# pachterlab/kallisto

Measured on AMD Instinct MI355X. Metric: M paired-end reads/sec quantified (human txome index), higher is better.
Workload: dtype u64+f64

## Files before the change

### kallisto_amd/csrc/kamd_ctx.hip

```cpp
#include "kamd_dev.h"

namespace {
void tuning_defaults(kamd_tuning* t) {
  memset(t, 0, sizeof *t);
  t->text_verify = 1; t->items_per_wave = 1024; t->refill_min = 8; t->lds_pad = -1;
  t->em_form = 3; t->em_local_block = 1024; t->em_group_div = -1; t->em_split_len = 16; t->em_small_nnz = -1; t->em_entries_per_lane = -1; t->em_windowed = 2; t->em_graph = 1; t->em_row_lanes = 4;
  t->em_fin_blocks = 1024; t->dedup_form = 2; t->align_chunks = -1; t->em_reg_slices = 1;
  t->em_hybrid = 1; t->overflow_second_pass = 1; t->em_giant_nnz = -1; t->em_blocked = 1;
}
void tuning_merge(kamd_tuning* t, const kamd_tuning& n) {
  if (n.text_verify == 1 || n.text_verify == 2) t->text_verify = n.text_verify;
  if (n.dedup_form == 1 || n.dedup_form == 2) t->dedup_form = n.dedup_form;
  if (n.items_per_wave >= 64) t->items_per_wave = n.items_per_wave;
  if (n.refill_min >= 1 && n.refill_min <= 64) t->refill_min = n.refill_min;
  if (n.lds_pad != 0) t->lds_pad = n.lds_pad < 0 ? -1 : n.lds_pad;
  if (n.em_form >= 1 && n.em_form <= 3) t->em_form = n.em_form;
  if (n.em_local_block == 128 || n.em_local_block == 256 || n.em_local_block == 512 || n.em_local_block == 1024) t->em_local_block = n.em_local_block;
  if (n.em_split_len >= 1 && n.em_split_len <= 64) t->em_split_len = n.em_split_len;
  if (n.em_group_div >= 1 && n.em_group_div <= 1024) t->em_group_div = n.em_group_div;
  else if (n.em_group_div < 0) t->em_group_div = -1;
  if (n.em_small_nnz != 0) t->em_small_nnz = n.em_small_nnz < 0 ? -1 : std::min(n.em_small_nnz, 4096);
  if (n.em_entries_per_lane != 0) t->em_entries_per_lane = n.em_entries_per_lane < 0 ? -1 : n.em_entries_per_lane;
  if (n.em_windowed == 1 || n.em_windowed == 2) t->em_windowed = n.em_windowed;
  if (n.em_graph == 1 || n.em_graph == 2) t->em_graph = n.em_graph;
// ... 10 lines not shown
  const char* e = getenv("KAMD_TUNE");
  if (!e || !*e) return;
  kamd_tuning n; memset(&n, 0, sizeof n);
  struct Field { const char* name; int32_t kamd_tuning::*p; bool onoff; };
  static const Field fields[] = {
    {"text_verify", &kamd_tuning::text_verify, true}, {"items_per_wave", &kamd_tuning::items_per_wave, false}, {"refill_min", &kamd_tuning::refill_min, false},
    {"lds_pad", &kamd_tuning::lds_pad, false}, {"em_form", &kamd_tuning::em_form, false}, {"em_entries_per_lane", &kamd_tuning::em_entries_per_lane, false},
    {"em_windowed", &kamd_tuning::em_windowed, true}, {"em_graph", &kamd_tuning::em_graph, true}, {"em_row_lanes", &kamd_tuning::em_row_lanes, false},
    {"em_fin_blocks", &kamd_tuning::em_fin_blocks, false}, {"em_local_block", &kamd_tuning::em_local_block, false}, {"em_group_div", &kamd_tuning::em_group_div, false},
    {"em_split_len", &kamd_tuning::em_split_len, false}, {"dedup_form", &kamd_tuning::dedup_form, false}, {"align_chunks", &kamd_tuning::align_chunks, false},
    {"em_small_nnz", &kamd_tuning::em_small_nnz, false}, {"em_reg_slices", &kamd_tuning::em_reg_slices, true}, {"em_hybrid", &kamd_tuning::em_hybrid, true},
    {"overflow_second_pass", &kamd_tuning::overflow_second_pass, false}, {"em_giant_nnz", &kamd_tuning::em_giant_nnz, false}, {"em_blocked", &kamd_tuning::em_blocked, true}};
  std::string all(e);
  for (size_t pos = 0; pos < all.size();) {
    size_t end = all.find(',', pos);
    if (end == std::string::npos) end = all.size();
    const std::string kv = all.substr(pos, end - pos);
    pos = end + 1;
    const size_t eq = kv.find('=');
    if (eq == std::string::npos) continue;
    const std::string key = kv.substr(0, eq), val = kv.substr(eq + 1);
    bool known = false;
    for (const Field& f : fields) {
      if (key != f.name) continue;
      known = true;
      int32_t v = atoi(val.c_str());
      if (key == "em_form") v = val == "streamed" ? 1 : val == "csr" ? 2 : val == "local" ? 3 : v;
      if (key == "overflow_second_pass" && v == 0) v = 2;
      n.*(f.p) = f.onoff ? (v != 0 ? 1 : 2) : v;
    }
    if (!known) fprintf(stderr, "[kallisto_amd] KAMD_TUNE: unknown field '%s' ignored\n", key.c_str());
  }
  tuning_merge(t, n);
}
}
namespace kamdi {
void apply_quant_opts(kamd_ctx* c, const kamd_quant_opts* o) {
  c->ix.no_jump = o->no_jump ? 1 : 0;
  c->ix.union_mode = o->do_union ? 1 : 0;
  c->ix.comprehensive = (o->strand != 0 && (o->no_jump || o->do_union || c->ix.n_shades)) ? 1 : 0;
}
void apply_tuning(kamd_ctx* c) {
  c->items_per_wave = c->tune.items_per_wave; c->refill_min = c->tune.refill_min;
}
int sync_state(kamd_ctx* c) {
  if (!c->state_pin) HIPC(hipHostMalloc((void**)&c->state_pin, sizeof(DevState), hipHostMallocDefault));
  HIPC(hipMemcpyAsync(c->state_pin, c->state.p, sizeof(DevState), hipMemcpyDeviceToHost, c->stream));
  HIPC(hipStreamSynchronize(c->stream));
  memcpy(&c->host_state, c->state_pin, sizeof(DevState));
  return 0;
}
int push_state(kamd_ctx* c) {
  HIPC(hipMemcpyAsync(c->state.p, &c->host_state, sizeof(DevState), hipMemcpyHostToDevice, c->stream));
  return 0;
}
}

extern "C" uint32_t kamd_abi_version(void) { return KAMD_ABI_VERSION; }
extern "C" int kamd_ctx_create(int device, void* hip_stream, kamd_ctx** out) {
  if (!out) return kamd::fail(-1, "kamd_ctx_create: null output pointer");
  *out = nullptr;
  int ndev = 0;
  if (hipGetDeviceCount(&ndev) != hipSuccess || ndev == 0)
    return kamd::fail(-102, "kamd_ctx_create: no HIP device available (this library has no CPU path)");
  if (device < 0 || device >= ndev) return kamd::fail(-1, "kamd_ctx_create: bad device ordinal");
  HIPC(hipSetDevice(device));
  kamd_ctx* c = new kamd_ctx;
  c->device = device;
  c->stream = (hipStream_t)hip_stream;
  { int v = 0; if (hipDeviceGetAttribute(&v, hipDeviceAttributeMultiprocessorCount, device) != hipSuccess || v <= 0) v = 256; c->n_cus = v; }
  if (c->state.ensure(sizeof(DevState), 0, c->stream)) { delete c; return -100; }
  memset(&c->host_state, 0, sizeof c->host_state);
  if (push_state(c)) { delete c; return -100; }
  if (hipEventCreate(&c->ev0) != hipSuccess || hipEventCreate(&c->ev1) != hipSuccess || hipEventCreate(&c->ev2) != hipSuccess || hipEventCreate(&c->ev3) != hipSuccess) { delete c; return kamd::fail(-100, "hipEventCreate failed"); }
  if (c->stats_a.ensure(sizeof(DevStatsA), 0, c->stream) || hipMemsetAsync(c->stats_a.p, 0, sizeof(DevStatsA), c->stream) != hipSuccess) { delete c; return -100; }
  tuning_defaults(&c->tune);
  tuning_from_env(&c->tune);
  apply_tuning(c);
  *out = c;
  return 0;
}

extern "C" int kamd_ctx_tune(kamd_ctx* c, const kamd_tuning* t) {
  if (!c || !t) return kamd::fail(-1, "kamd_ctx_tune: null argument");
  tuning_merge(&c->tune, *t);
  apply_tuning(c);
  return 0;
}
extern "C" int kamd_ctx_get_tuning(const kamd_ctx* c, kamd_tuning* out) {
  if (!c || !out) return kamd::fail(-1, "kamd_ctx_get_tuning: null argument");
  *out = c->tune;
  return 0;
}

extern "C" void kamd_ctx_destroy(kamd_ctx* c) {
  if (!c) return;
  (void)hipSetDevice(c->device);
  (void)hipStreamSynchronize(c->stream);
  comm_detach_all(c);
  if (c->ev0) (void)hipEventDestroy(c->ev0);
  if (c->ev1) (void)hipEventDestroy(c->ev1);
  if (c->ev2) (void)hipEventDestroy(c->ev2);
  if (c->ev3) (void)hipEventDestroy(c->ev3);
  if (c->al_stream) { (void)hipStreamSynchronize(c->al_stream); (void)hipStreamDestroy(c->al_stream); }
  if (c->al_ev_in) (void)hipEventDestroy(c->al_ev_in);
  if (c->al_ev_out) (void)hipEventDestroy(c->al_ev_out);
  for (hipEvent_t e : c->al_ev_chunk) if (e) (void)hipEventDestroy(e);
  if (c->ev_fin0) (void)hipEventDestroy(c->ev_fin0);
  if (c->ev_fin1) (void)hipEventDestroy(c->ev_fin1);
  for (hipEvent_t e : c->aa_ev) if (e) (void)hipEventDestroy(e);
  for (hipEvent_t e : c->rec_ev) if (e) (void)hipEventDestroy(e);
  for (hipEvent_t e : c->bus_ev) if (e) (void)hipEventDestroy(e);
  if (c->ev_ab0) (void)hipEventDestroy(c->ev_ab0);
  if (c->ev_ab1) (void)hipEventDestroy(c->ev_ab1);
  if (c->em_stream) (void)hipStreamDestroy(c->em_stream);
  if (c->em_side_stream) { (void)hipStreamSynchronize(c->em_side_stream); (void)hipStreamDestroy(c->em_side_stream); }
  if (c->em_ev_fork) (void)hipEventDestroy(c->em_ev_fork);
  if (c->em_ev_join) (void)hipEventDestroy(c->em_ev_join);
  if (c->em_pin) (void)hipHostFree(c->em_pin);
  if (c->plan_pin) (void)hipHostFree(c->plan_pin);
  if (c->state_pin) (void)hipHostFree(c->state_pin);
  c->em_clk.release();
  if (c->hy_giant_stream) { (void)hipStreamSynchronize(c->hy_giant_stream); (void)hipStreamDestroy(c->hy_giant_stream); }
  if (c->hy_ev_sell) (void)hipEventDestroy(c->hy_ev_sell);
  if (c->hy_ev_giant) (void)hipEventDestroy(c->hy_ev_giant);
  if (c->ev_mg0) (void)hipEventDestroy(c->ev_mg0);
  if (c->ev_mg1) (void)hipEventDestroy(c->ev_mg1);
  if (c->ev_ov0) (void)hipEventDestroy(c->ev_ov0);
  if (c->ev_ov1) (void)hipEventDestroy(c->ev_ov1);
  if (c->ov_stream) { (void)hipStreamSynchronize(c->ov_stream); (void)hipStreamDestroy(c->ov_stream); }
  for (hipEvent_t e : {c->ov_ev_in, c->ov_ev_done, c->ov_ev_t0, c->ov_ev_t1}) if (e) (void)hipEventDestroy(e);
  if (c->ov_pin) (void)hipHostFree(c->ov_pin);
  c->ov_state.release();
  for (DBuf* b : {&c->hy_sub, &c->hy_a, &c->hy_b, &c->hy_x, &c->hy_maps, &c->hy_gb[0], &c->hy_gb[1], &c->hy_gb[2], &c->hy_gb[3], &c->hy_gb[4], &c->hy_gb[5]}) b->release();
  if (c->fld_stream) { (void)hipStreamSynchronize(c->fld_stream); (void)hipStreamDestroy(c->fld_stream); }
  if (c->fld_ev) (void)hipEventDestroy(c->fld_ev);
  if (c->fld_ev_in) (void)hipEventDestroy(c->fld_ev_in);
  if (c->fld_host) (void)hipHostFree(c->fld_host);
  if (c->fq_host) (void)hipHostFree(c->fq_host);
  if (c->sell_cache) sell_cache_free(c->sell_cache);
  for (void* p : c->index_allocs) (void)hipFree(p);
  for (DBuf* b : {&c->dense, &c->stream_buf, &c->rec_off, &c->overflow_items, &c->overflow_scratch, &c->state, &c->rec_slot,
                  &c->retry, &c->ttable, &c->tstore, &c->stats_a, &c->list, &c->cand, &c->cand_off, &c->cand_slot, &c->ctable, &c->tup_bound, &c->tup_off, &c->tup_big, &c->raw2, &c->overflow_left, &c->stats_b, &c->clist, &c->sizes, &c->explicit_items,
                  &c->explicit_items_big, &c->exp_stream, &c->exp_off, &c->exp_scratch, &c->bs_cp, &c->bs_samp, &c->raw, &c->dense_first, &c->exp_key, &c->cand_key, &c->ec_first, &c->pm_a, &c->pm_b, &c->pm_rank, &c->eml_tmp, &c->ems_tmp, &c->ems_plan, &c->ems_maps, &c->fld_tl, &c->fld_card, &c->fld_scratch, &c->fld_items, &c->fld_cand,
                  &c->block_sums, &c->ec_off, &c->ec_ids, &c->ec_counts, &c->em_alpha, &c->em_next, &c->em_eff,
                  &c->em_state, &c->em_cn, &c->em_colcnt, &c->em_coloff, &c->em_colrow,
                  &c->em_segoff, &c->em_segt, &c->em_partial, &c->em_a0, &c->em_a1, &c->em_single, &c->em_actflag, &c->em_actpos, &c->em_active, &c->pt_label, &c->pt_flag, &c->pt_len,
                  &c->pt_rowpos, &c->pt_nnzpos, &c->pt_off, &c->pt_ids, &c->pt_counts, &c->pt_wcounts, &c->pt_hist, &c->pt_ck_alpha,
                  &c->pt_ck_a, &c->fq_tiles, &c->fq_nlpos[0], &c->fq_nlpos[1], &c->fq_recs, &c->fq_res, &c->fq_words, &c->fq_len, &c->aa_frames, &c->aa_flen, &c->aa_scratch, &c->aa_offlist, &c->aa_ctr, &c->inf_members, &c->inf_res, &c->txt_counts, &c->txt_res,
                  &c->rec_table, &c->rec_scratch, &c->rec_big_scratch, &c->rec_big_items, &c->rec_ctr, &c->bus_blk, &c->bus_ctr})
    b->release();
  delete c;
}

namespace {
__global__ void k_bm_fill(const u64* __restrict__ ec_off, const u32* __restrict__ ec_ids, const u32* __restrict__ which, u32 stride, u32* words) {
  const u32 e = which[blockIdx.x];
  u32* w = words + (u64)blockIdx.x * stride;
  for (u64 j = ec_off[e] + threadIdx.x; j < ec_off[e + 1]; j += blockDim.x) { const u32 x = ec_ids[j]; atomicOr(&w[x >> 5], 1u << (x & 31)); }
}
}
extern "C" int kamd_index_upload(kamd_ctx* c, const kamd_index* hix) {
  if (!c || !hix) return kamd::fail(-1, "kamd_index_upload: null argument");
  HIPC(hipSetDevice(c->device));
  kamd_index_view v;
  if (int rc = kamd_index_get_view(hix, &v)) return rc;
  const bool build_table = v.table == nullptr;
  HIPC(hipStreamSynchronize(c->stream));
  c->has_index = false;
  for (void* p : c->index_allocs) (void)hipFree(p);
  c->index_allocs.clear();
  DevIndex d{};
  d.k = v.k; d.n_buckets = v.n_buckets; d.n_ecs = v.n_ecs;
  d.table_layout = (int)v.table_layout; d.tag_q = v.tag_q; d.tag_dsh = v.tag_dsh; d.tag_w = v.tag_w;
  const u64 slots = (v.n_buckets + v.pad_buckets) * v.slots_per_bucket;
  if (!build_table) {
    if (int rc = upload(c, (const u64*)v.table, (size_t)(v.n_buckets + v.pad_buckets) * 8, &d.table)) return rc;
    if (int rc = upload(c, v.slot_block, slots, &d.slot_block)) return rc;
    if (int rc = upload(c, v.slot_dist, slots, &d.slot_dist)) return rc;
  }
  if (int rc = upload(c, v.uec_ec, v.n_uec, &d.uec_ec)) return rc;
  if (int rc = upload(c, (const u64*)v.ec_off, v.n_ecs + 1, &d.ec_off)) return rc;
  if (int rc = upload(c, v.ec_ids, v.ec_nnz, &d.ec_ids)) return rc;
  std::vector<uint8_t> ne(v.n_ecs + 1);
  for (u64 e = 0; e < v.n_ecs; e++) ne[e] = v.ec_off[e + 1] > v.ec_off[e];
  if (int rc = upload(c, ne.data(), v.n_ecs, &d.ec_nonempty)) return rc;
  std::vector<u32> ecn(v.n_uec + 1);
  for (u64 u = 0; u < v.n_uec; u++) ecn[u] = v.uec_ec[u] | (ne[v.uec_ec[u]] ? 0x80000000u : 0u);
  if (int rc = upload(c, ecn.data(), v.n_uec, &d.uec_ecn)) return rc;
  if (int rc = upload(c, v.onlist_bits, v.onlist_words, &d.onlist_bits)) return rc;
  d.n_shades = v.n_shades;
  if (v.n_shades) {
    if (int rc = upload(c, (const u64*)v.core_off, v.n_ecs + 1, &d.core_off)) return rc;
    if (int rc = upload(c, v.core_ids, (size_t)v.core_nnz, &d.core_ids)) return rc;
    if (int rc = upload(c, (const u64*)v.shade_off, v.n_ecs + 1, &d.shade_off)) return rc;
    if (int rc = upload(c, v.shade_ids, (size_t)v.shade_nnz, &d.shade_ids)) return rc;
// ... 434 lines not shown
  c->em_coll_ms = 0.f; c->em_coll_n = 0;
  if (int rc = kamd_em_run_partitioned(c, (uint32_t)m->rank, (uint32_t)m->world, comm_sum_cb, m, eff_lens, n_targets, n_iter, min_rounds, alpha, abz, rounds)) return rc;
  const auto t_fin = std::chrono::steady_clock::now();
  HIPC(hipSetDevice(c->device));
  if (int rc = m->tmp_a.ensure(2 * n_targets * sizeof(double), 0, c->stream)) return rc;
  double* d = m->tmp_a.as<double>();
  HIPC(hipMemcpyAsync(d, alpha, n_targets * sizeof(double), hipMemcpyHostToDevice, c->stream));
  HIPC(hipMemcpyAsync(d + n_targets, abz, n_targets * sizeof(double), hipMemcpyHostToDevice, c->stream));
  HIPC(hipStreamSynchronize(c->stream));
  if (int rc = comm_allreduce(m, d, 2 * n_targets, 3)) return rc;
  HIPC(hipMemcpyAsync(alpha, d, n_targets * sizeof(double), hipMemcpyDeviceToHost, c->stream));
  HIPC(hipMemcpyAsync(abz, d + n_targets, n_targets * sizeof(double), hipMemcpyDeviceToHost, c->stream));
  HIPC(hipStreamSynchronize(c->stream));
  c->em_coll_ms += std::chrono::duration<float, std::milli>(std::chrono::steady_clock::now() - t_fin).count(); c->em_coll_n += 1;
  return 0;
}

extern "C" int kamd_quant_batches(kamd_ctx* c, const kamd_quant_opts* o, const kamd_batch* batches, uint64_t n_batches, const int32_t* target_lens,
                                  uint64_t n_targets, kamd_comm* comm, kamd_quant_out* out) {
  if (!c || !o || (n_batches && !batches) || !target_lens || !out || !out->flens || !out->eff_lens || !out->est_counts)
    return kamd::fail(-1, "kamd_quant_batches: null argument");
  if (comm && comm->ctx != c) return kamd::fail(-1, "kamd_quant_batches: communicator of another context");
  if (n_targets != c->n_targets) return kamd::fail(-1, "kamd_quant_batches: n_targets differs from the uploaded index");
  const bool multi = comm && (comm->world > 1 || comm->nccl);
  const bool rank0 = !comm || comm->rank == 0;
  const bool estimate = o->paired && o->fld == 0.0;
  memset(out->flens, 0, KAMD_MAX_FRAG_LEN * sizeof(uint32_t));
  uint64_t used = 0, n_proc = 0;
  for (uint64_t b = 0; b < n_batches; b++) {
    const kamd_batch& B = batches[b];
    if (b == 0 && estimate && rank0) if (int rc = kamd_fld_prefetch(c, o, B.d_words, B.d_len, B.n_items, B.max_len)) return rc;
    if (int rc = kamd_pseudoalign(c, o, B.d_words, B.d_len, B.n_items, B.max_len)) return rc;
    n_proc += B.n_items;
    if (estimate && used < 10000 && rank0) if (int rc = kamd_fld_from_batch(c, o, B.d_words, B.d_len, B.n_items, B.max_len, out->flens, &used)) return rc;
  }
  if (multi) {
    if (int rc = kamd_comm_sum_u64_host(c, comm, &n_proc, 1)) return rc;
    if (estimate) {
      std::vector<uint32_t> pack(KAMD_MAX_FRAG_LEN + 2);
      for (int r = 0; r < comm->world; r++) {
        if (r > 0 && comm->rank == r)
          for (uint64_t b = 0; b < n_batches && used < 10000; b++)
            if (int rc = kamd_fld_from_batch(c, o, batches[b].d_words, batches[b].d_len, batches[b].n_items, batches[b].max_len, out->flens, &used)) return rc;
        memcpy(pack.data(), out->flens, KAMD_MAX_FRAG_LEN * sizeof(uint32_t));
        pack[KAMD_MAX_FRAG_LEN] = (uint32_t)used; pack[KAMD_MAX_FRAG_LEN + 1] = (uint32_t)(used >> 32);
        if (int rc = kamd_comm_broadcast_host(c, comm, pack.data(), pack.size() * sizeof(uint32_t), r)) return rc;
        memcpy(out->flens, pack.data(), KAMD_MAX_FRAG_LEN * sizeof(uint32_t));
        used = (uint64_t)pack[KAMD_MAX_FRAG_LEN] | ((uint64_t)pack[KAMD_MAX_FRAG_LEN + 1] << 32);
        if (used >= 10000) break;
      }
    }
    if (int rc = kamd_ec_allreduce(c, comm)) return rc;
  }
  std::vector<double> mft(KAMD_MAX_FRAG_LEN);
  std::thread eff_thread([&] {
    if (o->fld == 0.0) kamd_mean_frag_lens_trunc(out->flens, mft.data());
    else kamd_trunc_gaussian_fld(0, KAMD_MAX_FRAG_LEN, o->fld, o->sd, mft.data());
    kamd_eff_lens(target_lens, n_targets, mft.data(), out->eff_lens);
  });
  const int fin_rc = kamd_ec_finalize(c, nullptr);
  eff_thread.join();
  if (fin_rc) return fin_rc;
  int32_t rounds = 0;
  if (multi) { if (int rc = kamd_em_run_comm(c, comm, out->eff_lens, n_targets, 10000, 50, out->est_counts, out->alpha_before_zeroes, &rounds)) return rc; }
  else if (int rc = kamd_em_run(c, nullptr, nullptr, nullptr, nullptr, 0, out->eff_lens, n_targets, 10000, 50, out->est_counts, out->alpha_before_zeroes, &rounds)) return rc;
  if (out->tpm) kamd_counts_to_tpm(out->est_counts, out->eff_lens, n_targets, out->tpm);
  out->n_processed = n_proc; out->em_rounds = rounds;
  return 0;
}
```

### kallisto_amd/csrc/kamd_dev.h

```cpp
#pragma once

#include <hip/hip_runtime.h>

#include <dlfcn.h>

#include <algorithm>
#include <cstring>
#include <string>
#include <chrono>
#include <thread>
#include <vector>

#include "../../include/kallisto_amd.h"
#include "kamd_core.h"
#include "kamd_fq_core.h"
#include "kamd_host.h"
#include "kamd_em_local.h"
#include "kamd_em_sell.h"

#define HIPC(x)                                                                                   \
  do {                                                                                            \
    hipError_t e_ = (x);                                                                          \
    if (e_ != hipSuccess) return kamd::fail(-100, std::string(#x) + ": " + hipGetErrorString(e_)); \
  } while (0)

namespace kamdi {

typedef unsigned long long u64;
typedef unsigned int u32;

constexpr int BLOCK = 256;
constexpr int TUPLE_CAP = 12;
constexpr int TUPLE_CAP_BIG = 1024;
constexpr int EXPLICIT_HITS = 256;

struct DevIndex {
  const u64* table; u64 n_buckets;
  int table_layout; u32 tag_q, tag_dsh, tag_w;
  const u32* slot_block; const u32* slot_dist;
  const u32* uec_ec;
  const u64* ec_off; const u32* ec_ids; const uint8_t* ec_nonempty;
  const u32* uec_ecn;
  const u32* onlist_bits;
  const u32* ec_bm_slot; const u32* bm_words; u32 bm_stride, bm_min;
  u64 n_ecs; int k;
  const u64* unitig_blk_off; const u32* unitig_len; const u32* blk_unitig; const u32* blk_lb; const u32* blk_ub; const u32* blk_ec;
  const u64* blk_pos_off; const u32* blk_posw; const uint8_t* blk_sense; const int32_t* target_lens;
  const u64* dtable; u64 n_dbuckets; u64 dummy_slot; u32 dummy_uec; u32 dummy_strand;
  const u32* utext;
  int no_jump;
  int union_mode;
  int comprehensive;
  u64 n_shades; const u64* core_off; const u32* core_ids; const u64* shade_off; const u32* shade_ids; const u32* shade_colour;
};
__host__ __device__ inline kamd::Table make_table(const DevIndex& ix, bool partial) {
  kamd::Table t{(const uint64_t*)ix.table, ix.n_buckets};
  t.layout = (uint8_t)ix.table_layout; t.q = (uint8_t)ix.tag_q; t.dsh = (uint8_t)ix.tag_dsh; t.tagw = (uint8_t)ix.tag_w;
  t.dslots = (const uint64_t*)ix.dtable; t.n_dbuckets = ix.n_dbuckets; t.dummy_uec = ix.dummy_uec; t.dummy_slot = ix.dummy_slot;
  t.dummy_strand = ix.dummy_strand != 0; t.partial = partial && !ix.union_mode && !ix.n_shades;
  t.no_jump = ix.no_jump != 0;
// ... 144 lines not shown
using namespace kamdi;
namespace {
__global__ void k_copy_words(const u32* __restrict__ src, u64 n, u32* dst) {
  u64 i = (u64)blockIdx.x * blockDim.x + threadIdx.x;
  if (i < n) dst[i] = src[i];
}
__global__ void k_copy_offsets(const u64* __restrict__ src, u64 n, u64 base, u64* dst) {
  u64 i = (u64)blockIdx.x * blockDim.x + threadIdx.x;
  if (i < n) dst[i] = src[i] + base;
}
}

struct kamd_ctx {
  int device = 0;
  hipStream_t stream = nullptr;
  bool has_index = false;
  DevIndex ix{};
  std::vector<void*> index_allocs;
  u64 n_ecs = 0, n_targets = 0;
  u32 n_set_bitmaps = 0;
  kamd_table_info tinfo{};
  DBuf dense, stream_buf, rec_off, overflow_items, overflow_scratch, state, rec_slot, retry, ttable, list;
  DBuf cand, cand_off, cand_slot, ctable, clist, sizes, block_sums, tup_bound, tup_off, tup_big;
  DBuf raw2, overflow_left, stats_b;
  u64 overflow_second_total = 0;
  DBuf ov_state; DevState* ov_pin = nullptr; hipStream_t ov_stream = nullptr; hipEvent_t ov_ev_in = nullptr, ov_ev_done = nullptr, ov_ev_t0 = nullptr, ov_ev_t1 = nullptr;
  bool ov_side_pending = false;
  u64 last_fin_big = 0;
  DBuf explicit_items, explicit_items_big, exp_stream, exp_off, exp_scratch, bs_cp, bs_samp, raw, dense_first, exp_key, cand_key, ec_first;
  DBuf ec_off, ec_ids, ec_counts;
  DBuf em_alpha, em_next, em_eff, em_state, em_cn, em_colcnt, em_coloff, em_colrow, em_segoff, em_segt, em_partial, em_a0, em_a1, em_single, em_actflag, em_actpos, em_active;
  DBuf pm_a, pm_b, pm_rank;
  DBuf eml_tmp, ems_tmp, ems_plan, ems_maps;
  SellCache* sell_cache = nullptr;
  u64 ec_generation = 0;
  int last_em_plan_cached = 0;
  DBuf fq_tiles, fq_nlpos[2], fq_recs, fq_res, fq_words, fq_len;
  void* fq_host = nullptr;
  u64 fq_batch_reads = 0; int32_t fq_batch_max_len = 0, fq_batch_files = 0;
  DBuf fld_tl, fld_card, fld_scratch, fld_items, fld_cand;
  void* fld_host = nullptr; u64 fld_host_cap = 0;
  hipStream_t fld_stream = nullptr; hipEvent_t fld_ev = nullptr, fld_ev_in = nullptr;
  struct { const uint32_t* w = nullptr; const uint16_t* l = nullptr; u64 n = 0; int32_t max_len = 0, strand = 0, so = 0; bool valid = false; } fld_pending;
  struct { const uint32_t* w = nullptr; const uint16_t* l = nullptr; u64 n = 0; int32_t max_len = 0, strand = 0, so = 0, comp = 0; bool valid = false; } fld_deferred;
  DBuf pt_label, pt_flag, pt_len, pt_rowpos, pt_nnzpos, pt_off, pt_ids, pt_counts, pt_wcounts, pt_hist, pt_ck_alpha, pt_ck_a;
  DevState host_state{};
  DevState* state_pin = nullptr;
  u64 tcap = 0, ccap = 0;
  DBuf tstore;
  bool ttable_clean = false;
  u64 recs_total = 0;
  u64 multi_before = 0;
  u64 n_distinct_tuples = 0;
  float last_absorb_ms = 0.f; hipEvent_t ev_ab0 = nullptr, ev_ab1 = nullptr;
  kamd_ec_result result{};
  bool finalized = false;
  u64 exp_words_done = 0;
  hipEvent_t ev0 = nullptr, ev1 = nullptr;
  float last_align_ms = 0.f, last_em_ms = 0.f, last_classify_ms = 0.f;
  hipEvent_t ev2 = nullptr, ev3 = nullptr, ev_fin0 = nullptr, ev_fin1 = nullptr;
  DBuf stats_a;
  hipStream_t al_stream = nullptr; hipEvent_t al_ev_in = nullptr, al_ev_out = nullptr; std::vector<hipEvent_t> al_ev_chunk;
  float last_finalize_ms = 0.f; u64 last_fin_records = 0, last_fin_stream_words = 0, last_fin_cand_words = 0;
  hipStream_t em_stream = nullptr;
  hipStream_t em_side_stream = nullptr; hipEvent_t em_ev_fork = nullptr, em_ev_join = nullptr;
  void* em_pin = nullptr; size_t em_pin_bytes = 0;
  void* plan_pin = nullptr; size_t plan_pin_bytes = 0;
  DBuf em_clk;
  DBuf hy_sub, hy_a, hy_b, hy_x, hy_maps;
  DBuf hy_gb[6];
  hipStream_t hy_giant_stream = nullptr;
  hipEvent_t hy_ev_sell = nullptr, hy_ev_giant = nullptr;
  uint64_t last_em_max_comp_nnz = 0, last_em_giant_nnz = 0, last_em_giant_rows = 0, last_em_giant_tr = 0;
  uint32_t last_em_giant_chunks = 0; uint64_t last_em_giant_pieces = 0; int last_em_graph_fallback = 0; float last_em_plan_ms = 0.f;
  float last_merge_ms = 0.f, em_coll_ms = 0.f; uint32_t em_coll_n = 0; hipEvent_t ev_mg0 = nullptr, ev_mg1 = nullptr;
  const uint32_t* labels_override = nullptr;
  bool em_prefer_hybrid = false;
  uint64_t overflow_total = 0; float overflow_ms = 0.f; hipEvent_t ev_ov0 = nullptr, ev_ov1 = nullptr;
  int items_per_wave = 1024, refill_min = 8;
  kamd_tuning tune{};
  bool track_order = false;
  bool had_overflow_items = false;
  int n_cus = 0, last_em_k = 0; unsigned last_em_grid = 0, last_em_lds = 0;
  uint64_t last_em_iters = 0, last_em_nnz = 0, last_em_nnz_multi = 0, last_em_nseg = 0, last_em_necs = 0;
  DBuf aa_frames, aa_flen, aa_scratch, aa_offlist, aa_ctr;
  bool aa_ready = false;
  kamd_aa_stats aa_stats{};
  hipEvent_t aa_ev[3] = {nullptr, nullptr, nullptr};
  DBuf inf_members, inf_res, txt_counts, txt_res;
  DBuf rec_table, rec_scratch, rec_big_scratch, rec_big_items, rec_ctr;
  u64 rec_table_gen = 0, rec_table_cap = 0, rec_chunk = 0, rec_second = 0;
  int rec_small_cap = 0;
  hipEvent_t rec_ev[3] = {nullptr, nullptr, nullptr};
  float rec_table_ms = 0.f, rec_items_ms = 0.f;
  DBuf bus_blk, bus_ctr;
  hipEvent_t bus_ev[2] = {nullptr, nullptr};
  std::vector<struct kamd_comm*> comms;
};

namespace kamdi {
int sync_state(kamd_ctx* c);
int push_state(kamd_ctx* c);
void apply_quant_opts(kamd_ctx* c, const kamd_quant_opts* o);
void apply_tuning(kamd_ctx* c);
void comm_detach_all(kamd_ctx* c);
int index_build_device(kamd_ctx* c, const kamd_index* hix, const kamd_index_view& v, DevIndex* d, kamd_table_info* info);
int exclusive_scan(kamd_ctx* c, const u32* sizes, u64 n, u64* out, u64* d_total);
int tuples_clear(kamd_ctx* c);
int absorb_tuples(kamd_ctx* c, const u32* batch, const u64* rec_off, u64 n, u64 batch_words, u64 key_base, u64 n_tuple_bound,
                  const u64* first_idx = nullptr, u32 fixed_stride = 0, u64 item0 = 0);
template <class T>
int upload(kamd_ctx* c, const T* host, size_t n, const T** dev) {
  void* p = nullptr;
  size_t bytes = std::max<size_t>(n, 1) * sizeof(T);
  HIPC(hipMalloc(&p, bytes));
  c->index_allocs.push_back(p);
  if (n) HIPC(hipMemcpyAsync(p, host, n * sizeof(T), hipMemcpyHostToDevice, c->stream));
  *dev = reinterpret_cast<const T*>(p);
  return 0;
}
}
```

### kallisto_amd/csrc/kamd_ec.hip

```cpp
#include "kamd_dev.h"

namespace {

__global__ void k_table_init(TSlot* t, u64 cap) {
  u64 i = (u64)blockIdx.x * blockDim.x + threadIdx.x;
  if (i < cap) { t[i].tag = 0; t[i].owner = ~0ULL; t[i].count = 0; t[i].first = ~0ULL; }
}
__global__ void k_rec_insert(const u32* __restrict__ stream, const u64* __restrict__ rec_off, const u64* __restrict__ idx,
                             u64 r0, u64 n, TSlot* table, u64 mask, u64 seed, u64* rec_slot) {
  u64 i = (u64)blockIdx.x * blockDim.x + threadIdx.x;
  if (i >= n) return;
  const u64 r = idx ? idx[i] : r0 + i;
  const u64 off = rec_off[r];
  if (off == ~0ULL || stream[off] == 0u) return;
  const u32 m = stream[off + 1];
  const u64 tag = rec_hash(stream + off + 1, m + 1, seed);
  u64 s = (tag >> 1) & mask;
  for (;;) {
    u64 old = atomicCAS(&table[s].tag, 0ULL, tag);
    if (old == 0ULL || old == tag) break;
    s = (s + 1) & mask;
  }
  atomicMin(&table[s].owner, off);
  rec_slot[r] = s;
// ... 152 lines not shown
  for (int q = 0; q < ABS_Q; q++) {
    cand[q] = live[q] && !slow[q] && old[q] != 0ULL && (old[q] >> 32) == (h[q] >> 32);
    const u32* o = ((old[q] & TAG_LOCAL) ? batch : store) + ((old[q] & 0x7FFFFFFFULL) - 1);
    const u32 m = w[q][1];
#pragma unroll
    for (int j = 0; j < 5; j++) ow[q][j] = (cand[q] && (u32)j <= m) ? o[1 + j] : 0u;
  }
#pragma unroll
  for (int q = 0; q < ABS_Q; q++) {
    if (!live[q] || slow[q]) continue;
    bool same = cand[q] && ow[q][0] == w[q][1];
#pragma unroll
    for (int j = 0; j < 4; j++) if ((u32)j < w[q][1]) same = same && ow[q][1 + j] == w[q][2 + j];
    if (same) {
      atomicAdd(&table[sl[q]].count, (u64)w[q][0]);
      if (track & 1) atomicMin(&table[sl[q]].first, key_base + i + (u64)q * T);
    } else slow[q] = true;
  }
  u32 my[ABS_Q]; u64 own_s[ABS_Q]; bool is_owner[ABS_Q];
#pragma unroll
  for (int q = 0; q < ABS_Q; q++) {
    is_owner[q] = false; my[q] = 0; own_s[q] = 0;
    if (!slow[q]) continue;
    const u64 r = i + (u64)q * T, o = off[q];
    const u32 m = batch[o + 1];
    const u64 hh = rec_hash(batch + o + 1, m + 1, 1);
    const u64 mine = (hh & 0xFFFFFFFF00000000ULL) | TAG_LOCAL | (o + 1);
    u64 s = (hh >> 1) & mask;
    bool placed = false;
    for (u32 probes = 0; probes < max_probe; probes++) {
      u64 od = table[s].tag;
      if (od == 0ULL) od = atomicCAS(&table[s].tag, 0ULL, mine);
      if (od == 0ULL) { is_owner[q] = true; table[s].owner = o; placed = true; break; }
      if ((od >> 32) == (mine >> 32)) {
        const u32* ob = ((od & TAG_LOCAL) ? batch : store) + ((od & 0x7FFFFFFFULL) - 1);
        bool same = ob[1] == m;
        for (u32 j = 0; same && j < m; j++) same = ob[2 + j] == batch[o + 2 + j];
        if (same) { placed = true; break; }
      }
      s = (s + 1) & mask;
    }
    if (placed) {
      atomicAdd(&table[s].count, (u64)batch[o]);
      if (track & 1) atomicMin(&table[s].first, key_base + r);
    } else fail[atomicAdd(&st->tl_fail, 1ULL)] = r;
    if (is_owner[q]) { own_s[q] = s; my[q] = atomicAdd(&blk_n, 1u); atomicAdd(&blk_words, m + 2u); }
  }
  __syncthreads();
  if (threadIdx.x == 0 && blk_n) { blk_base = atomicAdd(&st->tl_n, (u64)blk_n); atomicAdd(&st->bound_words, (u64)blk_words); }
  __syncthreads();
#pragma unroll
  for (int q = 0; q < ABS_Q; q++) if (is_owner[q]) list[blk_base + my[q]] = own_s[q];
}
__global__ __launch_bounds__(BLOCK) void k_tup_store(const u32* __restrict__ batch, u32* store, TSlot* table, u64* list, u64 first_new,
                                                     u64 n_new, DevState* st) {
  __shared__ u32 wsum[BLOCK / 64]; __shared__ u64 blk_base;
  const u64 i = (u64)blockIdx.x * blockDim.x + threadIdx.x;
  u64 s = 0, off = 0; u32 need = 0;
  if (i < n_new) { s = list[first_new + i] & 0xFFFFFFFFULL; off = table[s].owner; need = batch[off + 1] + 2u; }
  const u32 incl = wave_incl_scan(need);
  if (lane_id() == 63) wsum[threadIdx.x >> 6] = incl;
  __syncthreads();
  if (threadIdx.x == 0) { u32 t = 0; for (int j = 0; j < BLOCK / 64; j++) t += wsum[j]; blk_base = t ? atomicAdd(&st->ts_words, (u64)t) : 0ULL; }
  __syncthreads();
  if (i >= n_new) return;
  u32 before = 0;
  for (u32 j = 0; j < (threadIdx.x >> 6); j++) before += wsum[j];
  const u64 dst = blk_base + before + incl - need;
  for (u32 j = 0; j < need; j++) store[dst + j] = batch[off + j];
  table[s].owner = dst;
  table[s].tag = (table[s].tag & 0xFFFFFFFF00000000ULL) | (dst + 1);
  list[first_new + i] = s | (dst << 32);
}
__global__ void k_tup_rehash(const u32* __restrict__ store, const TSlot* __restrict__ old, TSlot* nu, u64 mask, u64* list, u64 n) {
  const u64 i = (u64)blockIdx.x * blockDim.x + threadIdx.x;
  if (i >= n) return;
  const TSlot o = old[list[i] & 0xFFFFFFFFULL];
  const u32 m = store[o.owner + 1];
  const u64 h = rec_hash(store + o.owner + 1, m + 1, 1);
  const u64 tag = (h & 0xFFFFFFFF00000000ULL) | (o.owner + 1);
  u64 s = (h >> 1) & mask;
  while (atomicCAS(&nu[s].tag, 0ULL, tag) != 0ULL) s = (s + 1) & mask;
  nu[s].owner = o.owner; nu[s].count = o.count; nu[s].first = o.first;
  list[i] = s | (o.owner << 32);
}

constexpr u64 SHADE_SMALL = 64;
constexpr u64 SHADE_SLOT_FACTOR = 4;
constexpr u32 RES_BIG_MIN = 16;
__global__ void k_bound_tuples(DevIndex ix, const u32* __restrict__ stream, const TSlot* table, const u64* list, u64 n,
                               u32* per_tuple, u32* big_idx, u32* shade_idx, DevState* st) {
  u64 i = (u64)blockIdx.x * blockDim.x + threadIdx.x;
  u64 b = 0;
  bool big = false, huge = false, sh_small = false, sh_long = false;
  if (i < n) {
    const u64 off = list[i] >> 32;
    const u32 m = stream[off + 1];
    u64 core_b;
    if (ix.n_shades) {
      const kamd::ShadeTables sh = shade_tables(ix);
      const kamd::SetTables core{sh.core_off, sh.core_ids};
      core_b = kamd::set_size_bound(core, stream + off + 2, (int)m, ix.union_mode != 0);
      const u64 S = kamd::shaded_size_bound(sh, stream + off + 2, (int)m, ix.union_mode != 0) - core_b;
      b = core_b + (ix.union_mode ? S : SHADE_SLOT_FACTOR * S) + 2;
      sh_small = !ix.union_mode && S != 0 && core_b + S <= SHADE_SMALL;
      sh_long = !ix.union_mode && S != 0 && !sh_small;
    } else {
      const kamd::SetTables stt{(const uint64_t*)ix.ec_off, ix.ec_ids};
      core_b = kamd::set_size_bound(stt, stream + off + 2, (int)m, ix.union_mode != 0);
      b = core_b + 2;
    }
    per_tuple[i] = (u32)b;
    big = big_idx && !ix.union_mode && core_b > RES_BIG_MIN;
    huge = big && core_b > 1024;
  }
  b = wave_sum64(b);
  if (lane_id() == 0 && b) atomicAdd(&st->bound_words, b);
  const u64 bm = __ballot(big && !huge), hm = __ballot(huge);
  if (bm) {
    u64 base = 0;
    if (lane_id() == 0) base = atomicAdd(&st->n_big, (u64)__popcll(bm));
    base = shfl_u64(base, 0);
    if (big && !huge) big_idx[base + __popcll(bm & ((1ULL << lane_id()) - 1ULL))] = (u32)i;
  }
  if (hm) {
    u64 base = 0;
    if (lane_id() == 0) base = atomicAdd(&st->n_huge, (u64)__popcll(hm));
    base = shfl_u64(base, 0);
    if (huge) big_idx[n - 1 - (base + __popcll(hm & ((1ULL << lane_id()) - 1ULL)))] = (u32)i;
  }
  const u64 sm = __ballot(sh_small), lm = __ballot(sh_long);
  if (sm) {
    u64 base = 0;
    if (lane_id() == 0) base = atomicAdd(&st->n_sh_small, (u64)__popcll(sm));
    base = shfl_u64(base, 0);
    if (sh_small) shade_idx[base + __popcll(sm & ((1ULL << lane_id()) - 1ULL))] = (u32)i;
  }
  if (lm) {
    u64 base = 0;
    if (lane_id() == 0) base = atomicAdd(&st->n_sh_long, (u64)__popcll(lm));
    base = shfl_u64(base, 0);
    if (sh_long) shade_idx[n - 1 - (base + __popcll(lm & ((1ULL << lane_id()) - 1ULL)))] = (u32)i;
  }
}
__global__ void k_bound_singles(DevIndex ix, const u32* __restrict__ dense, DevState* st) {
  u64 e = (u64)blockIdx.x * blockDim.x + threadIdx.x;
  u64 b = 0;
  if (e < ix.n_ecs && dense[e]) b = ix.ec_off[e + 1] - ix.ec_off[e] + 2;
  b = wave_sum64(b);
  if (lane_id() == 0 && b) atomicAdd(&st->bound_words, b);
}
__global__ void k_cand_singles(DevIndex ix, const u32* __restrict__ dense, const u64* __restrict__ dense_first, u32* cand,
                               u64* cand_off, u64* cand_key, DevState* st) {
  u64 e = (u64)blockIdx.x * blockDim.x + threadIdx.x;
  const bool have = e < ix.n_ecs && dense[e] != 0;
  const u32* ids = nullptr; u32 n = 0;
  if (have) { ids = ix.ec_ids + ix.ec_off[e]; n = (u32)(ix.ec_off[e + 1] - ix.ec_off[e]); }
  const bool longset = n > 64;
  if (have && !longset) {
    u32 keep = 0;
    for (u32 j = 0; j < n; j++) keep += onlisted(ix.onlist_bits, ids[j]);
    if (keep) {
      u64 off = atomicAdd(&st->cand_words, (u64)keep + 2);
      u64 r = atomicAdd(&st->cand_recs, 1ULL);
      u32* w = cand + off;
      w[0] = dense[e]; w[1] = keep;
      u32 o = 0;
      for (u32 j = 0; j < n; j++) if (onlisted(ix.onlist_bits, ids[j])) w[2 + o++] = ids[j];
      cand_off[r] = off;
      if (cand_key) cand_key[r] = dense_first[e];
    }
  }
  u64 m = __ballot(longset);
  while (m) {
    const int src = __ffsll((long long)m) - 1;
    m &= m - 1;
    const u64 se = shfl_u64(e, src);
    const u32* sid = ix.ec_ids + ix.ec_off[se];
    const u32 sn = (u32)__shfl((int)n, src, 64);
    u32 keep = 0;
    for (u32 j = lane_id(); j < sn; j += 64) keep += onlisted(ix.onlist_bits, sid[j]);
#pragma unroll
    for (int d = 1; d < 64; d <<= 1) keep += (u32)__shfl_xor((int)keep, d, 64);
    if (keep == 0) continue;
    u64 off = 0, r = 0;
    if (lane_id() == 0) { off = atomicAdd(&st->cand_words, (u64)keep + 2); r = atomicAdd(&st->cand_recs, 1ULL); }
    off = shfl_u64(off, 0); r = shfl_u64(r, 0);
    u32* w = cand + off;
    if (lane_id() == 0) { w[0] = dense[se]; w[1] = keep; cand_off[r] = off; if (cand_key) cand_key[r] = dense_first[se]; }
    u32 o = 0;
    for (u32 j0 = 0; j0 < sn; j0 += 64) {
      const u32 j = j0 + lane_id();
      const u32 x = j < sn ? sid[j] : 0u;
      const bool ok = j < sn && onlisted(ix.onlist_bits, x);
      const u64 bm = __ballot(ok);
      if (ok) w[2 + o + __popcll(bm & ((1ULL << lane_id()) - 1ULL))] = x;
      o += (u32)__popcll(bm);
    }
  }
}
constexpr int RES_LANES = 16;
constexpr int RES_BLOCK = BLOCK;
__global__ __launch_bounds__(RES_BLOCK) void k_resolve(DevIndex ix, const u32* __restrict__ stream, const TSlot* table,
                                                   const u64* list, u64 n, const u64* __restrict__ slot_off, u32* cand, u64* cand_off,
                                                   u64* cand_key, const DevState* st) {
  const u64 base_words = st->cand_words, base_recs = st->cand_recs;
  const u64 gid = ((u64)blockIdx.x * blockDim.x + threadIdx.x) / RES_LANES;
  const bool valid = gid < n;
  const int lane = lane_id();
  const int sub = lane & (RES_LANES - 1);
  const int gsh = lane & ~(RES_LANES - 1);
  TSlot sl; sl.owner = 0; sl.count = 0; sl.tag = 0; sl.first = ~0ULL;
  u32 m = 0, best = 0, nb = 0;
  const u32* es = nullptr; const u32* base = nullptr;
  u64 my_off = 0; u32 my_sz = 0xFFFFFFFFu;
  bool small = false;
  if (valid) {
// ... 509 lines not shown
  if (c->tune.dedup_form != 1 && stream_words < 0xFFFFFFFFULL) {
    c->host_state.n_retry = 0;
    HIPC(hipMemcpyAsync(&((DevState*)c->state.p)->n_retry, &c->host_state.n_retry, sizeof(u64), hipMemcpyHostToDevice, c->stream));
    hipLaunchKernelGGL(k_rec_dedup, dim3(grid_for(n, BLOCK)), dim3(BLOCK), 0, c->stream, stream, rec_off, r0, n, table, cap - 1, list, keys, track,
                       max_probe ? max_probe : 0xFFFFFFFFu, (DevState*)c->state.p);
    HIPC(hipGetLastError());
    if (int rc = sync_state(c)) return rc;
    return c->host_state.n_retry ? 2 : 0;
  }
  if (int rc = slot_buf.ensure(r1 * sizeof(u64), 0, c->stream)) return rc;
  if (int rc = c->retry.ensure(2 * n * sizeof(u64), 0, c->stream)) return rc;
  u64* retry_a = c->retry.as<u64>();
  u64* retry_b = retry_a + n;
  const u64* idx = nullptr;
  u64 count = n;
  for (u64 seed = 1; count; seed++) {
    c->host_state.n_retry = 0;
    HIPC(hipMemcpyAsync(&((DevState*)c->state.p)->n_retry, &c->host_state.n_retry, sizeof(u64), hipMemcpyHostToDevice, c->stream));
    hipLaunchKernelGGL(k_rec_insert, dim3(grid_for(count, BLOCK)), dim3(BLOCK), 0, c->stream, stream, rec_off, idx, r0, count,
                       table, cap - 1, seed, slot_buf.as<u64>());
    hipLaunchKernelGGL(k_rec_verify, dim3(grid_for(count, VERIFY_BLOCK)), dim3(VERIFY_BLOCK), 0, c->stream, stream, rec_off, idx, r0, count,
                       table, slot_buf.as<u64>(), retry_b, list, keys, track, (DevState*)c->state.p);
    HIPC(hipGetLastError());
    if (int rc = sync_state(c)) return rc;
    count = c->host_state.n_retry;
    std::swap(retry_a, retry_b);
    idx = retry_a;
    if (seed > 64) return kamd::fail(-101, "dedup_records: tag collisions did not resolve");
  }
  return 0;
}


int exclusive_scan(kamd_ctx* c, const u32* sizes, u64 n, u64* out, u64* d_total) {
  const u64 nblocks = std::max<u64>(1, (n + SCAN_ELEMS - 1) / SCAN_ELEMS);
  if (int rc = c->block_sums.ensure((nblocks + 2) * sizeof(u64), 0, c->stream)) return rc;
  hipLaunchKernelGGL(k_scan_local, dim3((unsigned)nblocks), dim3(BLOCK), 0, c->stream, sizes, n, out, c->block_sums.as<u64>());
  hipLaunchKernelGGL(k_scan_blocks, dim3(1), dim3(BLOCK), 0, c->stream, c->block_sums.as<u64>(), nblocks, d_total);
  hipLaunchKernelGGL(k_scan_add, dim3((unsigned)nblocks), dim3(BLOCK), 0, c->stream, out, n, c->block_sums.as<u64>());
  HIPC(hipGetLastError());
  return 0;
}

u64 pow2_at_least(u64 x) { u64 p = 1024; while (p < x) p <<= 1; return p; }

int tuples_clear(kamd_ctx* c) {
  if (c->tcap && !c->ttable_clean) {
    hipLaunchKernelGGL(k_table_init, dim3(grid_for(c->tcap, BLOCK)), dim3(BLOCK), 0, c->stream, c->ttable.as<TSlot>(), c->tcap);
    HIPC(hipGetLastError());
    c->ttable_clean = true;
  }
  c->host_state.tl_n = 0; c->host_state.ts_words = 0; c->host_state.tl_fail = 0;
  c->n_distinct_tuples = 0;
  return 0;
}
int tuples_resize(kamd_ctx* c, u64 cap) {
  if (cap > (1ULL << 32)) return kamd::fail(-101, "absorb_tuples: the tuple table would need more than 2^32 slots");
  const u64 n = c->host_state.tl_n;
  DBuf nu;
  if (int rc = nu.ensure(cap * sizeof(TSlot), 0, c->stream)) return rc;
  hipLaunchKernelGGL(k_table_init, dim3(grid_for(cap, BLOCK)), dim3(BLOCK), 0, c->stream, nu.as<TSlot>(), cap);
  if (n) hipLaunchKernelGGL(k_tup_rehash, dim3(grid_for(n, BLOCK)), dim3(BLOCK), 0, c->stream, (const u32*)c->tstore.as<u32>(), (const TSlot*)c->ttable.as<TSlot>(),
                            nu.as<TSlot>(), cap - 1, c->list.as<u64>(), n);
  HIPC(hipGetLastError());
  HIPC(hipStreamSynchronize(c->stream));
  c->ttable.release();
  c->ttable = nu; c->tcap = cap; c->ttable_clean = n == 0;
  return 0;
}
int absorb_tuples(kamd_ctx* c, const u32* batch, const u64* rec_off, u64 n, u64 batch_words, u64 key_base, u64 n_tuple_bound,
                  const u64* first_idx, u32 fixed_stride, u64 item0) {
  if (n == 0) return 0;
  if (batch_words >= 0x7FFFFFF0ULL) return kamd::fail(-1, "kamd_pseudoalign: the record stream of one batch must stay below 2^31 words (use smaller batches)");
  DevState* dst = (DevState*)c->state.p;
  if (!c->ev_ab0) { HIPC(hipEventCreate(&c->ev_ab0)); HIPC(hipEventCreate(&c->ev_ab1)); }
  HIPC(hipEventRecord(c->ev_ab0, c->stream));
  const u64 bound = std::min(n, n_tuple_bound);
  u64 want = pow2_at_least(std::max<u64>(bound / 4, 2 * c->host_state.tl_n) + 16);
  if (c->tcap == 0) {
    c->tcap = want;
    if (int rc = c->ttable.ensure(c->tcap * sizeof(TSlot), 0, c->stream)) return rc;
    hipLaunchKernelGGL(k_table_init, dim3(grid_for(c->tcap, BLOCK)), dim3(BLOCK), 0, c->stream, c->ttable.as<TSlot>(), c->tcap);
    c->ttable_clean = true;
  } else if (2 * c->host_state.tl_n + 16 > c->tcap) {
    if (int rc = tuples_resize(c, pow2_at_least(4 * c->host_state.tl_n + 16))) return rc;
  }
  if (int rc = c->list.ensure((c->host_state.tl_n + bound + 1) * sizeof(u64), c->host_state.tl_n * sizeof(u64), c->stream)) return rc;
  if (int rc = c->retry.ensure(2 * (bound + 1) * sizeof(u64), 0, c->stream)) return rc;
  u64* fail_a = c->retry.as<u64>();
  u64* fail_b = fail_a + bound + 1;
  const u64* idx = first_idx;
  u64 count = n;
  for (int round = 0; count; round++) {
    if (round > 40) return kamd::fail(-101, "absorb_tuples: the tuple table does not settle");
    const u64 tl_before = c->host_state.tl_n;
    c->host_state.tl_fail = 0; c->host_state.bound_words = 0;
    if (int rc = push_state(c)) return rc;
    if (!idx && fixed_stride >= 6 && (fixed_stride & 1) == 0)
      hipLaunchKernelGGL(k_tup_absorb4, dim3(grid_for((count + ABS_Q - 1) / ABS_Q, BLOCK)), dim3(BLOCK), 0, c->stream, batch, (const u32*)c->tstore.as<u32>(), count,
                         c->ttable.as<TSlot>(), c->tcap - 1, c->list.as<u64>(), key_base, c->track_order ? 1 : 0, 64u, fail_a, dst, fixed_stride, item0);
    else
    hipLaunchKernelGGL(k_tup_absorb, dim3(grid_for(count, BLOCK)), dim3(BLOCK), 0, c->stream, batch, (const u32*)c->tstore.as<u32>(), rec_off, idx, count,
                       c->ttable.as<TSlot>(), c->tcap - 1, c->list.as<u64>(), key_base,
                       c->track_order ? 1 : 0, 64u, fail_a, dst,
                       fixed_stride, item0);
    HIPC(hipGetLastError());
    c->ttable_clean = false;
    if (int rc = sync_state(c)) return rc;
    const u64 n_new = c->host_state.tl_n - tl_before, new_words = c->host_state.bound_words;
    if (n_new) {
      if (c->host_state.ts_words + new_words >= 0x7FFFFFF0ULL) return kamd::fail(-101, "absorb_tuples: more than 2^31 words of distinct tuples");
      if (int rc = c->tstore.ensure((c->host_state.ts_words + new_words + 2) * sizeof(u32), c->host_state.ts_words * sizeof(u32), c->stream)) return rc;
      hipLaunchKernelGGL(k_tup_store, dim3(grid_for(n_new, BLOCK)), dim3(BLOCK), 0, c->stream, batch, c->tstore.as<u32>(), c->ttable.as<TSlot>(),
                         c->list.as<u64>(), tl_before, n_new, dst);
      HIPC(hipGetLastError());
      c->host_state.ts_words += new_words;
    }
    count = c->host_state.tl_fail;
    if (count) {
      if (int rc = tuples_resize(c, c->tcap * 4)) return rc;
      std::swap(fail_a, fail_b);
      idx = fail_b;
    }
  }
  c->n_distinct_tuples = c->host_state.tl_n;
  HIPC(hipEventRecord(c->ev_ab1, c->stream));
  HIPC(hipEventSynchronize(c->ev_ab1));
  float ms = 0.f;
  HIPC(hipEventElapsedTime(&ms, c->ev_ab0, c->ev_ab1));
  c->last_absorb_ms += ms;
  return 0;
}

}
extern "C" int kamd_ec_dense_counts(kamd_ctx* c, uint32_t** d_counts, uint64_t* n) {
  if (!c || !d_counts || !n) return kamd::fail(-1, "kamd_ec_dense_counts: null argument");
  *d_counts = c->dense.as<u32>(); *n = c->n_ecs;
  return 0;
}
extern "C" int kamd_ec_tuples_export(kamd_ctx* c, uint64_t* n_words, uint64_t* n_tuples) {
  if (!c || !n_words || !n_tuples) return kamd::fail(-1, "kamd_ec_tuples_export: null argument");
  HIPC(hipSetDevice(c->device));
  if (int rc = sync_state(c)) return rc;
  c->host_state.bound_words = 0;
  if (int rc = push_state(c)) return rc;
  const u64 n = c->n_distinct_tuples;
  if (n) hipLaunchKernelGGL(k_tuple_export_size, dim3(grid_for(n, BLOCK)), dim3(BLOCK), 0, c->stream, c->tstore.as<u32>(),
                            c->ttable.as<TSlot>(), c->list.as<u64>(), n, (DevState*)c->state.p);
  HIPC(hipGetLastError());
  if (int rc = sync_state(c)) return rc;
  *n_words = c->host_state.bound_words; *n_tuples = n;
  return 0;
}
extern "C" int kamd_ec_tuples_copy(kamd_ctx* c, uint32_t* d_out_words, uint64_t* d_out_rec_off) {
  if (!c || !d_out_words || !d_out_rec_off) return kamd::fail(-1, "kamd_ec_tuples_copy: null argument");
  HIPC(hipSetDevice(c->device));
  const u64 n = c->n_distinct_tuples;
  c->host_state.cand_words = 0; c->host_state.cand_recs = 0;
  if (int rc = push_state(c)) return rc;
  if (n) hipLaunchKernelGGL(k_tuple_export_offsets, dim3(grid_for(n, BLOCK)), dim3(BLOCK), 0, c->stream, c->tstore.as<u32>(),
                            c->ttable.as<TSlot>(), c->list.as<u64>(), n, d_out_words, (u64*)d_out_rec_off, (DevState*)c->state.p);
  HIPC(hipGetLastError());
  return sync_state(c);
}
extern "C" int kamd_ec_tuples_replace(kamd_ctx* c, const uint32_t* d_words, uint64_t n_words, const uint64_t* d_rec_off,
                                      uint64_t n_recs) {
  if (!c) return kamd::fail(-1, "kamd_ec_tuples_replace: null argument");
  if (c->track_order) return kamd::fail(-1, "kamd_ec_tuples_replace: merged records have no input order (kamd_ec_track_order is on)");
  HIPC(hipSetDevice(c->device));
  if (int rc = sync_state(c)) return rc;
  if (int rc = tuples_clear(c)) return rc;
  if (int rc = push_state(c)) return rc;
  c->had_overflow_items = true;
  c->finalized = false;
  return absorb_tuples(c, d_words, (const u64*)d_rec_off, n_recs, n_words, 0, n_recs);
}

extern "C" int kamd_ec_explicit_export(kamd_ctx* c, uint64_t* n_words, uint64_t* n_recs) {
  if (!c || !n_words || !n_recs) return kamd::fail(-1, "kamd_ec_explicit_export: null argument");
  HIPC(hipSetDevice(c->device));
  if (int rc = sync_state(c)) return rc;
  *n_words = c->exp_words_done; *n_recs = c->host_state.exp_recs;
  return 0;
}
extern "C" int kamd_ec_explicit_copy(kamd_ctx* c, uint32_t* d_out_words, uint64_t* d_out_rec_off) {
  if (!c) return kamd::fail(-1, "kamd_ec_explicit_copy: null argument");
  HIPC(hipSetDevice(c->device));
  if (c->exp_words_done) HIPC(hipMemcpyAsync(d_out_words, c->exp_stream.p, c->exp_words_done * sizeof(u32), hipMemcpyDeviceToDevice, c->stream));
  if (c->host_state.exp_recs) HIPC(hipMemcpyAsync(d_out_rec_off, c->exp_off.p, c->host_state.exp_recs * sizeof(u64), hipMemcpyDeviceToDevice, c->stream));
  HIPC(hipStreamSynchronize(c->stream));
  return 0;
}
extern "C" int kamd_ec_explicit_replace(kamd_ctx* c, const uint32_t* d_words, uint64_t n_words, const uint64_t* d_rec_off,
                                        uint64_t n_recs) {
  if (!c) return kamd::fail(-1, "kamd_ec_explicit_replace: null argument");
  if (c->track_order) return kamd::fail(-1, "kamd_ec_explicit_replace: merged records have no input order (kamd_ec_track_order is on)");
  HIPC(hipSetDevice(c->device));
  if (int rc = sync_state(c)) return rc;
  if (int rc = c->exp_stream.ensure(std::max<u64>(n_words, 1) * sizeof(u32), 0, c->stream)) return rc;
  if (int rc = c->exp_off.ensure((n_recs + 1) * sizeof(u64), 0, c->stream)) return rc;
  if (n_words) HIPC(hipMemcpyAsync(c->exp_stream.p, d_words, n_words * sizeof(u32), hipMemcpyDeviceToDevice, c->stream));
  if (n_recs) HIPC(hipMemcpyAsync(c->exp_off.p, d_rec_off, n_recs * sizeof(u64), hipMemcpyDeviceToDevice, c->stream));
  c->exp_words_done = n_words; c->host_state.exp_recs = n_recs; c->host_state.exp_words = n_words;
  c->finalized = false;
  return push_state(c);
}

extern "C" int kamd_ec_track_order(kamd_ctx* c, int on) {
  if (!c) return kamd::fail(-1, "kamd_ec_track_order: null context");
  if (c->host_state.st_processed != 0) return kamd::fail(-1, "kamd_ec_track_order: call before the first batch (or after kamd_ec_reset)");
  c->track_order = on != 0;
  return 0;
}

extern "C" int kamd_ec_finalize(kamd_ctx* c, kamd_ec_result* out) {
  if (!c) return kamd::fail(-1, "kamd_ec_finalize: null context");
  if (!c->has_index) return kamd::fail(-1, "kamd_ec_finalize: no index uploaded");
  HIPC(hipSetDevice(c->device));
  if (!c->ev_fin0) { HIPC(hipEventCreate(&c->ev_fin0)); HIPC(hipEventCreate(&c->ev_fin1)); }
  HIPC(hipEventRecord(c->ev_fin0, c->stream));
  if (int rc = sync_state(c)) return rc;
  DevState* dst = (DevState*)c->state.p;
  const u64 n_t = c->n_distinct_tuples;
  c->host_state.bound_words = 0; c->host_state.cand_words = 0; c->host_state.cand_recs = 0; c->host_state.n_big = 0; c->host_state.n_huge = 0;
  c->host_state.n_sh_small = 0; c->host_state.n_sh_long = 0; c->host_state.shade_err = 0;
  if (int rc = push_state(c)) return rc;
  hipLaunchKernelGGL(k_bound_singles, dim3(grid_for(c->n_ecs, BLOCK)), dim3(BLOCK), 0, c->stream, c->ix, c->dense.as<u32>(), dst);
  if (int rc = c->tup_bound.ensure((n_t + 1) * sizeof(u32), 0, c->stream)) return rc;
  if (int rc = c->tup_off.ensure((n_t + 2) * sizeof(u64), 0, c->stream)) return rc;
  if (int rc = c->tup_big.ensure(2 * (n_t + 1) * sizeof(u32), 0, c->stream)) return rc;
  if (n_t) {
    hipLaunchKernelGGL(k_bound_tuples, dim3(grid_for(n_t, BLOCK)), dim3(BLOCK), 0, c->stream, c->ix, c->tstore.as<u32>(),
                       c->ttable.as<TSlot>(), c->list.as<u64>(), n_t, c->tup_bound.as<u32>(), c->tup_big.as<u32>(), c->tup_big.as<u32>() + (n_t + 1), dst);
    if (int rc = exclusive_scan(c, c->tup_bound.as<u32>(), n_t, c->tup_off.as<u64>(), c->tup_off.as<u64>() + n_t)) return rc;
  }
  HIPC(hipGetLastError());
  u64 tup_words = 0;
  if (n_t) HIPC(hipMemcpyAsync(&tup_words, c->tup_off.as<u64>() + n_t, sizeof(u64), hipMemcpyDeviceToHost, c->stream));
  if (int rc = sync_state(c)) return rc;
  const u64 n_exp_w = c->exp_words_done, n_exp_r = c->host_state.exp_recs;
  const u64 bound = c->host_state.bound_words + n_exp_w;
  const u64 max_cands = c->n_ecs + n_t + n_exp_r;
  if (int rc = c->cand.ensure((bound + 2) * sizeof(u32), 0, c->stream)) return rc;
  if (int rc = c->cand_off.ensure((max_cands + 1) * sizeof(u64), 0, c->stream)) return rc;
  if (c->track_order) if (int rc = c->cand_key.ensure((max_cands + 1) * sizeof(u64), 0, c->stream)) return rc;
  u64* cand_key = c->track_order ? c->cand_key.as<u64>() : nullptr;
  hipLaunchKernelGGL(k_cand_singles, dim3(grid_for(c->n_ecs, BLOCK)), dim3(BLOCK), 0, c->stream, c->ix, c->dense.as<u32>(),
                     c->dense_first.as<u64>(), c->cand.as<u32>(), c->cand_off.as<u64>(), cand_key, dst);
  if (n_t && c->ix.union_mode) {
    const bool big = c->had_overflow_items;
    if (big) if (int rc = c->overflow_scratch.ensure(n_t * (u64)TUPLE_CAP_BIG * sizeof(u32), 0, c->stream)) return rc;
    hipLaunchKernelGGL(k_resolve_union, dim3(grid_for(n_t, BLOCK)), dim3(BLOCK), 0, c->stream, c->ix, c->tstore.as<u32>(),
                       c->ttable.as<TSlot>(), c->list.as<u64>(), n_t, c->tup_off.as<u64>(), c->cand.as<u32>(), c->cand_off.as<u64>(),
                       cand_key, big ? c->overflow_scratch.as<u32>() : nullptr, dst);
  } else if (n_t) {
    const DevIndex rix = core_view(c->ix);
    hipLaunchKernelGGL(k_resolve, dim3(grid_for(n_t * RES_LANES, RES_BLOCK)), dim3(RES_BLOCK), 0, c->stream, rix, c->tstore.as<u32>(),
                       c->ttable.as<TSlot>(), c->list.as<u64>(), n_t, c->tup_off.as<u64>(), c->cand.as<u32>(), c->cand_off.as<u64>(),
                       cand_key, dst);
    const u64 n_big = c->host_state.n_big, n_huge = c->host_state.n_huge;
    if (n_big) hipLaunchKernelGGL(k_resolve_big<(int)RB_CAND_BIG>, dim3(grid_for(n_big, RB_WAVES)), dim3(64 * RB_WAVES), 0, c->stream, rix, c->tstore.as<u32>(),
                                  c->ttable.as<TSlot>(), c->list.as<u64>(), c->tup_big.as<u32>(), n_big, c->tup_off.as<u64>(), c->cand.as<u32>(),
                                  c->cand_off.as<u64>(), cand_key, dst);
    if (n_huge) hipLaunchKernelGGL(k_resolve_big<(int)RB_CAND_HUGE>, dim3(grid_for(n_huge, RB_WAVES)), dim3(64 * RB_WAVES), 0, c->stream, rix, c->tstore.as<u32>(),
                                   c->ttable.as<TSlot>(), c->list.as<u64>(), c->tup_big.as<u32>() + (n_t - n_huge), n_huge, c->tup_off.as<u64>(), c->cand.as<u32>(),
                                   c->cand_off.as<u64>(), cand_key, dst);
    c->last_fin_big = n_big + n_huge;
    if (c->ix.n_shades) {
      const u64 n_s = c->host_state.n_sh_small, n_l = c->host_state.n_sh_long;
      const u32* sw = c->tup_big.as<u32>() + (n_t + 1);
      if (n_s) hipLaunchKernelGGL(k_shade_extend<16>, dim3(grid_for(n_s * 16, BLOCK)), dim3(BLOCK), 0, c->stream, c->ix, c->tstore.as<u32>(), c->list.as<u64>(), sw, n_s,
                                  c->tup_off.as<u64>(), c->tup_bound.as<u32>(), c->cand.as<u32>(), c->cand_off.as<u64>(), dst);
      if (n_l) hipLaunchKernelGGL(k_shade_extend<64>, dim3(grid_for(n_l * 64, BLOCK)), dim3(BLOCK), 0, c->stream, c->ix, c->tstore.as<u32>(), c->list.as<u64>(), sw + (n_t - n_l), n_l,
                                  c->tup_off.as<u64>(), c->tup_bound.as<u32>(), c->cand.as<u32>(), c->cand_off.as<u64>(), dst);
    }
    if (getenv("KAMD_DEBUG_FIN")) fprintf(stderr, "[kamd] finalize: %llu distinct tuples, smallest set 17..1024: %llu, beyond: %llu\n", (unsigned long long)n_t,
                                          (unsigned long long)n_big, (unsigned long long)n_huge);
  }
  HIPC(hipGetLastError());
  if (int rc = sync_state(c)) return rc;
  if (c->host_state.shade_err) return kamd::fail(-4, "kamd_ec_finalize: a candidate slot is smaller than its shades need (k_bound_tuples and k_shade_extend disagree)");
  c->host_state.cand_words += tup_words; c->host_state.cand_recs += n_t;
  if (int rc = push_state(c)) return rc;
  if (n_exp_r) {
    const u64 wbase = c->host_state.cand_words, rbase = c->host_state.cand_recs;
    hipLaunchKernelGGL(k_copy_words, dim3(grid_for(n_exp_w, BLOCK)), dim3(BLOCK), 0, c->stream, c->exp_stream.as<u32>(), n_exp_w,
                       c->cand.as<u32>() + wbase);
    hipLaunchKernelGGL(k_copy_offsets, dim3(grid_for(n_exp_r, BLOCK)), dim3(BLOCK), 0, c->stream, c->exp_off.as<u64>(), n_exp_r, wbase,
                       c->cand_off.as<u64>() + rbase);
    if (cand_key) hipLaunchKernelGGL(k_copy_offsets, dim3(grid_for(n_exp_r, BLOCK)), dim3(BLOCK), 0, c->stream, c->exp_key.as<u64>(), n_exp_r,
                                     0ULL, cand_key + rbase);
    HIPC(hipGetLastError());
    c->host_state.cand_words = wbase + n_exp_w; c->host_state.cand_recs = rbase + n_exp_r;
  }
  const u64 n_cand = c->host_state.cand_recs;
  c->ccap = pow2_at_least(2 * n_cand + 16);
  if (int rc = c->ctable.ensure(c->ccap * sizeof(TSlot), 0, c->stream)) return rc;
  hipLaunchKernelGGL(k_table_init, dim3(grid_for(c->ccap, BLOCK)), dim3(BLOCK), 0, c->stream, c->ctable.as<TSlot>(), c->ccap);
  if (int rc = c->clist.ensure((n_cand + 1) * sizeof(u64), 0, c->stream)) return rc;
  if (int rc = dedup_records(c, c->cand.as<u32>(), c->cand_off.as<u64>(), 0, n_cand, c->ctable.as<TSlot>(), c->ccap, c->cand_slot,
                             c->clist.as<u64>(), cand_key ? 2 : 0, cand_key, 0, c->host_state.cand_words)) return rc;
  const u64 n_final = c->host_state.n_list;
  if (c->track_order && n_final > 1) {
    if (int rc = c->ec_first.ensure(n_final * sizeof(u64), 0, c->stream)) return rc;
    hipLaunchKernelGGL(k_final_keys, dim3(grid_for(n_final, BLOCK)), dim3(BLOCK), 0, c->stream, c->ctable.as<TSlot>(), c->clist.as<u64>(), n_final,
                       c->ec_first.as<u64>());
    std::vector<u64> keys(n_final), slots(n_final), sorted(n_final);
    HIPC(hipMemcpyAsync(keys.data(), c->ec_first.p, n_final * sizeof(u64), hipMemcpyDeviceToHost, c->stream));
    HIPC(hipMemcpyAsync(slots.data(), c->clist.p, n_final * sizeof(u64), hipMemcpyDeviceToHost, c->stream));
    HIPC(hipStreamSynchronize(c->stream));
    std::vector<u64> perm(n_final);
    for (u64 i = 0; i < n_final; i++) perm[i] = i;
    std::sort(perm.begin(), perm.end(), [&](u64 a, u64 b) { return keys[a] != keys[b] ? keys[a] < keys[b] : slots[a] < slots[b]; });
    for (u64 i = 0; i < n_final; i++) sorted[i] = slots[perm[i]];
    HIPC(hipMemcpyAsync(c->clist.p, sorted.data(), n_final * sizeof(u64), hipMemcpyHostToDevice, c->stream));
    HIPC(hipStreamSynchronize(c->stream));
  }
  if (int rc = c->sizes.ensure((n_final + 1) * sizeof(u32), 0, c->stream)) return rc;
  if (int rc = c->ec_off.ensure((n_final + 2) * sizeof(u64), 0, c->stream)) return rc;
  if (int rc = c->ec_counts.ensure((n_final + 1) * sizeof(u32), 0, c->stream)) return rc;
  u64 nnz = 0;
  if (n_final) {
    hipLaunchKernelGGL(k_final_sizes, dim3(grid_for(n_final, BLOCK)), dim3(BLOCK), 0, c->stream, c->cand.as<u32>(), c->ctable.as<TSlot>(),
                       c->clist.as<u64>(), n_final, c->sizes.as<u32>());
    if (int rc = exclusive_scan(c, c->sizes.as<u32>(), n_final, c->ec_off.as<u64>(), &dst->bound_words)) return rc;
    hipLaunchKernelGGL(k_set_last, dim3(1), dim3(64), 0, c->stream, c->ec_off.as<u64>(), n_final, &dst->bound_words);
    if (int rc = sync_state(c)) return rc;
    nnz = c->host_state.bound_words;
    if (int rc = c->ec_ids.ensure((nnz + 1) * sizeof(u32), 0, c->stream)) return rc;
    hipLaunchKernelGGL(k_final_write, dim3(grid_for(n_final * 64, BLOCK)), dim3(BLOCK), 0, c->stream, c->cand.as<u32>(), c->ctable.as<TSlot>(),
                       c->clist.as<u64>(), n_final, c->ec_off.as<u64>(), c->ec_ids.as<u32>(), c->ec_counts.as<u32>());
    HIPC(hipGetLastError());
  } else {
    HIPC(hipMemsetAsync(c->ec_off.p, 0, sizeof(u64), c->stream));
    if (int rc = c->ec_ids.ensure(sizeof(u32), 0, c->stream)) return rc;
  }
  HIPC(hipEventRecord(c->ev_fin1, c->stream));
  HIPC(hipStreamSynchronize(c->stream));
  HIPC(hipEventElapsedTime(&c->last_finalize_ms, c->ev_fin0, c->ev_fin1));
  c->last_fin_records = n_t; c->last_fin_stream_words = c->host_state.ts_words; c->last_fin_cand_words = c->host_state.cand_words;
  ++c->ec_generation;
  c->result.n_ecs = n_final; c->result.nnz = nnz;
  c->result.d_ec_off = c->ec_off.as<uint64_t>(); c->result.d_ec_ids = c->ec_ids.as<u32>(); c->result.d_counts = c->ec_counts.as<u32>();
  c->result.n_pseudoaligned = 0;
  c->finalized = true;
  if (out) *out = c->result;
  return 0;
}

extern "C" int kamd_ec_finalize_result(kamd_ctx* c, kamd_ec_result* out) {
  if (!c || !out) return kamd::fail(-1, "kamd_ec_finalize_result: null argument");
  if (!c->finalized) return kamd::fail(-1, "kamd_ec_finalize_result: call kamd_ec_finalize first");
  *out = c->result;
  return 0;
}

extern "C" int kamd_ec_download(kamd_ctx* c, uint64_t* ec_off, uint32_t* ec_ids, uint32_t* counts) {
  if (!c || !c->finalized) return kamd::fail(-1, "kamd_ec_download: call kamd_ec_finalize first");
  HIPC(hipSetDevice(c->device));
  HIPC(hipMemcpyAsync(ec_off, c->ec_off.p, (c->result.n_ecs + 1) * sizeof(u64), hipMemcpyDeviceToHost, c->stream));
  if (c->result.nnz) HIPC(hipMemcpyAsync(ec_ids, c->ec_ids.p, c->result.nnz * sizeof(u32), hipMemcpyDeviceToHost, c->stream));
  if (c->result.n_ecs) HIPC(hipMemcpyAsync(counts, c->ec_counts.p, c->result.n_ecs * sizeof(u32), hipMemcpyDeviceToHost, c->stream));
  HIPC(hipStreamSynchronize(c->stream));
  return 0;
}

extern "C" int kamd_ec_upload(kamd_ctx* c, const uint64_t* ec_off, const uint32_t* ec_ids, const uint32_t* counts, uint64_t n_ecs) {
  if (!c || !ec_off || (n_ecs && !ec_ids)) return kamd::fail(-1, "kamd_ec_upload: null argument");
  if (ec_off[0] != 0) return kamd::fail(-1, "kamd_ec_upload: ec_off[0] must be 0");
  std::vector<std::pair<u64, u64>> by_hash((size_t)n_ecs);
  for (u64 e = 0; e < n_ecs; e++) {
    if (ec_off[e + 1] <= ec_off[e]) return kamd::fail(-1, "kamd_ec_upload: empty equivalence class or offsets not increasing");
    u64 h = kamd::mix64(ec_off[e + 1] - ec_off[e]);
    for (u64 j = ec_off[e]; j < ec_off[e + 1]; j++) {
      if (j > ec_off[e] && ec_ids[j] <= ec_ids[j - 1]) return kamd::fail(-1, "kamd_ec_upload: the transcripts of an equivalence class must be sorted and distinct");
      if (c->has_index && ec_ids[j] >= c->n_targets) return kamd::fail(-1, "kamd_ec_upload: transcript id beyond the targets of the uploaded index");
      h = kamd::mix64(h ^ ec_ids[j]);
    }
    by_hash[(size_t)e] = {h, e};
  }
  std::sort(by_hash.begin(), by_hash.end());
  for (size_t i = 1; i < by_hash.size(); i++) {
    if (by_hash[i].first != by_hash[i - 1].first) continue;
    const u64 a = by_hash[i - 1].second, b = by_hash[i].second;
    if (ec_off[a + 1] - ec_off[a] == ec_off[b + 1] - ec_off[b] && std::equal(ec_ids + ec_off[a], ec_ids + ec_off[a + 1], ec_ids + ec_off[b]))
      return kamd::fail(-1, "kamd_ec_upload: equivalence classes " + std::to_string(std::min(a, b)) + " and " + std::to_string(std::max(a, b)) + " hold the same transcripts");
  }
  HIPC(hipSetDevice(c->device));
  const u64 nnz = ec_off[n_ecs];
  if (int rc = c->ec_off.ensure((n_ecs + 1) * sizeof(u64), 0, c->stream)) return rc;
  if (int rc = c->ec_ids.ensure(std::max<u64>(nnz, 1) * sizeof(u32), 0, c->stream)) return rc;
// ... 25 lines not shown
```

### kallisto_amd/csrc/kamd_em.hip

```cpp
#include "kamd_dev.h"

namespace {

struct EmState {
  int iter;
  int chcount;
  int final_round;
  int done;
  int rounds;
  int force_final;
  int pad[2];
};
struct EmNow { int it, fin, done, rounds; };
__host__ __device__ inline EmNow em_next_round(const EmState& prev, int n_iter, int min_rounds, bool spec) {
  EmNow n; n.it = prev.iter; n.fin = prev.final_round; n.done = prev.done; n.rounds = prev.rounds;
  if (n.done) return n;
  if (prev.final_round) { n.done = 1; n.rounds = prev.iter; return n; }
  const bool stopEM = !spec && prev.chcount == 0 && prev.iter > min_rounds;
  n.it = prev.iter + 1;
  n.fin = (stopEM || prev.force_final) ? 1 : 0;
  if (n.it >= n_iter) { n.done = 1; n.rounds = n_iter; }
  return n;
}
__device__ __forceinline__ double em_clamped(const double* alpha, const double* a, u32 t, int clamp) {
// ... 1806 lines not shown
  for (u64 r = (u64)blockIdx.x * blockDim.x + threadIdx.x; r < T; r += (u64)gridDim.x * blockDim.x) {
    v0 = max(v0, c_nnz[r]);
    if (c_rows) v1 = max(v1, c_rows[r]);
    if (c_tr) v2 = max(v2, c_tr[r]);
  }
  __shared__ u32 red[3][BLOCK / 64];
#pragma unroll
  for (int d = 32; d > 0; d >>= 1) { v0 = max(v0, (u32)__shfl_down(v0, d, 64)); v1 = max(v1, (u32)__shfl_down(v1, d, 64)); v2 = max(v2, (u32)__shfl_down(v2, d, 64)); }
  const int w = threadIdx.x >> 6;
  if (lane_id() == 0) { red[0][w] = v0; red[1][w] = v1; red[2][w] = v2; }
  __syncthreads();
  if (threadIdx.x == 0) {
    for (int i = 1; i < (int)(blockDim.x >> 6); i++) { v0 = max(v0, red[0][i]); v1 = max(v1, red[1][i]); v2 = max(v2, red[2][i]); }
    if (v0 > __atomic_load_n(&stats[0], __ATOMIC_RELAXED)) atomicMax(&stats[0], v0);
    if (v1 > __atomic_load_n(&stats[1], __ATOMIC_RELAXED)) atomicMax(&stats[1], v1);
    if (v2 > __atomic_load_n(&stats[2], __ATOMIC_RELAXED)) atomicMax(&stats[2], v2);
  }
}
constexpr unsigned COMP_STATS_BLOCKS = 256;
int cc_labels(kamd_ctx* c, const u64* d_ec_off, const u32* d_ec_ids, u64 n_ecs, u64 T) {
  if (int rc = c->pt_label.ensure((T + 1) * sizeof(u32), 0, c->stream)) return rc;
  hipLaunchKernelGGL(k_cc_init, dim3(grid_for(T, BLOCK)), dim3(BLOCK), 0, c->stream, c->pt_label.as<u32>(), T);
  if (n_ecs) hipLaunchKernelGGL(k_cc_union, dim3(grid_for(n_ecs, BLOCK)), dim3(BLOCK), 0, c->stream, d_ec_off, d_ec_ids, n_ecs, c->pt_label.as<u32>());
  hipLaunchKernelGGL(k_cc_flatten, dim3(grid_for(T, BLOCK)), dim3(BLOCK), 0, c->stream, c->pt_label.as<u32>(), T);
  HIPC(hipGetLastError());
  return 0;
}
int plan_pin_ensure(kamd_ctx* c, size_t bytes) {
  if (c->plan_pin_bytes >= bytes) return 0;
  if (c->plan_pin) { HIPC(hipStreamSynchronize(c->stream)); HIPC(hipHostFree(c->plan_pin)); c->plan_pin = nullptr; c->plan_pin_bytes = 0; }
  const size_t want = std::max<size_t>(bytes * 2, 64 * 1024);
  HIPC(hipHostMalloc(&c->plan_pin, want, hipHostMallocDefault));
  c->plan_pin_bytes = want;
  return 0;
}
int em_local_setup_device(kamd_ctx* c, const u64* d_ec_off, const u32* d_ec_ids, const u32* d_counts, const u32* d_wcounts, u64 n_ecs, u64 nnz,
                          const double* eff_lens, u64 T, u64 budget, u64 target, kamd_em_local::Plan* P, EmLocalDev* dev,
                          kamd_em_local::BuildArgs* args_out = nullptr, u32 small_limit = 0, u64 target_small = 0, bool host_maps = true,
                          CompStats* comp_out = nullptr) {
  namespace L = kamd_em_local;
  if (nnz >= (1ULL << 32) || T >= 0xFFFFFFF0ULL || n_ecs >= 0xFFFFFFF0ULL) return 1;
  if (int rc = c->pt_label.ensure((T + 1) * sizeof(u32), 0, c->stream)) return rc;
  if (int rc = c->pt_hist.ensure(64, 0, c->stream)) return rc;
  if (!c->labels_override) if (int rc = cc_labels(c, d_ec_off, d_ec_ids, n_ecs, T)) return rc;
  Carver t1;
  const size_t o_inm = t1.take(T + 8), o_sall = t1.take(T * 8 + 8), o_cn = t1.take(T * 4 + 8), o_cr = t1.take(T * 4 + 8), o_ct = t1.take(T * 4 + 8);
  const size_t o_cum = t1.take((T + 2) * 8), o_loc = t1.take(T * 4 + 8), o_eff = t1.take(T * 8 + 8), o_rnew = t1.take(n_ecs * 4 + 8);
  const size_t o_cs = t1.take(small_limit ? T * 4 + 8 : 8), o_cb = t1.take(small_limit ? T * 4 + 8 : 8), o_cumb = t1.take(small_limit ? (T + 2) * 8 : 8);
  const u64 ng_max = nnz / std::max<u64>(1, target) + 2 + (small_limit ? nnz / std::max<u64>(1, target_small) + 2 : 0);
  const size_t o_gr = t1.take(ng_max * 4 + 8), o_gt = t1.take(ng_max * 4 + 8), o_gn = t1.take(ng_max * 4 + 8), o_rf = t1.take(ng_max * 4 + 8),
               o_tf = t1.take(ng_max * 4 + 8);
  if (int rc = c->eml_tmp.ensure(t1.off, 0, c->stream)) return rc;
  char* tb = (char*)c->eml_tmp.p;
  HIPC(hipMemsetAsync(tb, 0, o_cum, c->stream));
  HIPC(hipMemcpyAsync(tb + o_eff, eff_lens, T * 8, hipMemcpyHostToDevice, c->stream));
  L::BuildArgs A{};
  A.ec_off = (const uint64_t*)d_ec_off; A.ec_ids = d_ec_ids; A.counts = d_counts; A.wcounts = d_wcounts; A.n_ecs = n_ecs;
  A.eff = (const double*)(tb + o_eff); A.T = T; A.label = c->labels_override ? c->labels_override : c->pt_label.as<u32>(); A.target_nnz = std::max<u64>(1, target);
  A.in_multi = (uint8_t*)(tb + o_inm); A.single_all = (double*)(tb + o_sall); A.c_nnz = (u32*)(tb + o_cn); A.c_rows = (u32*)(tb + o_cr);
  A.c_tr = (u32*)(tb + o_ct); A.cum_nnz = (const uint64_t*)(tb + o_cum); A.local_of = (u32*)(tb + o_loc); A.row_new = (u32*)(tb + o_rnew);
  hipLaunchKernelGGL(k_eml_step<0>, dim3(grid_for(n_ecs, BLOCK)), dim3(BLOCK), 0, c->stream, A, n_ecs);
  hipLaunchKernelGGL(k_eml_step<1>, dim3(grid_for(T, BLOCK)), dim3(BLOCK), 0, c->stream, A, T);
  if (int rc = plan_pin_ensure(c, 256)) return rc;
  CompStats cst{};
  CompStats* const cst_pin = (CompStats*)c->plan_pin;
  u64* const nz_pin = (u64*)((char*)c->plan_pin + 64);
  HIPC(hipMemsetAsync(c->pt_hist.p, 0, sizeof(CompStats), c->stream));
  hipLaunchKernelGGL(k_comp_stats, dim3(std::min<unsigned>(grid_for(T, BLOCK), COMP_STATS_BLOCKS)), dim3(BLOCK), 0, c->stream, A.c_nnz, A.c_rows, A.c_tr, T, (u32*)c->pt_hist.p);
  HIPC(hipMemcpyAsync(cst_pin, c->pt_hist.p, sizeof(CompStats), hipMemcpyDeviceToHost, c->stream));
  u64 NZ = 0;
  u32 ng = 0;
  P->n_small = 0;
  if (small_limit) {
    A.small_limit = small_limit; A.c_small = (u32*)(tb + o_cs); A.c_big = (u32*)(tb + o_cb);
    hipLaunchKernelGGL(k_eml_step<9>, dim3(grid_for(T, BLOCK)), dim3(BLOCK), 0, c->stream, A, T);
    if (int rc = exclusive_scan(c, A.c_small, T, (u64*)(tb + o_cum), (u64*)(tb + o_cum) + T)) return rc;
    if (int rc = exclusive_scan(c, A.c_big, T, (u64*)(tb + o_cumb), (u64*)(tb + o_cumb) + T)) return rc;
    HIPC(hipMemcpyAsync(&nz_pin[0], (u64*)(tb + o_cum) + T, 8, hipMemcpyDeviceToHost, c->stream));
    HIPC(hipMemcpyAsync(&nz_pin[1], (u64*)(tb + o_cumb) + T, 8, hipMemcpyDeviceToHost, c->stream));
    HIPC(hipStreamSynchronize(c->stream));
    const u64 nz2[2] = {nz_pin[0], nz_pin[1]};
    cst = *cst_pin;
    NZ = nz2[0] + nz2[1];
    if (comp_out) *comp_out = cst;
    if (NZ == 0) return 1;
    A.target_big = A.target_nnz; A.target_nnz = std::max<u64>(1, target_small); A.cum_big = (const uint64_t*)(tb + o_cumb);
    A.ng_small = nz2[0] ? (u32)((nz2[0] - 1) / A.target_nnz + 1) : 0u;
    ng = A.ng_small + (nz2[1] ? (u32)((nz2[1] - 1) / A.target_big + 1) : 0u);
    P->n_small = A.ng_small;
  } else {
    if (int rc = exclusive_scan(c, A.c_nnz, T, (u64*)(tb + o_cum), (u64*)(tb + o_cum) + T)) return rc;
    HIPC(hipMemcpyAsync(&nz_pin[0], (u64*)(tb + o_cum) + T, 8, hipMemcpyDeviceToHost, c->stream));
    HIPC(hipStreamSynchronize(c->stream));
    NZ = nz_pin[0];
    cst = *cst_pin;
    if (comp_out) *comp_out = cst;
    if (NZ == 0) return 1;
    ng = (u32)((NZ - 1) / A.target_nnz + 1);
  }
  if (comp_out) *comp_out = cst;
  if ((u64)ng > ng_max) return kamd::fail(-105, "kamd_em_run: component-local EM: more groups than entries allow");
  A.n_groups = ng;
  HIPC(hipMemsetAsync(tb + o_gr, 0, t1.off - o_gr, c->stream));
  A.g_rows = (u32*)(tb + o_gr); A.g_tr = (u32*)(tb + o_gt); A.g_nnz = (u32*)(tb + o_gn); A.row_fill = (u32*)(tb + o_rf); A.tr_fill = (u32*)(tb + o_tf);
  hipLaunchKernelGGL(k_eml_step<2>, dim3(grid_for(T, BLOCK)), dim3(BLOCK), 0, c->stream, A, T);
  const size_t g_span = (o_gn - o_gr) + (size_t)ng * 4;
  if (int rc = plan_pin_ensure(c, g_span)) return rc;
  HIPC(hipMemcpyAsync(c->plan_pin, tb + o_gr, g_span, hipMemcpyDeviceToHost, c->stream));
  HIPC(hipStreamSynchronize(c->stream));
  const u32* const g_rows = (const u32*)c->plan_pin;
  const u32* const g_tr = (const u32*)((const char*)c->plan_pin + (o_gt - o_gr));
  const u32* const g_nnz = (const u32*)((const char*)c->plan_pin + (o_gn - o_gr));
  P->n_groups = ng; P->T = T; P->max_group_bytes = 0;
  P->row_base.assign(ng + 1, 0); P->tr_base.assign(ng + 1, 0); P->nz_base.assign(ng + 1, 0);
  for (u32 g = 0; g < ng; g++) {
    const u64 gb = L::group_bytes(g_nnz[g], g_rows[g], g_tr[g]);
    if (g_rows[g] > 65535 || g_tr[g] > 65535 || gb > budget) return 1;
    P->max_group_bytes = std::max<uint64_t>(P->max_group_bytes, gb);
    P->row_base[g + 1] = P->row_base[g] + g_rows[g]; P->tr_base[g + 1] = P->tr_base[g] + g_tr[g]; P->nz_base[g + 1] = P->nz_base[g] + g_nnz[g];
  }
  const u64 R = P->row_base[ng], M = P->tr_base[ng];
  if (P->nz_base[ng] != NZ) return kamd::fail(-105, "kamd_em_run: component-local EM: group sizes do not add up");
  Carver pv;
  const size_t p_rb = pv.take((ng + 1) * 4), p_tb = pv.take((ng + 1) * 4), p_zb = pv.take((ng + 1) * 8);
  const size_t p_rp = pv.take((R + ng) * 4 + 8), p_cp = pv.take((M + ng) * 4 + 8), p_rt = pv.take(NZ * 2 + 8), p_cr = pv.take(NZ * 2 + 8);
  const size_t p_cw = pv.take(R * 8 + 8), p_sg = pv.take(M * 8 + 8), p_ef = pv.take(M * 8 + 8), p_id = pv.take(M * 4 + 8);
  const size_t p_len = pv.take(R * 4 + 8), p_rabs = pv.take((R + 2) * 8), p_cc = pv.take(M * 4 + 8), p_cf = pv.take(M * 4 + 8), p_cabs = pv.take((M + 2) * 8);
  const size_t p_tt = pv.take(M * 4 + 8), p_rk = pv.take(R * 8 + 8), p_crt = pv.take(NZ * 2 + 8), p_ec = pv.take(NZ * 4 + 8), p_re = pv.take(R * 4 + 8), p_ref = pv.take(R * 4 + 8);
  if (int rc = c->pm_a.ensure(pv.off, 0, c->stream)) return rc;
  char* pb = (char*)c->pm_a.p;
  HIPC(hipMemcpyAsync(pb + p_rb, P->row_base.data(), (ng + 1) * 4, hipMemcpyHostToDevice, c->stream));
  HIPC(hipMemcpyAsync(pb + p_tb, P->tr_base.data(), (ng + 1) * 4, hipMemcpyHostToDevice, c->stream));
  HIPC(hipMemcpyAsync(pb + p_zb, P->nz_base.data(), (ng + 1) * 8, hipMemcpyHostToDevice, c->stream));
  HIPC(hipMemsetAsync(pb + p_cc, 0, p_cabs - p_cc, c->stream));
  A.row_base = (const u32*)(pb + p_rb); A.tr_base = (const u32*)(pb + p_tb); A.nz_base = (const uint64_t*)(pb + p_zb);
  A.row_ptr = (u32*)(pb + p_rp); A.col_ptr = (u32*)(pb + p_cp); A.row_tr = (uint16_t*)(pb + p_rt); A.col_row = (uint16_t*)(pb + p_cr);
  A.cw = (uint64_t*)(pb + p_cw); A.single = (double*)(pb + p_sg); A.eff_m = (double*)(pb + p_ef); A.tr_id = (u32*)(pb + p_id);
  A.len_new = (u32*)(pb + p_len); A.row_abs = (const uint64_t*)(pb + p_rabs); A.col_cnt = (u32*)(pb + p_cc); A.col_fill = (u32*)(pb + p_cf);
  A.col_abs = (const uint64_t*)(pb + p_cabs);
  A.tmp_tr_id = (u32*)(pb + p_tt); A.row_key = (uint64_t*)(pb + p_rk); A.col_row_tmp = (uint16_t*)(pb + p_crt); A.ent_col = (u32*)(pb + p_ec); A.row_e = (u32*)(pb + p_re); A.row_e_final = (u32*)(pb + p_ref);
  size_t rk_lds = 0;
  for (u32 g = 0; g < ng; g++) rk_lds = std::max(rk_lds, std::max((size_t)g_tr[g] * 4, (size_t)g_rows[g] * 12) + 16);
  const bool lds_rank = rk_lds <= 150 * 1024;
  hipLaunchKernelGGL(k_eml_step<3>, dim3(grid_for(T, BLOCK)), dim3(BLOCK), 0, c->stream, A, T);
  if (lds_rank) {
    HIPC(hipFuncSetAttribute((const void*)k_eml_rank_tr, hipFuncAttributeMaxDynamicSharedMemorySize, (int)rk_lds));
    HIPC(hipFuncSetAttribute((const void*)k_eml_rank_rows, hipFuncAttributeMaxDynamicSharedMemorySize, (int)rk_lds));
    hipLaunchKernelGGL(k_eml_rank_tr, dim3(ng), dim3(BLOCK), rk_lds, c->stream, A);
  } else hipLaunchKernelGGL(k_eml_step<10>, dim3(grid_for(M, BLOCK)), dim3(BLOCK), 0, c->stream, A, M);
  if (A.n_groups <= (u32)RG_BINS) hipLaunchKernelGGL(k_eml_rows_g, dim3(grid_for(n_ecs, RG_BLOCK * RG_PER)), dim3(RG_BLOCK), 0, c->stream, A);
  else hipLaunchKernelGGL(k_eml_step<4>, dim3(grid_for(n_ecs, BLOCK)), dim3(BLOCK), 0, c->stream, A, n_ecs);
  if (lds_rank) hipLaunchKernelGGL(k_eml_rank_rows, dim3(ng), dim3(EML_RANK_BLOCK), rk_lds, c->stream, A);
  else hipLaunchKernelGGL(k_eml_step<11>, dim3(grid_for(R, BLOCK)), dim3(BLOCK), 0, c->stream, A, R);
  size_t gb_lds = 0;
  for (u32 g = 0; g < ng; g++)
    gb_lds = std::max(gb_lds, ((size_t)g_rows[g] + 1 + 2 * (size_t)g_tr[g] + 1) * 4 + (((size_t)g_nnz[g] + 1) & ~(size_t)1) * 4 + 16);
  if (gb_lds <= 150 * 1024) {
    HIPC(hipFuncSetAttribute((const void*)k_eml_group_build, hipFuncAttributeMaxDynamicSharedMemorySize, (int)gb_lds));
    hipLaunchKernelGGL(k_eml_group_build, dim3(ng), dim3(BLOCK), gb_lds, c->stream, A);
  } else {
    if (int rc = exclusive_scan(c, A.len_new, R, (u64*)(pb + p_rabs), (u64*)(pb + p_rabs) + R)) return rc;
    hipLaunchKernelGGL(k_eml_step<5>, dim3(grid_for(n_ecs, BLOCK)), dim3(BLOCK), 0, c->stream, A, n_ecs);
    if (int rc = exclusive_scan(c, A.col_cnt, M, (u64*)(pb + p_cabs), (u64*)(pb + p_cabs) + M)) return rc;
    hipLaunchKernelGGL(k_eml_step<6>, dim3(grid_for(M, BLOCK)), dim3(BLOCK), 0, c->stream, A, M);
    hipLaunchKernelGGL(k_eml_step<7>, dim3(grid_for(ng, BLOCK)), dim3(BLOCK), 0, c->stream, A, (u64)ng);
    hipLaunchKernelGGL(k_eml_step<8>, dim3(grid_for(n_ecs, BLOCK)), dim3(BLOCK), 0, c->stream, A, n_ecs);
    hipLaunchKernelGGL(k_eml_step<12>, dim3(grid_for(NZ, BLOCK)), dim3(BLOCK), 0, c->stream, A, NZ);
  }
  HIPC(hipGetLastError());
  if (host_maps) {
    P->tr_id.resize(M); P->single_all.resize(T);
    if (M) HIPC(hipMemcpyAsync(P->tr_id.data(), A.tr_id, M * 4, hipMemcpyDeviceToHost, c->stream));
    HIPC(hipMemcpyAsync(P->single_all.data(), A.single_all, T * 8, hipMemcpyDeviceToHost, c->stream));
    HIPC(hipStreamSynchronize(c->stream));
  }
  *dev = EmLocalDev{(const u32*)(pb + p_rb), (const u32*)(pb + p_tb), (const u64*)(pb + p_zb), (const u32*)(pb + p_rp), (const u32*)(pb + p_cp),
                    (const uint16_t*)(pb + p_rt), (const uint16_t*)(pb + p_cr), (const u64*)(pb + p_cw), (const double*)(pb + p_sg),
                    (const double*)(pb + p_ef), (const u32*)(pb + p_id)};
  if (args_out) *args_out = A;
  return 0;
}
constexpr u32 SELL_NONE = 0xFFFFFFFFu;
__global__ void k_sell_maps(kamd_em_local::BuildArgs A, SellBuild B, u32* row_final, u32* mslot) {
  const u64 i = (u64)blockIdx.x * blockDim.x + threadIdx.x;
  if (i < A.n_ecs) {
    const u64 a = A.ec_off[i], b = A.ec_off[i + 1];
    u32 rf = SELL_NONE;
    if (b - a >= 2) {
      const u32 rn = A.row_new[i];
      const u32 g = sell_group_of(B.row_base, B.n_groups, rn);
      rf = B.row_base[g] + B.rnew[rn];
    }
    row_final[i] = rf;
  }
  if (i < A.T) {
    u32 ms = SELL_NONE;
    if (A.in_multi[i]) {
      const u32 g = kamd_em_local::eml_group_of(A, A.label[i]);
      const u32 old_m = B.tr_base[g] + A.local_of[i];
      ms = B.tr_base[g] + B.cnew[old_m];
    }
    mslot[i] = ms;
  }
}
__global__ void k_sell_refresh(const u64* __restrict__ ec_off, const u32* __restrict__ ec_ids, const u32* __restrict__ counts,
                               const u32* __restrict__ wcounts, u64 n_ecs, const double* __restrict__ eff, u64 T,
                               const u32* __restrict__ row_final, const u32* __restrict__ mslot, u64* cw, double* single_m,
                               double* eff_m, double* single_all) {
  const u64 i = (u64)blockIdx.x * blockDim.x + threadIdx.x;
  if (i < n_ecs) {
    const u64 a = ec_off[i], b = ec_off[i + 1];
    if (b - a == 1) {
      const u32 t = ec_ids[a];
      single_all[t] = (double)counts[i];
      if (mslot[t] != SELL_NONE) single_m[mslot[t]] = (double)counts[i];
    } else if (b - a >= 2) cw[row_final[i]] = (u64)counts[i] | ((u64)wcounts[i] << 32);
  }
  if (i < T && mslot[i] != SELL_NONE) eff_m[mslot[i]] = eff[i];
}

struct GiDesc { int* hist; int stopped; int pad; };
__global__ void k_gi_set_desc(GiDesc* d, EmsPrev prev, int* hist) {
// ... 505 lines not shown
  HIPC(hipMemsetD16Async((hipDeviceptr_t)stream, (unsigned short)GB_PAD, nzpad, c->stream));
  HIPC(hipMemcpyAsync(wg_desc, desc.data(), desc.size() * 4, hipMemcpyHostToDevice, c->stream));
  if (!items.empty()) HIPC(hipMemcpyAsync(wg_items, items.data(), items.size() * 4, hipMemcpyHostToDevice, c->stream));
  if (dir == 0) {
    hipLaunchKernelGGL(k_gb_scatter<true>, dim3(grid_for(n_seg * 8, BLOCK)), dim3(BLOCK), 0, c->stream, off, ids, n_seg, (const u32*)cnt, (const u64*)sub_off, (const u64*)blk_shift,
                       shift, fill, stream, (u32*)nullptr);
  } else {
    u32* info = end_slot;
    hipLaunchKernelGGL(k_gb_scatter<false>, dim3(grid_for(n_seg * 8, BLOCK)), dim3(BLOCK), 0, c->stream, off, ids, n_seg, (const u32*)cnt, (const u64*)sub_off, (const u64*)blk_shift,
                       shift, fill, stream, info);
    hipLaunchKernelGGL(k_gb_sort_small, dim3(grid_for(nzpad, BLOCK)), dim3(BLOCK), 0, c->stream, (const uint16_t*)stream, (const u32*)info, (const u32*)cnt, (const u64*)sub_off,
                       (const u64*)blk_shift, n_seg, nzpad, tmp);
    hipLaunchKernelGGL(k_gb_sort_big, dim3(grid_for(n_keys, BLOCK)), dim3(BLOCK), 0, c->stream, (const uint16_t*)stream, (const u32*)cnt, (const u64*)sub_off, (const u64*)blk_shift,
                       n_seg, n_keys, tmp);
    HIPC(hipMemcpyAsync(stream, tmp, nzpad * 2, hipMemcpyDeviceToDevice, c->stream));
  }
  hipLaunchKernelGGL(k_gb_piece_count, dim3(grid_for(n_keys, BLOCK)), dim3(BLOCK), 0, c->stream, (const u32*)cnt, (const u64*)sub_off, (const u64*)blk_shift, n_seg, (u32)n_blk, pc);
  HIPC(hipGetLastError());
  if (int rc = exclusive_scan(c, pc, n_keys, slot_scan, slot_scan + n_keys)) return rc;
  u64 n_pieces = 0;
  HIPC(hipMemcpyAsync(&n_pieces, slot_scan + n_keys, 8, hipMemcpyDeviceToHost, c->stream));
  HIPC(hipStreamSynchronize(c->stream));
  if (n_pieces == 0 || n_pieces >= 0x7FFFFFF0ULL) return 1;
  Carver vq;
  const size_t o_ps = vq.take((n_pieces + 64) * 4), o_part = vq.take(n_pieces * 8), o_slb = vq.take((n_seg + 2) * 4);
  if (int rc = pq.ensure(vq.off, 0, c->stream)) return rc;
  char* bq = (char*)pq.p;
  u32* piece_slot = (u32*)(bq + o_ps); double* part = (double*)(bq + o_part); u32* slot_base = (u32*)(bq + o_slb);
  hipLaunchKernelGGL(k_gb_piece_ends, dim3(grid_for(n_keys, BLOCK)), dim3(BLOCK), 0, c->stream, (const u32*)cnt, (const u64*)sub_off, (const u64*)blk_shift, n_seg, (u32)n_blk,
                     (const u64*)slot_scan, stream, end_slot);
  hipLaunchKernelGGL(k_gb_slot_base, dim3(grid_for(n_seg + 1, BLOCK)), dim3(BLOCK), 0, c->stream, (const u64*)slot_scan, n_seg, (u32)n_blk, n_pieces, slot_base);
  hipLaunchKernelGGL(k_gb_lanes, dim3(grid_for(n_chunks, BLOCK / 64)), dim3(BLOCK), 0, c->stream, (const uint16_t*)stream, (u32)n_chunks, lane_word, chunk_ends);
  HIPC(hipGetLastError());
  if (int rc = exclusive_scan(c, chunk_ends, n_chunks, seg_base64, seg_base64 + n_chunks)) return rc;
  hipLaunchKernelGGL(k_gb_piece_slot, dim3(grid_for(n_chunks, BLOCK / 64)), dim3(BLOCK), 0, c->stream, (const uint16_t*)stream, (const u32*)lane_word, (const u64*)seg_base64,
                     (u32)n_chunks, (const u32*)end_slot, piece_slot, seg_base);
  HIPC(hipMemsetAsync(part, 0, n_pieces * 8, c->stream));
  HIPC(hipMemsetAsync(piece_slot + n_pieces, 0, 64 * 4, c->stream));
  HIPC(hipGetLastError());
  out->stream = stream; out->seg_base = seg_base; out->lane_word = lane_word; out->piece_slot = piece_slot; out->part = part; out->slot_base = slot_base; out->wg_desc = wg_desc; out->wg_items = wg_items;
  out->n_wg = n_wg; out->n_chunks = (u32)n_chunks; out->n_pieces = (u32)n_pieces; out->n_seg = (u32)n_seg; out->n_tgt = (u32)n_tgt;
  return 0;
}
constexpr size_t GB_LDS_BYTES = (size_t)(GB_B + 1) * 8 + 8 + (size_t)GB_WAVES * GB_CH * 8;
int gb_setup(kamd_ctx* c, GiantPart& G) {
  G.gb.valid = false;
  const PmPlan& P = G.plan;
  const PmArgs& A = P.args;
  if (P.nzpad == 0 || A.R < 2 || A.M < 2) return 1;
  GbArgs ga{};
  if (int rc = gb_setup_side(c, P.roff, P.rs, A.R, A.M, 0, &ga.rows)) return rc;
  if (int rc = gb_setup_side(c, P.coff, P.cs, A.M, A.R, 1, &ga.cols)) return rc;
  ga.cw = A.cw; ga.single = A.single; ga.eff = A.eff; ga.R = A.R; ga.M = A.M;
  HIPC(hipFuncSetAttribute((const void*)k_gb_pass<0>, hipFuncAttributeMaxDynamicSharedMemorySize, (int)GB_LDS_BYTES));
  HIPC(hipFuncSetAttribute((const void*)k_gb_pass<1>, hipFuncAttributeMaxDynamicSharedMemorySize, (int)GB_LDS_BYTES));
  G.gb.args = ga; G.gb.valid = true;
  if (getenv("KAMD_DEBUG_FIN")) fprintf(stderr, "[kamd] blocked EM: R %u M %u nnz %llu; rows: %u chunks, %u pieces, %u workgroups; columns: %u chunks, %u pieces, %u workgroups\n", A.R, A.M,
                                        (unsigned long long)P.nzpad, ga.rows.n_chunks, ga.rows.n_pieces, ga.rows.n_wg, ga.cols.n_chunks, ga.cols.n_pieces, ga.cols.n_wg);
  return 0;
}
void gb_round(const GiantPart& G, hipStream_t s, int round, int clamp, const double* al_src, const double* a_src, double* al_dst, double* a_dst) {
  const GbArgs& A = G.gb.args;
  hipLaunchKernelGGL(k_gb_pass<0>, dim3(A.rows.n_wg), dim3(GB_THREADS), GB_LDS_BYTES, s, A, a_src, G.desc);
  hipLaunchKernelGGL(k_gb_pass<1>, dim3(A.cols.n_wg), dim3(GB_THREADS), GB_LDS_BYTES, s, A, a_src, G.desc);
  hipLaunchKernelGGL(k_gb_finish, dim3(grid_for(A.M, BLOCK)), dim3(BLOCK), 0, s, A, al_src, a_src, al_dst, a_dst, round, clamp, G.desc);
}
template <int K>
void gi_round(const GiantPart& G, hipStream_t s, int round, int clamp, const double* al_src, const double* a_src, double* al_dst, double* a_dst) {
  const PmPlan& P = G.plan;
  const unsigned grid = grid_for(P.n_chunks, PM_BLOCK / 64);
  constexpr int PRE_R = (K + 5) / 6 < 2 ? 2 : (K + 5) / 6;
  constexpr int PRE_C = K / 16 + 1;
  if (P.windowed) hipLaunchKernelGGL((k_gi_rows<K, PRE_R, true>), dim3(grid), dim3(PM_BLOCK), 0, s, P.args, a_src, G.desc);
  else hipLaunchKernelGGL((k_gi_rows<K, PRE_R, false>), dim3(grid), dim3(PM_BLOCK), 0, s, P.args, a_src, G.desc);
  if (P.n_fix[0]) hipLaunchKernelGGL(k_gi_rows_fix, dim3(grid_for(P.n_chunks, PM_BLOCK)), dim3(PM_BLOCK), 0, s, P.args, G.desc);
  if (P.windowed) hipLaunchKernelGGL((k_gi_cols<K, PRE_C, true>), dim3(grid), dim3(PM_BLOCK), 0, s, P.args, al_src, a_src, al_dst, a_dst, round, clamp, G.desc);
  else hipLaunchKernelGGL((k_gi_cols<K, PRE_C, false>), dim3(grid), dim3(PM_BLOCK), 0, s, P.args, al_src, a_src, al_dst, a_dst, round, clamp, G.desc);
  if (P.n_fix[1]) hipLaunchKernelGGL(k_gi_cols_fix, dim3(grid_for(P.n_chunks, PM_BLOCK)), dim3(PM_BLOCK), 0, s, P.args, al_src, a_src, al_dst, a_dst, round, clamp, G.desc);
}
void gi_enqueue_rounds(const GiantPart& G, hipStream_t s, int n, int clamp, int pin, int pout) {
  const u32 M = G.plan.args.M;
  for (int i = 0; i < n; i++) {
    const double* al_src = i == 0 ? G.G_al[pin] : G.S_al[(i - 1) & 1];
    const double* a_src = i == 0 ? G.G_a[pin] : G.S_a[(i - 1) & 1];
    double* al_dst = i == n - 1 ? G.G_al[pout] : G.S_al[i & 1];
    double* a_dst = i == n - 1 ? G.G_a[pout] : G.S_a[i & 1];
    if (clamp) {
      hipLaunchKernelGGL(k_gi_clamp, dim3(grid_for((u64)M + 1, BLOCK)), dim3(BLOCK), 0, s, al_src, a_src, G.ac, M, G.desc);
      a_src = G.ac;
    }
    if (G.gb.valid) { gb_round(G, s, i, clamp, al_src, a_src, al_dst, a_dst); continue; }
    switch (G.plan.k) {
      case 8: gi_round<8>(G, s, i, clamp, al_src, a_src, al_dst, a_dst); break;
      case 12: gi_round<12>(G, s, i, clamp, al_src, a_src, al_dst, a_dst); break;
      case 16: gi_round<16>(G, s, i, clamp, al_src, a_src, al_dst, a_dst); break;
      case 20: gi_round<20>(G, s, i, clamp, al_src, a_src, al_dst, a_dst); break;
      case 24: gi_round<24>(G, s, i, clamp, al_src, a_src, al_dst, a_dst); break;
      case 28: gi_round<28>(G, s, i, clamp, al_src, a_src, al_dst, a_dst); break;
      default: gi_round<32>(G, s, i, clamp, al_src, a_src, al_dst, a_dst); break;
    }
  }
}
int gi_launch_chunk(GiantPart& G, int n, int clamp, int pin, int pout, int* d_h, const EmsPrev& prev) {
  hipLaunchKernelGGL(k_gi_set_desc, dim3(1), dim3(64), 0, G.stream, G.desc, prev, d_h);
  if (G.use_graph && n == EML_MAX_ROUNDS && !clamp && pin != pout) {
    if (!G.gexec[pin]) {
      const bool inject = getenv("KAMD_DEBUG_GRAPH_FAIL") != nullptr;
      hipError_t e = hipStreamBeginCapture(G.stream, hipStreamCaptureModeThreadLocal);
// ... 101 lines not shown
    EmsPrev prev_w = prev;
    if (n_big) prev_w.host_hist = nullptr;
    if (P.n_small) hipLaunchKernelGGL(k_em_sell_wave, dim3((P.n_small + EMS_WAVE_TEAMS - 1) / EMS_WAVE_TEAMS), dim3(64 * EMS_WAVE_TEAMS), (size_t)EMS_WAVE_TEAMS * team_bytes,
                                      fork ? side : c->stream, dev, P.n_small, (u32)team_bytes, al_in, a_in, al_out, a_out, n, clamp, d_h, prev_w);
    if (hipGetLastError() != hipSuccess) return -104;
    if (fork && (hipEventRecord(ev_join, side) != hipSuccess || hipStreamWaitEvent(c->stream, ev_join, 0) != hipSuccess)) return -104;
    if (gi) {
      if (ss != c->stream && (hipEventRecord(ev_sell, ss) != hipSuccess || hipStreamWaitEvent(c->stream, ev_sell, 0) != hipSuccess)) return -104;
      if (hipStreamWaitEvent(c->stream, gi->ev, 0) != hipSuccess) return -104;
    }
    return 0;
  }
  void run(int n, int clamp, int* hist) {
    if (err || n <= 0) return;
    if (n > EML_MAX_ROUNDS) { err = -104; return; }
    if (hist && hipMemsetAsync(d_hist, 0, (size_t)n * sizeof(int), c->stream) != hipSuccess) { err = -104; return; }
    if (int rc = launch(n, clamp, d_alpha, d_a, d_alpha, d_a, hist ? d_hist : nullptr, EmsPrev{})) { err = rc; return; }
    if (hist && part) {
      if (hipStreamSynchronize(c->stream) != hipSuccess) { err = -104; return; }
      if (part->cb(part->user, (int32_t*)d_hist, n)) { err = -103; return; }
    }
    if (hist && (hipMemcpyAsync(hist, d_hist, (size_t)n * sizeof(int), hipMemcpyDeviceToHost, c->stream) != hipSuccess ||
                 hipStreamSynchronize(c->stream) != hipSuccess)) err = -104;
  }
  const std::vector<double>& host_alpha() {
    h_alpha.resize(M);
    if (gi && !err) {
      h_gi_prev.swap(h_gi_cur);
      h_gi_cur.resize(gi->plan.args.M);
      if (hipMemcpyAsync(h_gi_cur.data(), gi->G_al[0], (size_t)gi->plan.args.M * 8, hipMemcpyDeviceToHost, c->stream) != hipSuccess) err = -104;
    }
    ++host_reads;
    if (!err && ((M && hipMemcpyAsync(h_alpha.data(), d_alpha, M * 8, hipMemcpyDeviceToHost, c->stream) != hipSuccess) ||
                 hipStreamSynchronize(c->stream) != hipSuccess)) err = -104;
    return h_alpha;
  }
};
int EmSellGpu::setup(int hist_ints, const double* d_eff_new, u64 T_out) {
  Carver sv;
  const u64 Mp = M ? M : 1;
  const size_t o_al = sv.take(2 * Mp * 8 + 8), o_a = sv.take(2 * Mp * 8 + 8), o_h = sv.take((size_t)hist_ints * 4 + 8), o_out = sv.take(2 * T_out * 8 + 8);
  if (int rc = c->pm_b.ensure(sv.off, 0, c->stream)) return rc;
  char* sb = (char*)c->pm_b.p;
  d_alpha = (double*)(sb + o_al); d_a = (double*)(sb + o_a); d_ck_alpha = d_alpha + Mp; d_ck_a = d_a + Mp; d_hist = (int*)(sb + o_h); d_out = (double*)(sb + o_out);
  if (M) hipLaunchKernelGGL(k_eml_init, dim3(grid_for(M, BLOCK)), dim3(BLOCK), 0, c->stream, d_alpha, d_a, d_eff_new, M, 1.0 / (double)P.T);
  HIPC(hipGetLastError());
  lds = (size_t)P.max_group_bytes;
  reg_words = 0;
  {
    const int cap = std::min(64, std::max(1, c->tune.em_split_len));
    if (c->tune.em_reg_slices == 1) reg_words = cap <= 8 ? 2 : cap <= 16 ? 4 : cap <= 32 ? 8 : 0;
  }
  if (P.n_groups > P.n_small) {
    HIPC(hipFuncSetAttribute((const void*)k_em_sell<false, 0>, hipFuncAttributeMaxDynamicSharedMemorySize, (int)lds));
    HIPC(hipFuncSetAttribute((const void*)k_em_sell<true, 0>, hipFuncAttributeMaxDynamicSharedMemorySize, (int)lds));
    HIPC(hipFuncSetAttribute((const void*)k_em_sell<false, 0, 2>, hipFuncAttributeMaxDynamicSharedMemorySize, (int)lds));
    HIPC(hipFuncSetAttribute((const void*)k_em_sell<true, 0, 2>, hipFuncAttributeMaxDynamicSharedMemorySize, (int)lds));
    HIPC(hipFuncSetAttribute((const void*)k_em_sell<false, 0, 4, 2>, hipFuncAttributeMaxDynamicSharedMemorySize, (int)lds));
    HIPC(hipFuncSetAttribute((const void*)k_em_sell<true, 0, 4, 2>, hipFuncAttributeMaxDynamicSharedMemorySize, (int)lds));
    HIPC(hipFuncSetAttribute((const void*)k_em_sell<false, 0, 8>, hipFuncAttributeMaxDynamicSharedMemorySize, (int)lds));
    HIPC(hipFuncSetAttribute((const void*)k_em_sell<true, 0, 8>, hipFuncAttributeMaxDynamicSharedMemorySize, (int)lds));
  }
  if (gi && !c->em_ev_fork) {
    HIPC(hipEventCreateWithFlags(&c->em_ev_fork, hipEventDisableTiming));
    HIPC(hipEventCreateWithFlags(&c->em_ev_join, hipEventDisableTiming));
  }
  if (gi) ev_fork = c->em_ev_fork;
  if (P.n_small) {
    team_bytes = ((size_t)P.max_small_bytes + 15) & ~(size_t)15;
    HIPC(hipFuncSetAttribute((const void*)k_em_sell_wave, hipFuncAttributeMaxDynamicSharedMemorySize, (int)(EMS_WAVE_TEAMS * team_bytes)));
    if (!c->em_side_stream) {
      HIPC(hipStreamCreateWithFlags(&c->em_side_stream, hipStreamNonBlocking));
      if (!c->em_ev_fork) {
        HIPC(hipEventCreateWithFlags(&c->em_ev_fork, hipEventDisableTiming));
        HIPC(hipEventCreateWithFlags(&c->em_ev_join, hipEventDisableTiming));
      }
    }
    side = c->em_side_stream; ev_fork = c->em_ev_fork; ev_join = c->em_ev_join;
  }
  return 0;
}
__global__ void k_em_scatter(const u32* __restrict__ mslot, const double* __restrict__ single_all, const double* __restrict__ fin,
                             const double* __restrict__ before, u64 T, int have_final, double* out_alpha, double* out_abz) {
  const u64 t = (u64)blockIdx.x * blockDim.x + threadIdx.x;
  if (t >= T) return;
  const u32 ms = mslot[t];
  const double sa = single_all[t];
  out_alpha[t] = ms != 0xFFFFFFFFu ? fin[ms] : sa;
  out_abz[t] = have_final ? (ms != 0xFFFFFFFFu ? before[ms] : sa) : 0.0;
}
__global__ void k_em_publish(EmsPrev prev) {
  __shared__ int s_stop;
  (void)ems_prev_stopped(prev, &s_stop);
}
int em_sell_drive_async(kamd_ctx* c, EmSellGpu& B, const SellCache& K, u64 T, int n_iter, int min_rounds, double* alpha_out, double* abz_out, int* rounds_out) {
  const int CH = EML_MAX_ROUNDS;
  if (n_iter <= 0) {
    hipLaunchKernelGGL(k_em_scatter, dim3(grid_for(T, BLOCK)), dim3(BLOCK), 0, c->stream, K.mslot, K.single_all, B.d_alpha, B.d_alpha, T, 0, B.d_out, B.d_out + T);
    if (B.gi) hipLaunchKernelGGL(k_gi_scatter, dim3(grid_for(T, BLOCK)), dim3(BLOCK), 0, c->stream, T, B.gi->plan.mflag, B.gi->plan.mpos, B.gi->G_al[0], B.gi->G_al[0], 0,
                                 B.d_out, B.d_out + T);
    HIPC(hipGetLastError());
    std::vector<double> tmp(2 * T);
    HIPC(hipMemcpyAsync(tmp.data(), B.d_out, 2 * T * 8, hipMemcpyDeviceToHost, c->stream));
    HIPC(hipStreamSynchronize(c->stream));
    memcpy(alpha_out, tmp.data(), T * 8);
    if (abz_out) memcpy(abz_out, tmp.data() + T, T * 8);
    *rounds_out = 0;
    return 0;
  }
  const int n_chunks = std::max(1, (n_iter + CH - 1) / CH);
  const size_t hist_ints = (size_t)(n_chunks + 1) * CH;
  const size_t need = hist_ints * 4 + 256 + 2 * T * 8 + 256;
  if (c->em_pin_bytes < need) {
    if (c->em_pin) { HIPC(hipStreamSynchronize(c->stream)); HIPC(hipHostFree(c->em_pin)); c->em_pin = nullptr; c->em_pin_bytes = 0; }
    HIPC(hipHostMalloc(&c->em_pin, need, hipHostMallocMapped));
    c->em_pin_bytes = need;
  }
  int* h_hist = (int*)c->em_pin;
  int* h_seq = h_hist + hist_ints;
  double* h_out = (double*)((char*)c->em_pin + hist_ints * 4 + 256);
  void* dp = nullptr;
  HIPC(hipHostGetDevicePointer(&dp, c->em_pin, 0));
  int* d_hh = (int*)dp; int* d_seq = d_hh + hist_ints;
// ... 59 lines not shown
    if (int rc = B.launch(1, 1, al[(s + 1) & 1], av[(s + 1) & 1], al[s & 1], av[s & 1], nullptr, EmsPrev{})) return kamd::fail(rc, "kamd_em_run: final round failed to launch");
    before = al[(s + 1) & 1]; fin = al[s & 1];
    rounds = stop + 1;
  } else {
    fin = al[n_chunks & 1]; before = fin;
    rounds = n_iter;
  }
  hipLaunchKernelGGL(k_em_scatter, dim3(grid_for(T, BLOCK)), dim3(BLOCK), 0, c->stream, K.mslot, K.single_all, fin, before, T, have_final ? 1 : 0, B.d_out, B.d_out + T);
  if (B.gi) hipLaunchKernelGGL(k_gi_scatter, dim3(grid_for(T, BLOCK)), dim3(BLOCK), 0, c->stream, T, B.gi->plan.mflag, B.gi->plan.mpos, B.gi->G_al[B.gi_par(fin)],
                               B.gi->G_al[B.gi_par(before)], have_final ? 1 : 0, B.d_out, B.d_out + T);
  HIPC(hipGetLastError());
  HIPC(hipMemcpyAsync(h_out, B.d_out, 2 * T * 8, hipMemcpyDeviceToHost, c->stream));
  HIPC(hipStreamSynchronize(c->stream));
  memcpy(alpha_out, h_out, T * 8);
  if (abz_out) memcpy(abz_out, h_out + T, T * 8);
  if (d_clk) {
    std::vector<long long> hc(clk_words);
    HIPC(hipMemcpy(hc.data(), d_clk, clk_words * 8, hipMemcpyDeviceToHost));
    if (FILE* f = fopen(clk_path, "wb")) {
      const long long hdr[4] = {(long long)(B.P.n_groups - B.P.n_small), EMS_MAX_BLOCK / 64, EMS_CLK_WORDS, B.block};
      fwrite(hdr, 8, 4, f); fwrite(hc.data(), 8, clk_words, f); fclose(f);
    }
  }
  *rounds_out = rounds;
  return 0;
}
int em_sell_setup_device(kamd_ctx* c, const u64* d_ec_off, const u32* d_ec_ids, const u32* d_counts, const u32* d_wcounts, u64 n_ecs, u64 nnz,
                         const double* eff_lens, u64 T, u64 lds_budget, u64 target, kamd_em_sell::Plan* P, EmSellDev* dev, SellCache* cache,
                         u32 small_limit = 0, u64 target_small = 0, u64 small_budget = 0, bool host_maps = true, CompStats* comp_out = nullptr) {
  namespace S = kamd_em_sell;
  kamd_em_local::Plan C;
  EmLocalDev cd{};
  kamd_em_local::BuildArgs A{};
  if (int rc = em_local_setup_device(c, d_ec_off, d_ec_ids, d_counts, d_wcounts, n_ecs, nnz, eff_lens, T, ~0ULL, target, &C, &cd, &A, small_limit, target_small, host_maps, comp_out)) return rc;
  const u32 ng = C.n_groups;
  const u64 R = C.row_base[ng], M = C.tr_base[ng];
  if (R >= 0xFFFFFFF0ULL || M >= 0xFFFFFFF0ULL) return 1;
  for (u32 g = 0; g < ng; g++)
    if (C.row_base[g + 1] - C.row_base[g] >= S::SELL_PAD || C.tr_base[g + 1] - C.tr_base[g] >= S::SELL_PAD) return 1;
  Carver tv;
  const size_t o_rlen = tv.take(R * 4 + 8), o_clen = tv.take(M * 4 + 8), o_rnew = tv.take(R * 4 + 8), o_cnew = tv.take(M * 4 + 8);
  const size_t o_rlane = tv.take(R * 4 + 8), o_clane = tv.take(M * 4 + 8), o_rvl = tv.take(R * 4 + 8), o_cvl = tv.take(M * 4 + 8), o_gsz = tv.take((size_t)ng * 16 + 16);
  if (int rc = c->ems_tmp.ensure(tv.off, 0, c->stream)) return rc;
  char* tb = (char*)c->ems_tmp.p;
  SellBuild B{};
  B.row_base = cd.row_base; B.tr_base = cd.tr_base; B.row_ptr = cd.row_ptr; B.col_ptr = cd.col_ptr; B.row_tr = cd.row_tr; B.col_row = cd.col_row;
  B.nz_base = cd.nz_base; B.cw = cd.cw; B.single = cd.single; B.eff = cd.eff; B.tr_id = cd.tr_id; B.n_groups = ng; B.R = (u32)R; B.M = (u32)M;
  B.cap = (u32)std::min(64, std::max(1, c->tune.em_split_len));
  B.rlen = (u32*)(tb + o_rlen); B.clen = (u32*)(tb + o_clen); B.rnew = (u32*)(tb + o_rnew); B.cnew = (u32*)(tb + o_cnew);
  B.rlane = (u32*)(tb + o_rlane); B.clane = (u32*)(tb + o_clane); B.rvl = (u32*)(tb + o_rvl); B.cvl = (u32*)(tb + o_cvl); B.gsz = (u32*)(tb + o_gsz);
  const u64 nseg = std::max(R, M);
  hipLaunchKernelGGL(k_sell_lens, dim3(grid_for(nseg, BLOCK)), dim3(BLOCK), 0, c->stream, B);
  hipLaunchKernelGGL(k_sell_sizes, dim3(grid_for(2 * (u64)ng, SELL_BUILD_WAVES)), dim3(64 * SELL_BUILD_WAVES), 0, c->stream, B);
  if (int rc = plan_pin_ensure(c, (size_t)ng * 16)) return rc;
  const u32* const gsz = (const u32*)c->plan_pin;
  HIPC(hipMemcpyAsync(c->plan_pin, B.gsz, (size_t)ng * 16, hipMemcpyDeviceToHost, c->stream));
  HIPC(hipStreamSynchronize(c->stream));
  P->n_groups = ng; P->n_small = C.n_small; P->T = T; P->row_base = C.row_base; P->tr_base = C.tr_base; P->single_all = C.single_all;
  P->rslice_base.assign(ng + 1, 0); P->cslice_base.assign(ng + 1, 0); P->rell_base.assign(ng + 1, 0); P->cell_base.assign(ng + 1, 0);
  P->max_group_bytes = 0; P->max_small_bytes = 0;
  for (u32 g = 0; g < ng; g++) {
    const u64 gb = S::group_bytes(C.row_base[g + 1] - C.row_base[g], C.tr_base[g + 1] - C.tr_base[g], gsz[4 * g], gsz[4 * g + 2], gsz[4 * g + 1], gsz[4 * g + 3]);
    if (g < P->n_small) {
      if (gb > small_budget) return 2;
      P->max_small_bytes = std::max<uint64_t>(P->max_small_bytes, gb);
    } else {
      if (gb > lds_budget) return 1;
      P->max_group_bytes = std::max<uint64_t>(P->max_group_bytes, gb);
    }
    P->rslice_base[g + 1] = P->rslice_base[g] + gsz[4 * g]; P->rell_base[g + 1] = P->rell_base[g] + gsz[4 * g + 1];
    P->cslice_base[g + 1] = P->cslice_base[g] + gsz[4 * g + 2]; P->cell_base[g + 1] = P->cell_base[g] + gsz[4 * g + 3];
  }
  const u64 nrs = P->rslice_base[ng], ncs = P->cslice_base[ng], nru = P->rell_base[ng], ncu = P->cell_base[ng];
  Carver pv;
  const size_t p_rsb = pv.take((ng + 1) * 4), p_csb = pv.take((ng + 1) * 4), p_reb = pv.take((ng + 1) * 8), p_ceb = pv.take((ng + 1) * 8);
  const size_t p_rd = pv.take(nrs * 8 + 8), p_cdesc = pv.take(ncs * 8 + 8), p_re = pv.take(nru * 2 + 16), p_ce = pv.take(ncu * 2 + 16);
  const size_t p_cw = pv.take(R * 8 + 8), p_sg = pv.take(M * 8 + 8), p_ef = pv.take(M * 8 + 8), p_id = pv.take(M * 4 + 8);
  if (int rc = c->ems_plan.ensure(pv.off, 0, c->stream)) return rc;
  char* pb = (char*)c->ems_plan.p;
  HIPC(hipMemcpyAsync(pb + p_rsb, P->rslice_base.data(), (ng + 1) * 4, hipMemcpyHostToDevice, c->stream));
  HIPC(hipMemcpyAsync(pb + p_csb, P->cslice_base.data(), (ng + 1) * 4, hipMemcpyHostToDevice, c->stream));
  HIPC(hipMemcpyAsync(pb + p_reb, P->rell_base.data(), (ng + 1) * 8, hipMemcpyHostToDevice, c->stream));
  HIPC(hipMemcpyAsync(pb + p_ceb, P->cell_base.data(), (ng + 1) * 8, hipMemcpyHostToDevice, c->stream));
  HIPC(hipMemsetAsync(pb + p_re, 0xFF, nru * 2, c->stream));
  HIPC(hipMemsetAsync(pb + p_ce, 0xFF, ncu * 2, c->stream));
  B.rslice_base = (const u32*)(pb + p_rsb); B.cslice_base = (const u32*)(pb + p_csb); B.rell_base = (const u64*)(pb + p_reb); B.cell_base = (const u64*)(pb + p_ceb);
  B.rdesc = (u32*)(pb + p_rd); B.cdesc = (u32*)(pb + p_cdesc); B.rell = (uint16_t*)(pb + p_re); B.cell = (uint16_t*)(pb + p_ce);
  B.cw_new = (u64*)(pb + p_cw); B.single_new = (double*)(pb + p_sg); B.eff_new = (double*)(pb + p_ef); B.tr_id_new = (u32*)(pb + p_id);
  hipLaunchKernelGGL(k_sell_layout, dim3(grid_for(2 * (u64)ng, SELL_BUILD_WAVES)), dim3(64 * SELL_BUILD_WAVES), 0, c->stream, B);
  hipLaunchKernelGGL(k_sell_entries, dim3(grid_for(nseg, BLOCK)), dim3(BLOCK), 0, c->stream, B);
  HIPC(hipGetLastError());
  if (host_maps) {
    P->tr_id.resize(M);
    if (M) HIPC(hipMemcpyAsync(P->tr_id.data(), B.tr_id_new, M * 4, hipMemcpyDeviceToHost, c->stream));
  }
  Carver bv;
  const size_t b_rb = bv.take((ng + 1) * 4), b_tb = bv.take((ng + 1) * 4), b_rf = bv.take(n_ecs * 4 + 8), b_ms = bv.take(T * 4 + 8), b_sa = bv.take(T * 8 + 8),
               b_ef = bv.take(T * 8 + 8), b_gr = bv.take((size_t)ng * EMS_GREC_WORDS * 4 + 16);
  if (int rc = c->ems_maps.ensure(bv.off, 0, c->stream)) return rc;
  char* mb = (char*)c->ems_maps.p;
  HIPC(hipMemcpyAsync(mb + b_rb, cd.row_base, (ng + 1) * 4, hipMemcpyDeviceToDevice, c->stream));
  HIPC(hipMemcpyAsync(mb + b_tb, cd.tr_base, (ng + 1) * 4, hipMemcpyDeviceToDevice, c->stream));
  hipLaunchKernelGGL(k_sell_maps, dim3(grid_for(std::max<u64>(n_ecs, T), BLOCK)), dim3(BLOCK), 0, c->stream, A, B, (u32*)(mb + b_rf), (u32*)(mb + b_ms));
  HIPC(hipMemcpyAsync(mb + b_sa, A.single_all, T * 8, hipMemcpyDeviceToDevice, c->stream));
  *dev = EmSellDev{(const u32*)(mb + b_rb), (const u32*)(mb + b_tb), B.rslice_base, B.cslice_base, B.rell_base, B.cell_base, B.rdesc, B.cdesc, B.rell, B.cell,
                   B.cw_new, B.single_new, B.eff_new, (const u32*)(mb + b_gr)};
  hipLaunchKernelGGL(k_sell_group_rec, dim3(grid_for(ng, BLOCK)), dim3(BLOCK), 0, c->stream, *dev, ng, (u32*)(mb + b_gr));
  HIPC(hipGetLastError());
  HIPC(hipStreamSynchronize(c->stream));
  if (cache) { cache->row_final = (u32*)(mb + b_rf); cache->mslot = (u32*)(mb + b_ms); cache->single_all = (double*)(mb + b_sa); cache->d_eff = (double*)(mb + b_ef); }
  return 0;
}
}
namespace kamdi { void sell_cache_free(SellCache* k) { delete k; } }
namespace {
__global__ void k_hy_comp_nnz(const u64* __restrict__ ec_off, const u32* __restrict__ ec_ids, u64 n_ecs, const u32* __restrict__ label, u32* c_nnz) {
  const u64 e = (u64)blockIdx.x * blockDim.x + threadIdx.x;
  u32 root = 0xFFFFFFFFu, len = 0;
  if (e < n_ecs) {
    const u64 a = ec_off[e], b = ec_off[e + 1];
    if (b - a >= 2) { root = label[ec_ids[a]]; len = (u32)(b - a); }
  }
  const bool act = len != 0;
  const u64 am = __ballot(act);
  if (!am) return;
  const int leader = __ffsll((long long)am) - 1;
  const u32 lroot = (u32)__shfl((int)root, leader, 64);
  const bool with_leader = act && root == lroot;
  u32 v = with_leader ? len : 0u;
#pragma unroll
  for (int d = 32; d > 0; d >>= 1) v += (u32)__shfl_down((int)v, d, 64);
  if (lane_id() == 0 && v) atomicAdd(&c_nnz[lroot], v);
  if (act && !with_leader) atomicAdd(&c_nnz[root], len);
}
__global__ void k_hy_sizes(const u64* __restrict__ ec_off, const u32* __restrict__ ec_ids, u64 n_ecs, const u32* __restrict__ label,
                           const u32* __restrict__ c_nnz, u32 lim, u32* flag_s, u32* len_s, u32* flag_g, u32* len_g) {
  const u64 e = (u64)blockIdx.x * blockDim.x + threadIdx.x;
  if (e >= n_ecs) return;
  const u64 a = ec_off[e], b = ec_off[e + 1];
  const bool any = b > a;
  const bool giant = any && c_nnz[label[ec_ids[a]]] > lim;
  flag_s[e] = any && !giant ? 1u : 0u; len_s[e] = any && !giant ? (u32)(b - a) : 0u;
  flag_g[e] = giant ? 1u : 0u; len_g[e] = giant ? (u32)(b - a) : 0u;
}
__global__ void k_hy_single(const u64* __restrict__ ec_off, const u32* __restrict__ ec_ids, const u32* __restrict__ counts, u64 n_ecs, double* single_all) {
  const u64 e = (u64)blockIdx.x * blockDim.x + threadIdx.x;
  if (e >= n_ecs) return;
  const u64 a = ec_off[e];
  if (ec_off[e + 1] - a == 1) single_all[ec_ids[a]] = (double)counts[e];
}
int hy_streams(kamd_ctx* c) {
  if (!c->hy_giant_stream) {
    HIPC(hipStreamCreateWithFlags(&c->hy_giant_stream, hipStreamNonBlocking));
    HIPC(hipEventCreateWithFlags(&c->hy_ev_giant, hipEventDisableTiming));
    HIPC(hipEventCreateWithFlags(&c->hy_ev_sell, hipEventDisableTiming));
  }
  return 0;
}
int em_sell_plan_search(kamd_ctx* c, const u64* d_ec_off, const u32* d_ec_ids, const u32* d_counts, const u32* d_wcounts, u64 n_ecs, u64 nnz,
                        const double* eff_lens, u64 T, u64 lds_budget, int n_cus, bool multi, SellCache& K, CompStats* cst) {
  u32 small = c->tune.em_small_nnz > 0 ? (u32)c->tune.em_small_nnz : 0u;
  const bool auto_div = c->tune.em_group_div < 0;
// ... 660 lines not shown
```

### kallisto_amd/csrc/kamd_match.hip

```cpp
#include "kamd_dev.h"

namespace {

struct AlignOut {
  u32* dense_counts;
  u64* dense_first;
  u32* stream;
  u64* rec_off;
  u64* overflow_items;
  u64* explicit_items;
  u64* explicit_items_big;
  DevState* st;
};

template <bool PAIRED, bool FILTER>
__device__ __forceinline__ void emit_item(const DevIndex& ix, const FilterDev& fd, const AlignOut& out, const kamd::EcList& ecs,
                                          const kamd::MateInfo& m0, const kamd::MateInfo& m1, u64 item, bool active) {
  int kind = 0;
  if (active) {
    if (ecs.overflow) kind = 3;
    else if (kamd::pair_is_mapped(m0, m1)) kind = ecs.n == 1 ? 1 : 2;
  }
  if (FILTER && (kind == 1 || kind == 2)) {
    u32 kept = 0;
// ... 652 lines not shown
#pragma unroll
    for (int k = 0; k < FLD_RANK_BLOCK / 64; k++) { const u32 x = wsum[k]; total += x; if (k < wv) before += x; }
    const u32 carry = carry_s;
    if (i < n_blk) blk[i] = carry + before + incl - v;
    __syncthreads();
    if (tid == 0) carry_s = carry + total;
    __syncthreads();
  }
  if (tid == 0) head[2] = carry_s;
}
__global__ __launch_bounds__(FLD_RANK_BLOCK) void k_fld_emit(const int32_t* __restrict__ tl, const u32* __restrict__ card, u64 n, u32 want,
                                                            const u32* __restrict__ blk, int32_t* out) {
  __shared__ u32 wsum[FLD_RANK_BLOCK / 64];
  const u32 base = blk[blockIdx.x];
  if (base >= want) return;
  const int tid = (int)threadIdx.x, wv = tid >> 6, lane = tid & 63;
  int32_t t[FLD_RANK_PER];
  const u32 mine = fld_rank_load(tl, card, n, ((u64)blockIdx.x * FLD_RANK_BLOCK + threadIdx.x) * FLD_RANK_PER, t);
  const u32 incl = wave_incl_scan(mine);
  if (lane == 63) wsum[wv] = incl;
  __syncthreads();
  u32 before = 0;
#pragma unroll
  for (int k = 0; k < FLD_RANK_BLOCK / 64; k++) if (k < wv) before += wsum[k];
  u32 r = base + before + incl - mine;
#pragma unroll
  for (int j = 0; j < FLD_RANK_PER; j++) if (t[j] > 0) { if (r < want) out[r] = t[j]; ++r; }
}

}

namespace {
__global__ void k_mark_overflow(u32* raw, int raw_stride, u64 n_items) {
  const u64 i = (u64)blockIdx.x * blockDim.x + threadIdx.x;
  if (i < n_items) raw[i * (u64)raw_stride] = RAW_OVERFLOW;
}
template <bool PAIRED, bool FILTER>
int launch_match_chunk(kamd_ctx* c, hipStream_t s, const u32* d_words, const uint16_t* d_len, u64 first, u64 n, int seq_words, int rec_words, u32* slots,
                       int stride) {
  constexpr int WAVES = BLOCK / 64;
  constexpr int NM = PAIRED ? 2 : 1;
  const int lane_words = seq_words * NM;
  size_t lds_bytes = ((size_t)WAVES * 64 * lane_words + (size_t)BLOCK * V3_LIST_CAP) * sizeof(u32);
  if (c->tune.lds_pad > 0 && lds_bytes <= 64 * 1024) lds_bytes = std::min<size_t>(64 * 1024, lds_bytes + (size_t)c->tune.lds_pad);
  const u64 n_waves = (n + c->items_per_wave - 1) / c->items_per_wave;
  const u32* w = d_words + first * (u64)(rec_words * NM);
  const uint16_t* l = d_len + first * NM;
  u32* raw = slots + first * (u64)stride;
  if (lds_bytes > 64 * 1024) {
    hipLaunchKernelGGL(k_mark_overflow, dim3(grid_for(n, BLOCK)), dim3(BLOCK), 0, s, raw, stride, n);
  } else {
#define KAMD_LAUNCH_V3L(DLV, TXT, LAY)                                                                                                   \
  do {                                                                                                                                  \
    HIPC(hipFuncSetAttribute((const void*)k_match_v3<PAIRED, FILTER, DLV, TXT, LAY>, hipFuncAttributeMaxDynamicSharedMemorySize, (int)lds_bytes)); \
    hipLaunchKernelGGL((k_match_v3<PAIRED, FILTER, DLV, TXT, LAY>), dim3(grid_for(n_waves, WAVES)), dim3(BLOCK), lds_bytes, s, c->ix, w, l, n, seq_words, \
                       rec_words, c->items_per_wave, c->refill_min, raw, stride, c->stats_a.as<DevStatsA>());                           \
  } while (0)
#define KAMD_LAUNCH_V3(DLV, TXT)                                                                                                         \
  do { if (c->ix.table_layout == kamd::LAYOUT_COMPACT) KAMD_LAUNCH_V3L(DLV, TXT, kamd::LAYOUT_COMPACT); else KAMD_LAUNCH_V3L(DLV, TXT, kamd::LAYOUT_WIDE); } while (0)
    const bool dl = c->ix.n_dbuckets != 0, txt = c->tune.text_verify == 1;
    if (dl) { if (txt) KAMD_LAUNCH_V3(true, true); else KAMD_LAUNCH_V3(true, false); }
    else { if (txt) KAMD_LAUNCH_V3(false, true); else KAMD_LAUNCH_V3(false, false); }
#undef KAMD_LAUNCH_V3
#undef KAMD_LAUNCH_V3L
  }
  HIPC(hipGetLastError());
  return 0;
}
struct WorkStream {
  kamd_ctx* c; hipStream_t user; bool swapped = false;
  explicit WorkStream(kamd_ctx* ctx) : c(ctx), user(ctx->stream) {}
  int fork() {
    if (!c->al_stream) {
      HIPC(hipStreamCreateWithFlags(&c->al_stream, hipStreamNonBlocking));
      HIPC(hipEventCreateWithFlags(&c->al_ev_in, hipEventDisableTiming));
      HIPC(hipEventCreateWithFlags(&c->al_ev_out, hipEventDisableTiming));
    }
    HIPC(hipEventRecord(c->al_ev_in, user));
    HIPC(hipStreamWaitEvent(c->al_stream, c->al_ev_in, 0));
    c->stream = c->al_stream; swapped = true;
    return 0;
  }
  ~WorkStream() {
    if (!swapped) return;
    (void)hipEventRecord(c->al_ev_out, c->al_stream);
    (void)hipStreamWaitEvent(user, c->al_ev_out, 0);
    c->stream = user;
  }
};
int fld_launch(kamd_ctx* c, const FilterDev& fd, const u32* w, const uint16_t* l, u64 n, int seq_words, int rec_words, hipStream_t s);
template <bool PAIRED, bool FILTER>
int overflow_side_launch(kamd_ctx* c, const u32* d_words, const uint16_t* d_len, u64 nov, int seq_words, int rec_words, const FilterDev& fd, AlignOut& out);
template <bool PAIRED, bool FILTER>
int align_batch(kamd_ctx* c, WorkStream& ws, const u32* d_words, const uint16_t* d_len, u64 n_items, int seq_words, int rec_words, const FilterDev& fd,
                AlignOut& out, u64 key_base) {
  const int stride = 2 + V3_LIST_CAP + (FILTER ? 4 : 0);
  if (int rc = c->stream_buf.ensure(n_items * (u64)stride * sizeof(u32), 0, c->stream)) return rc;
  if (int rc = c->rec_off.ensure(n_items * sizeof(u64), 0, c->stream)) return rc;
  out.stream = c->stream_buf.as<u32>(); out.rec_off = c->rec_off.as<u64>();
  c->host_state.stream_words = n_items * (u64)stride;
  c->host_state.n_recs = n_items;
  if (int rc = push_state(c)) return rc;
  u32* slots = c->stream_buf.as<u32>();
  int chunks = c->tune.align_chunks > 0 ? c->tune.align_chunks : 1;
  chunks = (int)std::min<u64>((u64)std::min(chunks, 64), std::max<u64>(1, n_items / 65536));
  const u64 per = (n_items + chunks - 1) / chunks;
  if (chunks > 1) {
// ... 21 lines not shown
    c->fld_pending.strand = q.strand; c->fld_pending.so = q.so; c->fld_pending.valid = true;
  }
  c->last_classify_ms = 0.f;
  for (int k = 0; k < chunks; k++) {
    const u64 first = (u64)k * per, n = std::min(per, n_items - first);
    if (chunks > 1) HIPC(hipStreamWaitEvent(c->stream, c->al_ev_chunk[k], 0));
    HIPC(hipEventRecord(c->ev2, c->stream));
    const unsigned grid = (unsigned)std::min<u64>(grid_for(n, BLOCK), (u64)std::max(1, c->n_cus) * 4);
    hipLaunchKernelGGL((k_classify<PAIRED, FILTER, V3_LIST_CAP>), dim3(grid), dim3(BLOCK), 0, c->stream, c->ix, slots + first * (u64)stride, stride, n,
                       first * (u64)stride, first, key_base + first, first, fd, out);
    HIPC(hipGetLastError());
    HIPC(hipEventRecord(c->ev3, c->stream));
    if (int rc = sync_state(c)) return rc;
    float ms = 0.f;
    HIPC(hipEventElapsedTime(&ms, c->ev2, c->ev3));
    c->last_classify_ms += ms;
    if (chunks == 1 && c->host_state.n_overflow && c->tune.overflow_second_pass == 1 && !FILTER && !c->ix.union_mode) {
      const int sr = overflow_side_launch<PAIRED, FILTER>(c, d_words, d_len, c->host_state.n_overflow, seq_words, rec_words, fd, out);
      if (sr < 0) return sr;
    }
    if (int rc = absorb_tuples(c, c->stream_buf.as<u32>(), c->rec_off.as<u64>() + first, n, c->host_state.stream_words, key_base + first,
                               c->host_state.st_multi - c->multi_before, nullptr, (u32)stride, first)) return rc;
    c->multi_before = c->host_state.st_multi;
  }
  HIPC(hipEventSynchronize(c->ev1));
  HIPC(hipEventElapsedTime(&c->last_align_ms, c->ev0, c->ev1));
  return 0;
}
template <bool PAIRED, bool FILTER>
void launch_overflow(kamd_ctx* c, const u32* d_words, const uint16_t* d_len, u64 nov, int seq_words, int rec_words, const FilterDev& fd,
                     u64 rec_base, const AlignOut& out, const u64* items = nullptr) {
  hipLaunchKernelGGL((k_pseudoalign_overflow<PAIRED, FILTER>), dim3(grid_for(nov, 64)), dim3(64), 0, c->stream, c->ix, d_words, d_len,
                     items ? items : (const u64*)c->overflow_items.as<u64>(), nov, seq_words, rec_words, c->overflow_scratch.as<u32>(), fd, rec_base, out);
}
template <bool PAIRED, bool FILTER>
int overflow_second_pass(kamd_ctx* c, hipStream_t s, bool side, const u32* d_words, const uint16_t* d_len, u64 nov, int seq_words, int rec_words, const FilterDev& fd,
                         const AlignOut& out) {
  constexpr int WAVES = BLOCK / 64;
  constexpr int NM = PAIRED ? 2 : 1;
  constexpr int LC = V3_LIST_CAP_LONG;
  const int lane_words = seq_words * NM;
  const size_t lds_bytes = (size_t)WAVES * 64 * lane_words * sizeof(u32);
  if (lds_bytes > 96 * 1024) return 1;
  const int stride2 = 2 + LC + (FILTER ? 4 : 0);
  if (int rc = c->raw2.ensure(nov * (u64)stride2 * sizeof(u32), 0, c->stream)) return rc;
  if (int rc = c->overflow_left.ensure(nov * sizeof(u64), 0, c->stream)) return rc;
  if (int rc = c->stats_b.ensure(sizeof(DevStatsA), 0, c->stream)) return rc;
  HIPC(hipMemsetAsync(c->stats_b.p, 0, sizeof(DevStatsA), s));
  const int ipw = (int)std::min<u64>(1024, std::max<u64>(64, nov / ((u64)std::max(1, c->n_cus) * 32)));
  const u64 n_waves = (nov + (u64)ipw - 1) / (u64)ipw;
  u32* raw2 = c->raw2.as<u32>();
#define KAMD_LAUNCH_V3L2(DLV, TXT, LAY)                                                                                                  \
  do {                                                                                                                                  \
    HIPC(hipFuncSetAttribute((const void*)k_match_v3<PAIRED, FILTER, DLV, TXT, LAY, LC, true>, hipFuncAttributeMaxDynamicSharedMemorySize, (int)lds_bytes)); \
    hipLaunchKernelGGL((k_match_v3<PAIRED, FILTER, DLV, TXT, LAY, LC, true>), dim3(grid_for(n_waves, WAVES)), dim3(BLOCK), lds_bytes, s, c->ix, d_words, d_len, nov, \
                       seq_words, rec_words, ipw, std::min(c->refill_min, 8), raw2, stride2, c->stats_b.as<DevStatsA>(), (const u64*)c->overflow_items.as<u64>()); \
  } while (0)
#define KAMD_LAUNCH_V32(DLV, TXT)                                                                                                        \
  do { if (c->ix.table_layout == kamd::LAYOUT_COMPACT) KAMD_LAUNCH_V3L2(DLV, TXT, kamd::LAYOUT_COMPACT); else KAMD_LAUNCH_V3L2(DLV, TXT, kamd::LAYOUT_WIDE); } while (0)
  const bool dl = c->ix.n_dbuckets != 0, txt = c->tune.text_verify == 1;
  if (dl) { if (txt) KAMD_LAUNCH_V32(true, true); else KAMD_LAUNCH_V32(true, false); }
  else { if (txt) KAMD_LAUNCH_V32(false, true); else KAMD_LAUNCH_V32(false, false); }
#undef KAMD_LAUNCH_V32
#undef KAMD_LAUNCH_V3L2
  if (!side) {
    c->host_state.n_overflow = 0;
    if (int rc = push_state(c)) return rc;
  }
  hipLaunchKernelGGL((k_classify_long<PAIRED, FILTER, LC>), dim3(grid_for(nov, CL_WAVES * CL_ITEMS)), dim3(64 * CL_WAVES), 0, s, c->ix, (const u32*)raw2, stride2,
                     (const u64*)c->overflow_items.as<u64>(), nov, c->overflow_scratch.as<u32>(), fd, 0ULL, out, c->overflow_left.as<u64>());
  HIPC(hipGetLastError());
  return side ? 0 : sync_state(c);
}
template <bool PAIRED, bool FILTER>
int overflow_side_launch(kamd_ctx* c, const u32* d_words, const uint16_t* d_len, u64 nov, int seq_words, int rec_words, const FilterDev& fd, AlignOut& out) {
  if ((size_t)(BLOCK / 64) * 64 * seq_words * (PAIRED ? 2 : 1) * sizeof(u32) > 96 * 1024) return 1;
  if (!c->ov_stream) {
    HIPC(hipStreamCreateWithFlags(&c->ov_stream, hipStreamNonBlocking));
    HIPC(hipEventCreateWithFlags(&c->ov_ev_in, hipEventDisableTiming)); HIPC(hipEventCreateWithFlags(&c->ov_ev_done, hipEventDisableTiming));
    HIPC(hipEventCreate(&c->ov_ev_t0)); HIPC(hipEventCreate(&c->ov_ev_t1));
    HIPC(hipHostMalloc((void**)&c->ov_pin, 2 * sizeof(DevState), hipHostMallocDefault));
  }
  const u64 w = c->host_state.stream_words, r = c->host_state.n_recs;
  if (int rc = c->stream_buf.ensure((w + nov * (TUPLE_CAP_BIG + 2)) * sizeof(u32), w * sizeof(u32), c->stream)) return rc;
  if (int rc = c->rec_off.ensure((r + nov) * sizeof(u64), r * sizeof(u64), c->stream)) return rc;
  if (int rc = c->ov_state.ensure(sizeof(DevState), 0, c->stream)) return rc;
  out.stream = c->stream_buf.as<u32>(); out.rec_off = c->rec_off.as<u64>();
  memset(&c->ov_pin[0], 0, sizeof(DevState));
  c->ov_pin[0].stream_words = w;
  HIPC(hipMemcpyAsync(c->ov_state.p, &c->ov_pin[0], sizeof(DevState), hipMemcpyHostToDevice, c->stream));
  HIPC(hipEventRecord(c->ov_ev_in, c->stream));
  HIPC(hipStreamWaitEvent(c->ov_stream, c->ov_ev_in, 0));
  AlignOut out2 = out;
  out2.st = (DevState*)c->ov_state.p;
  HIPC(hipEventRecord(c->ov_ev_t0, c->ov_stream));
  const int sp = overflow_second_pass<PAIRED, FILTER>(c, c->ov_stream, true, d_words, d_len, nov, seq_words, rec_words, fd, out2);
  if (sp != 0) return sp;
  HIPC(hipEventRecord(c->ov_ev_t1, c->ov_stream));
  HIPC(hipMemcpyAsync(&c->ov_pin[1], c->ov_state.p, sizeof(DevState), hipMemcpyDeviceToHost, c->ov_stream));
  HIPC(hipEventRecord(c->ov_ev_done, c->ov_stream));
  c->ov_side_pending = true;
  return 0;
}
int overflow_side_join(kamd_ctx* c, u64 nov, u64* n_again) {
  HIPC(hipEventSynchronize(c->ov_ev_done));
  c->ov_side_pending = false;
  const DevState& e = c->ov_pin[1];
// ... 268 lines not shown
```

Measured before the change: 1171.

## Fuse tuple bound computation into store, cache LDS attributes, batch plan uploads

Tuple slot bounds and route flags are now computed inside k_tup_store, which handles several tuples per thread, and a lighter k_bound_lists builds the big and shade index lists from those stored values, so the separate bounding pass no longer rereads each tuple. Repeated hipFuncSetAttribute calls go through a mutex-protected cache that skips the call when the requested dynamic LDS size is already set. The four small plan uploads are packed into one pinned staging image and sent with a single copy, and the effective-length host work is handed to the finalize routine as a callback instead of running on a spawned thread. Optional host timestamps are added behind an environment variable; the costs are register pressure from the multi-item loops and a static cache that must stay valid.

```diff
diff --git a/kallisto_amd/csrc/kamd_ctx.hip b/kallisto_amd/csrc/kamd_ctx.hip
--- a/kallisto_amd/csrc/kamd_ctx.hip
+++ b/kallisto_amd/csrc/kamd_ctx.hip
@@ -86,6 +86,18 @@
 }
 int push_state(kamd_ctx* c) {
   HIPC(hipMemcpyAsync(c->state.p, &c->host_state, sizeof(DevState), hipMemcpyHostToDevice, c->stream));
+  return 0;
+}
+int max_dynamic_lds(int device, const void* fn, size_t bytes) {
+  struct Seen { int device; const void* fn; size_t bytes; };
+  static std::mutex mu;
+  static std::vector<Seen> seen;
+  std::lock_guard<std::mutex> lock(mu);
+  Seen* s = nullptr;
+  for (Seen& e : seen) if (e.device == device && e.fn == fn) { s = &e; break; }
+  if (s && s->bytes >= bytes) return 0;
+  HIPC(hipFuncSetAttribute(fn, hipFuncAttributeMaxDynamicSharedMemorySize, (int)bytes));
+  if (s) s->bytes = bytes; else seen.push_back(Seen{device, fn, bytes});
   return 0;
 }
 }
@@ -175,7 +187,7 @@
   if (c->sell_cache) sell_cache_free(c->sell_cache);
   for (void* p : c->index_allocs) (void)hipFree(p);
   for (DBuf* b : {&c->dense, &c->stream_buf, &c->rec_off, &c->overflow_items, &c->overflow_scratch, &c->state, &c->rec_slot,
-                  &c->retry, &c->ttable, &c->tstore, &c->stats_a, &c->list, &c->cand, &c->cand_off, &c->cand_slot, &c->ctable, &c->tup_bound, &c->tup_off, &c->tup_big, &c->raw2, &c->overflow_left, &c->stats_b, &c->clist, &c->sizes, &c->explicit_items,
+                  &c->retry, &c->ttable, &c->tstore, &c->stats_a, &c->list, &c->cand, &c->cand_off, &c->cand_slot, &c->ctable, &c->tup_bound, &c->tup_route, &c->tup_off, &c->tup_big, &c->raw2, &c->overflow_left, &c->stats_b, &c->clist, &c->sizes, &c->explicit_items,
                   &c->explicit_items_big, &c->exp_stream, &c->exp_off, &c->exp_scratch, &c->bs_cp, &c->bs_samp, &c->raw, &c->dense_first, &c->exp_key, &c->cand_key, &c->ec_first, &c->pm_a, &c->pm_b, &c->pm_rank, &c->eml_tmp, &c->ems_tmp, &c->ems_plan, &c->ems_maps, &c->fld_tl, &c->fld_card, &c->fld_scratch, &c->fld_items, &c->fld_cand,
                   &c->block_sums, &c->ec_off, &c->ec_ids, &c->ec_counts, &c->em_alpha, &c->em_next, &c->em_eff,
                   &c->em_state, &c->em_cn, &c->em_colcnt, &c->em_coloff, &c->em_colrow,
@@ -716,19 +728,26 @@
     }
     if (int rc = kamd_ec_allreduce(c, comm)) return rc;
   }
-  std::vector<double> mft(KAMD_MAX_FRAG_LEN);
-  std::thread eff_thread([&] {
-    if (o->fld == 0.0) kamd_mean_frag_lens_trunc(out->flens, mft.data());
-    else kamd_trunc_gaussian_fld(0, KAMD_MAX_FRAG_LEN, o->fld, o->sd, mft.data());
-    kamd_eff_lens(target_lens, n_targets, mft.data(), out->eff_lens);
-  });
-  const int fin_rc = kamd_ec_finalize(c, nullptr);
-  eff_thread.join();
+  struct EffWork { const kamd_quant_opts* o; const int32_t* target_lens; uint64_t n_targets; kamd_quant_out* out; bool done; } ew{o, target_lens, n_targets, out, false};
+  auto eff_fn = [](void* p) {
+    EffWork& w = *(EffWork*)p;
+    std::vector<double> mft(KAMD_MAX_FRAG_LEN);
+    if (w.o->fld == 0.0) kamd_mean_frag_lens_trunc(w.out->flens, mft.data());
+    else kamd_trunc_gaussian_fld(0, KAMD_MAX_FRAG_LEN, w.o->fld, w.o->sd, mft.data());
+    kamd_eff_lens(w.target_lens, w.n_targets, mft.data(), w.out->eff_lens);
+    w.done = true;
+  };
+  HostStamps hs("kamd_quant_batches");
+  const int fin_rc = kamdi::ec_finalize_impl(c, nullptr, eff_fn, &ew);
+  hs.mark("finalize");
+  if (!ew.done) eff_fn(&ew);
   if (fin_rc) return fin_rc;
   int32_t rounds = 0;
   if (multi) { if (int rc = kamd_em_run_comm(c, comm, out->eff_lens, n_targets, 10000, 50, out->est_counts, out->alpha_before_zeroes, &rounds)) return rc; }
   else if (int rc = kamd_em_run(c, nullptr, nullptr, nullptr, nullptr, 0, out->eff_lens, n_targets, 10000, 50, out->est_counts, out->alpha_before_zeroes, &rounds)) return rc;
+  hs.mark("em");
   if (out->tpm) kamd_counts_to_tpm(out->est_counts, out->eff_lens, n_targets, out->tpm);
+  hs.mark("tpm");
   out->n_processed = n_proc; out->em_rounds = rounds;
   return 0;
 }
diff --git a/kallisto_amd/csrc/kamd_dev.h b/kallisto_amd/csrc/kamd_dev.h
--- a/kallisto_amd/csrc/kamd_dev.h
+++ b/kallisto_amd/csrc/kamd_dev.h
@@ -5,7 +5,10 @@
 #include <dlfcn.h>
 
 #include <algorithm>
+#include <cstdio>
+#include <cstdlib>
 #include <cstring>
+#include <mutex>
 #include <string>
 #include <chrono>
 #include <thread>
@@ -256,6 +259,7 @@
   u64 recs_total = 0;
   u64 multi_before = 0;
   u64 n_distinct_tuples = 0;
+  DBuf tup_route; bool tup_bound_valid = true; int tup_bound_union = -1;
   float last_absorb_ms = 0.f; hipEvent_t ev_ab0 = nullptr, ev_ab1 = nullptr;
   kamd_ec_result result{};
   bool finalized = false;
@@ -313,6 +317,20 @@
 int tuples_clear(kamd_ctx* c);
 int absorb_tuples(kamd_ctx* c, const u32* batch, const u64* rec_off, u64 n, u64 batch_words, u64 key_base, u64 n_tuple_bound,
                   const u64* first_idx = nullptr, u32 fixed_stride = 0, u64 item0 = 0);
+int ec_finalize_impl(kamd_ctx* c, kamd_ec_result* out, void (*fn)(void*), void* user);
+int max_dynamic_lds(int device, const void* fn, size_t bytes);
+struct HostStamps {
+  const char* who; bool on; int n = 0;
+  std::chrono::steady_clock::time_point t[24]; const char* what[24];
+  explicit HostStamps(const char* w) : who(w), on(getenv("KAMD_DEBUG_FIN") != nullptr) { mark("enter"); }
+  void mark(const char* w) { if (on && n < 24) { t[n] = std::chrono::steady_clock::now(); what[n++] = w; } }
+  ~HostStamps() {
+    if (!on || n < 2) return;
+    std::string s = std::string("[kamd] host us ") + who + ":";
+    for (int i = 1; i < n; i++) s += std::string(" ") + what[i] + " +" + std::to_string(std::chrono::duration_cast<std::chrono::microseconds>(t[i] - t[i - 1]).count());
+    fprintf(stderr, "%s\n", s.c_str());
+  }
+};
 template <class T>
 int upload(kamd_ctx* c, const T* host, size_t n, const T** dev) {
   void* p = nullptr;
diff --git a/kallisto_amd/csrc/kamd_ec.hip b/kallisto_amd/csrc/kamd_ec.hip
--- a/kallisto_amd/csrc/kamd_ec.hip
+++ b/kallisto_amd/csrc/kamd_ec.hip
@@ -228,25 +228,101 @@
 #pragma unroll
   for (int q = 0; q < ABS_Q; q++) if (is_owner[q]) list[blk_base + my[q]] = own_s[q];
 }
-__global__ __launch_bounds__(BLOCK) void k_tup_store(const u32* __restrict__ batch, u32* store, TSlot* table, u64* list, u64 first_new,
-                                                     u64 n_new, DevState* st) {
+constexpr u64 SHADE_SMALL = 64;
+constexpr u64 SHADE_SLOT_FACTOR = 4;
+constexpr u32 RES_BIG_MIN = 16;
+constexpr uint8_t ROUTE_BIG = 1, ROUTE_HUGE = 2, ROUTE_SH_SMALL = 4, ROUTE_SH_LONG = 8;
+__device__ __forceinline__ u64 slot_bound_from(const DevIndex& ix, u64 core_b, u64 S, uint8_t* route) {
+  const u64 b = core_b + (ix.union_mode ? S : SHADE_SLOT_FACTOR * S) + 2;
+  const bool sh_small = !ix.union_mode && S != 0 && core_b + S <= SHADE_SMALL;
+  const bool sh_long = !ix.union_mode && S != 0 && !sh_small;
+  const bool big = !ix.union_mode && core_b > RES_BIG_MIN;
+  const bool huge = big && core_b > 1024;
+  *route = (uint8_t)((big && !huge ? ROUTE_BIG : 0) | (huge ? ROUTE_HUGE : 0) | (sh_small ? ROUTE_SH_SMALL : 0) | (sh_long ? ROUTE_SH_LONG : 0));
+  return b;
+}
+__device__ __forceinline__ u64 tuple_slot_bound(const DevIndex& ix, const u32* es, u32 m, uint8_t* route) {
+  if (ix.n_shades) {
+    const kamd::ShadeTables sh = shade_tables(ix);
+    const kamd::SetTables core{sh.core_off, sh.core_ids};
+    const u64 core_b = kamd::set_size_bound(core, es, (int)m, ix.union_mode != 0);
+    return slot_bound_from(ix, core_b, kamd::shaded_size_bound(sh, es, (int)m, ix.union_mode != 0) - core_b, route);
+  }
+  const kamd::SetTables stt{(const uint64_t*)ix.ec_off, ix.ec_ids};
+  return slot_bound_from(ix, kamd::set_size_bound(stt, es, (int)m, ix.union_mode != 0), 0, route);
+}
+constexpr int TS_Q_MAIN = 4, TS_W = 6;
+constexpr u64 TS_MAIN_MIN = 1ULL << 18;
+template <int TS_Q>
+__global__ __launch_bounds__(BLOCK) void k_tup_store(DevIndex ix, const u32* __restrict__ batch, u32* store, TSlot* table, u64* list, u64 first_new,
+                                                     u64 n_new, DevState* st, u32* tup_bound, uint8_t* tup_route) {
   __shared__ u32 wsum[BLOCK / 64]; __shared__ u64 blk_base;
-  const u64 i = (u64)blockIdx.x * blockDim.x + threadIdx.x;
-  u64 s = 0, off = 0; u32 need = 0;
-  if (i < n_new) { s = list[first_new + i] & 0xFFFFFFFFULL; off = table[s].owner; need = batch[off + 1] + 2u; }
-  const u32 incl = wave_incl_scan(need);
+  const u64 T = (u64)gridDim.x * blockDim.x;
+  const u64 t = (u64)blockIdx.x * blockDim.x + threadIdx.x;
+  u64 s[TS_Q], off[TS_Q]; u32 need[TS_Q], w[TS_Q][TS_W]; bool live[TS_Q];
+#pragma unroll
+  for (int q = 0; q < TS_Q; q++) {
+    const u64 i = t + (u64)q * T;
+    live[q] = i < n_new;
+    s[q] = live[q] ? (list[first_new + i] & 0xFFFFFFFFULL) : 0ULL;
+  }
+#pragma unroll
+  for (int q = 0; q < TS_Q; q++) off[q] = live[q] ? table[s[q]].owner : 0ULL;
+#pragma unroll
+  for (int q = 0; q < TS_Q; q++) {
+    w[q][0] = live[q] ? batch[off[q]] : 0u; w[q][1] = live[q] ? batch[off[q] + 1] : 0u;
+    need[q] = live[q] ? w[q][1] + 2u : 0u;
+  }
+#pragma unroll
+  for (int q = 0; q < TS_Q; q++)
+#pragma unroll
+    for (int j = 2; j < TS_W; j++) w[q][j] = (u32)j < need[q] ? batch[off[q] + j] : 0u;
+  u32 sz[TS_Q][TS_W - 2]; bool fast[TS_Q];
+#pragma unroll
+  for (int q = 0; q < TS_Q; q++) {
+    fast[q] = live[q] && !ix.n_shades && need[q] <= (u32)TS_W;
+#pragma unroll
+    for (int j = 0; j < TS_W - 2; j++) {
+      sz[q][j] = 0;
+      if (fast[q] && (u32)j + 2u < need[q]) { const u32 x = w[q][2 + j] & kamd::EC_ID_MASK; sz[q][j] = (u32)(ix.ec_off[x + 1] - ix.ec_off[x]); }
+    }
+  }
+  u64 tag[TS_Q];
+#pragma unroll
+  for (int q = 0; q < TS_Q; q++) tag[q] = live[q] ? table[s[q]].tag : 0ULL;
+  u32 total = 0;
+#pragma unroll
+  for (int q = 0; q < TS_Q; q++) total += need[q];
+  const u32 incl = wave_incl_scan(total);
   if (lane_id() == 63) wsum[threadIdx.x >> 6] = incl;
   __syncthreads();
-  if (threadIdx.x == 0) { u32 t = 0; for (int j = 0; j < BLOCK / 64; j++) t += wsum[j]; blk_base = t ? atomicAdd(&st->ts_words, (u64)t) : 0ULL; }
-  __syncthreads();
-  if (i >= n_new) return;
+  if (threadIdx.x == 0) { u32 a = 0; for (int j = 0; j < BLOCK / 64; j++) a += wsum[j]; blk_base = a ? atomicAdd(&st->ts_words, (u64)a) : 0ULL; }
+  __syncthreads();
   u32 before = 0;
   for (u32 j = 0; j < (threadIdx.x >> 6); j++) before += wsum[j];
-  const u64 dst = blk_base + before + incl - need;
-  for (u32 j = 0; j < need; j++) store[dst + j] = batch[off + j];
-  table[s].owner = dst;
-  table[s].tag = (table[s].tag & 0xFFFFFFFF00000000ULL) | (dst + 1);
-  list[first_new + i] = s | (dst << 32);
+  u64 dst = blk_base + before + incl - total;
+#pragma unroll
+  for (int q = 0; q < TS_Q; q++) {
+    if (!live[q]) continue;
+    const u64 i = t + (u64)q * T;
+#pragma unroll
+    for (int j = 0; j < TS_W; j++) if ((u32)j < need[q]) store[dst + j] = w[q][j];
+    for (u32 j = TS_W; j < need[q]; j++) store[dst + j] = batch[off[q] + j];
+    table[s[q]].owner = dst;
+    table[s[q]].tag = (tag[q] & 0xFFFFFFFF00000000ULL) | (dst + 1);
+    list[first_new + i] = s[q] | (dst << 32);
+    uint8_t route; u64 b;
+    if (fast[q]) {
+      const u32 m = need[q] - 2u;
+      u64 mn = ~0ULL, sum = 0;
+#pragma unroll
+      for (int j = 0; j < TS_W - 2; j++) if ((u32)j < m) { sum += sz[q][j]; if (sz[q][j] < mn) mn = sz[q][j]; }
+      b = slot_bound_from(ix, ix.union_mode ? sum : (m ? mn : 0ULL), 0, &route);
+    } else b = tuple_slot_bound(ix, batch + off[q] + 2, need[q] - 2u, &route);
+    tup_bound[first_new + i] = (u32)b;
+    tup_route[first_new + i] = route;
+    dst += need[q];
+  }
 }
 __global__ void k_tup_rehash(const u32* __restrict__ store, const TSlot* __restrict__ old, TSlot* nu, u64 mask, u64* list, u64 n) {
   const u64 i = (u64)blockIdx.x * blockDim.x + threadIdx.x;
@@ -261,84 +337,122 @@
   list[i] = s | (o.owner << 32);
 }
 
-constexpr u64 SHADE_SMALL = 64;
-constexpr u64 SHADE_SLOT_FACTOR = 4;
-constexpr u32 RES_BIG_MIN = 16;
-__global__ void k_bound_tuples(DevIndex ix, const u32* __restrict__ stream, const TSlot* table, const u64* list, u64 n,
-                               u32* per_tuple, u32* big_idx, u32* shade_idx, DevState* st) {
-  u64 i = (u64)blockIdx.x * blockDim.x + threadIdx.x;
+constexpr int BL_PER = 4;
+__device__ __forceinline__ void bound_lists(u64 i0, u64 n, u64 b, const uint8_t* r, u32* big_idx, u32* shade_idx, DevState* st) {
+  __shared__ u32 s_cnt[4][BLOCK / 64]; __shared__ u64 s_base[4]; __shared__ u64 s_sum[BLOCK / 64];
+  const int wv = threadIdx.x >> 6;
+  u32 c[4] = {0, 0, 0, 0};
+#pragma unroll
+  for (int q = 0; q < BL_PER; q++) {
+    c[0] += (r[q] & ROUTE_BIG) ? 1u : 0u; c[1] += (r[q] & ROUTE_HUGE) ? 1u : 0u;
+    c[2] += (r[q] & ROUTE_SH_SMALL) ? 1u : 0u; c[3] += (r[q] & ROUTE_SH_LONG) ? 1u : 0u;
+  }
+  u32 incl[4];
+#pragma unroll
+  for (int l = 0; l < 4; l++) { incl[l] = wave_incl_scan(c[l]); if (lane_id() == 63) s_cnt[l][wv] = incl[l]; }
+  b = wave_sum64(b);
+  if (lane_id() == 0) s_sum[wv] = b;
+  __syncthreads();
+  if (threadIdx.x < 4) {
+    u32 t = 0;
+    for (int j = 0; j < BLOCK / 64; j++) t += s_cnt[threadIdx.x][j];
+    u64* cur = threadIdx.x == 0 ? &st->n_big : threadIdx.x == 1 ? &st->n_huge : threadIdx.x == 2 ? &st->n_sh_small : &st->n_sh_long;
+    s_base[threadIdx.x] = t ? atomicAdd(cur, (u64)t) : 0ULL;
+  } else if (threadIdx.x == 4) {
+    u64 t = 0;
+    for (int j = 0; j < BLOCK / 64; j++) t += s_sum[j];
+    if (t) atomicAdd(&st->bound_words, t);
+  }
+  __syncthreads();
+  u64 pos[4];
+#pragma unroll
+  for (int l = 0; l < 4; l++) {
+    u32 before = 0;
+    for (int j = 0; j < wv; j++) before += s_cnt[l][j];
+    pos[l] = s_base[l] + before + incl[l] - c[l];
+  }
+#pragma unroll
+  for (int q = 0; q < BL_PER; q++) {
+    const u32 i = (u32)(i0 + q);
+    if (r[q] & ROUTE_BIG) big_idx[pos[0]++] = i;
+    if (r[q] & ROUTE_HUGE) big_idx[n - 1 - pos[1]++] = i;
+    if (r[q] & ROUTE_SH_SMALL) shade_idx[pos[2]++] = i;
+    if (r[q] & ROUTE_SH_LONG) shade_idx[n - 1 - pos[3]++] = i;
+  }
+}
+__global__ __launch_bounds__(BLOCK) void k_bound_tuples(DevIndex ix, const u32* __restrict__ stream, const TSlot* table, const u64* list, u64 n,
+                                                        u32* per_tuple, u32* big_idx, u32* shade_idx, DevState* st) {
+  const u64 i0 = ((u64)blockIdx.x * BLOCK + threadIdx.x) * BL_PER;
+  u64 b = 0, off[BL_PER]; uint8_t r[BL_PER];
+#pragma unroll
+  for (int q = 0; q < BL_PER; q++) off[q] = i0 + q < n ? list[i0 + q] >> 32 : 0ULL;
+#pragma unroll
+  for (int q = 0; q < BL_PER; q++) {
+    r[q] = 0;
+    if (i0 + q < n) {
+      const u64 bq = tuple_slot_bound(ix, stream + off[q] + 2, stream[off[q] + 1], &r[q]);
+      per_tuple[i0 + q] = (u32)bq;
+      b += bq;
+    }
+  }
+  bound_lists(i0, n, b, r, big_idx, shade_idx, st);
+}
+__global__ __launch_bounds__(BLOCK) void k_bound_lists(const u32* __restrict__ tup_bound, const uint8_t* __restrict__ tup_route, u64 n, u32* big_idx, u32* shade_idx,
+                                                       DevState* st) {
+  const u64 i0 = ((u64)blockIdx.x * BLOCK + threadIdx.x) * BL_PER;
+  u64 b = 0; uint8_t r[BL_PER];
+#pragma unroll
+  for (int q = 0; q < BL_PER; q++) {
+    r[q] = 0;
+    if (i0 + q < n) { b += tup_bound[i0 + q]; r[q] = tup_route[i0 + q]; }
+  }
+  bound_lists(i0, n, b, r, big_idx, shade_idx, st);
+}
+constexpr int BS_PER = 4;
+__global__ __launch_bounds__(BLOCK) void k_bound_singles(DevIndex ix, const u32* __restrict__ dense, DevState* st) {
+  __shared__ u64 s_sum[BLOCK / 64];
   u64 b = 0;
-  bool big = false, huge = false, sh_small = false, sh_long = false;
-  if (i < n) {
-    const u64 off = list[i] >> 32;
-    const u32 m = stream[off + 1];
-    u64 core_b;
-    if (ix.n_shades) {
-      const kamd::ShadeTables sh = shade_tables(ix);
-      const kamd::SetTables core{sh.core_off, sh.core_ids};
-      core_b = kamd::set_size_bound(core, stream + off + 2, (int)m, ix.union_mode != 0);
-      const u64 S = kamd::shaded_size_bound(sh, stream + off + 2, (int)m, ix.union_mode != 0) - core_b;
-      b = core_b + (ix.union_mode ? S : SHADE_SLOT_FACTOR * S) + 2;
-      sh_small = !ix.union_mode && S != 0 && core_b + S <= SHADE_SMALL;
-      sh_long = !ix.union_mode && S != 0 && !sh_small;
-    } else {
-      const kamd::SetTables stt{(const uint64_t*)ix.ec_off, ix.ec_ids};
-      core_b = kamd::set_size_bound(stt, stream + off + 2, (int)m, ix.union_mode != 0);
-      b = core_b + 2;
-    }
-    per_tuple[i] = (u32)b;
-    big = big_idx && !ix.union_mode && core_b > RES_BIG_MIN;
-    huge = big && core_b > 1024;
+#pragma unroll
+  for (int q = 0; q < BS_PER; q++) {
+    const u64 e = ((u64)blockIdx.x * BS_PER + q) * BLOCK + threadIdx.x;
+    if (e < ix.n_ecs && dense[e]) b += ix.ec_off[e + 1] - ix.ec_off[e] + 2;
   }
   b = wave_sum64(b);
-  if (lane_id() == 0 && b) atomicAdd(&st->bound_words, b);
-  const u64 bm = __ballot(big && !huge), hm = __ballot(huge);
-  if (bm) {
-    u64 base = 0;
-    if (lane_id() == 0) base = atomicAdd(&st->n_big, (u64)__popcll(bm));
-    base = shfl_u64(base, 0);
-    if (big && !huge) big_idx[base + __popcll(bm & ((1ULL << lane_id()) - 1ULL))] = (u32)i;
-  }
-  if (hm) {
-    u64 base = 0;
-    if (lane_id() == 0) base = atomicAdd(&st->n_huge, (u64)__popcll(hm));
-    base = shfl_u64(base, 0);
-    if (huge) big_idx[n - 1 - (base + __popcll(hm & ((1ULL << lane_id()) - 1ULL)))] = (u32)i;
-  }
-  const u64 sm = __ballot(sh_small), lm = __ballot(sh_long);
-  if (sm) {
-    u64 base = 0;
-    if (lane_id() == 0) base = atomicAdd(&st->n_sh_small, (u64)__popcll(sm));
-    base = shfl_u64(base, 0);
-    if (sh_small) shade_idx[base + __popcll(sm & ((1ULL << lane_id()) - 1ULL))] = (u32)i;
-  }
-  if (lm) {
-    u64 base = 0;
-    if (lane_id() == 0) base = atomicAdd(&st->n_sh_long, (u64)__popcll(lm));
-    base = shfl_u64(base, 0);
-    if (sh_long) shade_idx[n - 1 - (base + __popcll(lm & ((1ULL << lane_id()) - 1ULL)))] = (u32)i;
-  }
-}
-__global__ void k_bound_singles(DevIndex ix, const u32* __restrict__ dense, DevState* st) {
-  u64 e = (u64)blockIdx.x * blockDim.x + threadIdx.x;
-  u64 b = 0;
-  if (e < ix.n_ecs && dense[e]) b = ix.ec_off[e + 1] - ix.ec_off[e] + 2;
-  b = wave_sum64(b);
-  if (lane_id() == 0 && b) atomicAdd(&st->bound_words, b);
-}
-__global__ void k_cand_singles(DevIndex ix, const u32* __restrict__ dense, const u64* __restrict__ dense_first, u32* cand,
-                               u64* cand_off, u64* cand_key, DevState* st) {
+  if (lane_id() == 0) s_sum[threadIdx.x >> 6] = b;
+  __syncthreads();
+  if (threadIdx.x == 0) {
+    u64 t = 0;
+    for (int j = 0; j < BLOCK / 64; j++) t += s_sum[j];
+    if (t) atomicAdd(&st->bound_words, t);
+  }
+}
+__global__ __launch_bounds__(BLOCK) void k_cand_singles(DevIndex ix, const u32* __restrict__ dense, const u64* __restrict__ dense_first, u32* cand,
+                                                        u64* cand_off, u64* cand_key, DevState* st) {
+  __shared__ u32 s_w[BLOCK / 64], s_r[BLOCK / 64]; __shared__ u64 s_bw, s_br;
   u64 e = (u64)blockIdx.x * blockDim.x + threadIdx.x;
   const bool have = e < ix.n_ecs && dense[e] != 0;
   const u32* ids = nullptr; u32 n = 0;
   if (have) { ids = ix.ec_ids + ix.ec_off[e]; n = (u32)(ix.ec_off[e + 1] - ix.ec_off[e]); }
   const bool longset = n > 64;
+  u32 keep = 0;
+  if (have && !longset) for (u32 j = 0; j < n; j++) keep += onlisted(ix.onlist_bits, ids[j]);
+  const u32 need = keep ? keep + 2u : 0u, one = keep ? 1u : 0u;
+  const u32 iw = wave_incl_scan(need), ir = wave_incl_scan(one);
+  if (lane_id() == 63) { s_w[threadIdx.x >> 6] = iw; s_r[threadIdx.x >> 6] = ir; }
+  __syncthreads();
+  if (threadIdx.x == 0) {
+    u32 tw = 0, tr = 0;
+    for (int j = 0; j < BLOCK / 64; j++) { tw += s_w[j]; tr += s_r[j]; }
+    s_bw = tw ? atomicAdd(&st->cand_words, (u64)tw) : 0ULL;
+    s_br = tr ? atomicAdd(&st->cand_recs, (u64)tr) : 0ULL;
+  }
+  __syncthreads();
   if (have && !longset) {
-    u32 keep = 0;
-    for (u32 j = 0; j < n; j++) keep += onlisted(ix.onlist_bits, ids[j]);
     if (keep) {
-      u64 off = atomicAdd(&st->cand_words, (u64)keep + 2);
-      u64 r = atomicAdd(&st->cand_recs, 1ULL);
+      u32 bw = 0, br = 0;
+      for (u32 j = 0; j < (threadIdx.x >> 6); j++) { bw += s_w[j]; br += s_r[j]; }
+      const u64 off = s_bw + bw + iw - need;
+      const u64 r = s_br + br + ir - one;
       u32* w = cand + off;
       w[0] = dense[e]; w[1] = keep;
       u32 o = 0;
@@ -954,6 +1068,7 @@
   }
   c->host_state.tl_n = 0; c->host_state.ts_words = 0; c->host_state.tl_fail = 0;
   c->n_distinct_tuples = 0;
+  c->tup_bound_valid = true; c->tup_bound_union = -1;
   return 0;
 }
 int tuples_resize(kamd_ctx* c, u64 cap) {
@@ -988,6 +1103,10 @@
     if (int rc = tuples_resize(c, pow2_at_least(4 * c->host_state.tl_n + 16))) return rc;
   }
   if (int rc = c->list.ensure((c->host_state.tl_n + bound + 1) * sizeof(u64), c->host_state.tl_n * sizeof(u64), c->stream)) return rc;
+  if (int rc = c->tup_bound.ensure((c->host_state.tl_n + bound + 1) * sizeof(u32), c->tup_bound_valid ? c->host_state.tl_n * sizeof(u32) : 0, c->stream)) return rc;
+  if (int rc = c->tup_route.ensure(c->host_state.tl_n + bound + 1, c->tup_bound_valid ? c->host_state.tl_n : 0, c->stream)) return rc;
+  if (c->tup_bound_union < 0) c->tup_bound_union = c->ix.union_mode;
+  else if (c->tup_bound_union != c->ix.union_mode) c->tup_bound_valid = false;
   if (int rc = c->retry.ensure(2 * (bound + 1) * sizeof(u64), 0, c->stream)) return rc;
   u64* fail_a = c->retry.as<u64>();
   u64* fail_b = fail_a + bound + 1;
@@ -1013,8 +1132,12 @@
     if (n_new) {
       if (c->host_state.ts_words + new_words >= 0x7FFFFFF0ULL) return kamd::fail(-101, "absorb_tuples: more than 2^31 words of distinct tuples");
       if (int rc = c->tstore.ensure((c->host_state.ts_words + new_words + 2) * sizeof(u32), c->host_state.ts_words * sizeof(u32), c->stream)) return rc;
-      hipLaunchKernelGGL(k_tup_store, dim3(grid_for(n_new, BLOCK)), dim3(BLOCK), 0, c->stream, batch, c->tstore.as<u32>(), c->ttable.as<TSlot>(),
-                         c->list.as<u64>(), tl_before, n_new, dst);
+      if (n_new >= TS_MAIN_MIN)
+        hipLaunchKernelGGL(k_tup_store<TS_Q_MAIN>, dim3(grid_for((n_new + TS_Q_MAIN - 1) / TS_Q_MAIN, BLOCK)), dim3(BLOCK), 0, c->stream, c->ix, batch, c->tstore.as<u32>(),
+                           c->ttable.as<TSlot>(), c->list.as<u64>(), tl_before, n_new, dst, c->tup_bound.as<u32>(), c->tup_route.as<uint8_t>());
+      else
+        hipLaunchKernelGGL(k_tup_store<1>, dim3(grid_for(n_new, BLOCK)), dim3(BLOCK), 0, c->stream, c->ix, batch, c->tstore.as<u32>(),
+                           c->ttable.as<TSlot>(), c->list.as<u64>(), tl_before, n_new, dst, c->tup_bound.as<u32>(), c->tup_route.as<uint8_t>());
       HIPC(hipGetLastError());
       c->host_state.ts_words += new_words;
     }
@@ -1115,10 +1238,13 @@
   return 0;
 }
 
-extern "C" int kamd_ec_finalize(kamd_ctx* c, kamd_ec_result* out) {
+extern "C" int kamd_ec_finalize(kamd_ctx* c, kamd_ec_result* out) { return kamdi::ec_finalize_impl(c, out, nullptr, nullptr); }
+
+int kamdi::ec_finalize_impl(kamd_ctx* c, kamd_ec_result* out, void (*fn)(void*), void* user) {
   if (!c) return kamd::fail(-1, "kamd_ec_finalize: null context");
   if (!c->has_index) return kamd::fail(-1, "kamd_ec_finalize: no index uploaded");
   HIPC(hipSetDevice(c->device));
+  HostStamps hs("kamd_ec_finalize");
   if (!c->ev_fin0) { HIPC(hipEventCreate(&c->ev_fin0)); HIPC(hipEventCreate(&c->ev_fin1)); }
   HIPC(hipEventRecord(c->ev_fin0, c->stream));
   if (int rc = sync_state(c)) return rc;
@@ -1127,19 +1253,27 @@
   c->host_state.bound_words = 0; c->host_state.cand_words = 0; c->host_state.cand_recs = 0; c->host_state.n_big = 0; c->host_state.n_huge = 0;
   c->host_state.n_sh_small = 0; c->host_state.n_sh_long = 0; c->host_state.shade_err = 0;
   if (int rc = push_state(c)) return rc;
-  hipLaunchKernelGGL(k_bound_singles, dim3(grid_for(c->n_ecs, BLOCK)), dim3(BLOCK), 0, c->stream, c->ix, c->dense.as<u32>(), dst);
-  if (int rc = c->tup_bound.ensure((n_t + 1) * sizeof(u32), 0, c->stream)) return rc;
+  hipLaunchKernelGGL(k_bound_singles, dim3(grid_for(c->n_ecs, BLOCK * BS_PER)), dim3(BLOCK), 0, c->stream, c->ix, c->dense.as<u32>(), dst);
+  const bool kept = c->tup_bound_valid && (n_t == 0 || c->tup_bound_union == c->ix.union_mode);
+  if (!kept) if (int rc = c->tup_bound.ensure((n_t + 1) * sizeof(u32), 0, c->stream)) return rc;
   if (int rc = c->tup_off.ensure((n_t + 2) * sizeof(u64), 0, c->stream)) return rc;
   if (int rc = c->tup_big.ensure(2 * (n_t + 1) * sizeof(u32), 0, c->stream)) return rc;
   if (n_t) {
-    hipLaunchKernelGGL(k_bound_tuples, dim3(grid_for(n_t, BLOCK)), dim3(BLOCK), 0, c->stream, c->ix, c->tstore.as<u32>(),
-                       c->ttable.as<TSlot>(), c->list.as<u64>(), n_t, c->tup_bound.as<u32>(), c->tup_big.as<u32>(), c->tup_big.as<u32>() + (n_t + 1), dst);
+    if (kept) hipLaunchKernelGGL(k_bound_lists, dim3(grid_for(n_t, BLOCK * BL_PER)), dim3(BLOCK), 0, c->stream, (const u32*)c->tup_bound.as<u32>(), (const uint8_t*)c->tup_route.as<uint8_t>(),
+                                 n_t, c->tup_big.as<u32>(), c->tup_big.as<u32>() + (n_t + 1), dst);
+    else {
+      c->tup_bound_valid = false;
+      hipLaunchKernelGGL(k_bound_tuples, dim3(grid_for(n_t, BLOCK * BL_PER)), dim3(BLOCK), 0, c->stream, c->ix, c->tstore.as<u32>(),
+                         c->ttable.as<TSlot>(), c->list.as<u64>(), n_t, c->tup_bound.as<u32>(), c->tup_big.as<u32>(), c->tup_big.as<u32>() + (n_t + 1), dst);
+    }
     if (int rc = exclusive_scan(c, c->tup_bound.as<u32>(), n_t, c->tup_off.as<u64>(), c->tup_off.as<u64>() + n_t)) return rc;
   }
   HIPC(hipGetLastError());
   u64 tup_words = 0;
   if (n_t) HIPC(hipMemcpyAsync(&tup_words, c->tup_off.as<u64>() + n_t, sizeof(u64), hipMemcpyDeviceToHost, c->stream));
+  hs.mark("bounds queued");
   if (int rc = sync_state(c)) return rc;
+  hs.mark("bounds read");
   const u64 n_exp_w = c->exp_words_done, n_exp_r = c->host_state.exp_recs;
   const u64 bound = c->host_state.bound_words + n_exp_w;
   const u64 max_cands = c->n_ecs + n_t + n_exp_r;
@@ -1176,11 +1310,16 @@
       if (n_l) hipLaunchKernelGGL(k_shade_extend<64>, dim3(grid_for(n_l * 64, BLOCK)), dim3(BLOCK), 0, c->stream, c->ix, c->tstore.as<u32>(), c->list.as<u64>(), sw + (n_t - n_l), n_l,
                                   c->tup_off.as<u64>(), c->tup_bound.as<u32>(), c->cand.as<u32>(), c->cand_off.as<u64>(), dst);
     }
-    if (getenv("KAMD_DEBUG_FIN")) fprintf(stderr, "[kamd] finalize: %llu distinct tuples, smallest set 17..1024: %llu, beyond: %llu\n", (unsigned long long)n_t,
-                                          (unsigned long long)n_big, (unsigned long long)n_huge);
+    if (getenv("KAMD_DEBUG_FIN")) fprintf(stderr, "[kamd] finalize: %llu distinct tuples, smallest set 17..1024: %llu, beyond: %llu, shades by a 16-lane group: %llu, by a wavefront: %llu, bounds %s\n",
+                                          (unsigned long long)n_t, (unsigned long long)n_big, (unsigned long long)n_huge, (unsigned long long)c->host_state.n_sh_small,
+                                          (unsigned long long)c->host_state.n_sh_long, kept ? "kept" : "recomputed");
   }
   HIPC(hipGetLastError());
+  hs.mark("resolve queued");
+  if (fn) fn(user);
+  hs.mark("caller's work");
   if (int rc = sync_state(c)) return rc;
+  hs.mark("resolve done");
   if (c->host_state.shade_err) return kamd::fail(-4, "kamd_ec_finalize: a candidate slot is smaller than its shades need (k_bound_tuples and k_shade_extend disagree)");
   c->host_state.cand_words += tup_words; c->host_state.cand_recs += n_t;
   if (int rc = push_state(c)) return rc;
@@ -1196,6 +1335,7 @@
     c->host_state.cand_words = wbase + n_exp_w; c->host_state.cand_recs = rbase + n_exp_r;
   }
   const u64 n_cand = c->host_state.cand_recs;
+  const u64 cand_words_bound = c->host_state.cand_words;
   c->ccap = pow2_at_least(2 * n_cand + 16);
   if (int rc = c->ctable.ensure(c->ccap * sizeof(TSlot), 0, c->stream)) return rc;
   hipLaunchKernelGGL(k_table_init, dim3(grid_for(c->ccap, BLOCK)), dim3(BLOCK), 0, c->stream, c->ctable.as<TSlot>(), c->ccap);
@@ -1203,6 +1343,7 @@
   if (int rc = dedup_records(c, c->cand.as<u32>(), c->cand_off.as<u64>(), 0, n_cand, c->ctable.as<TSlot>(), c->ccap, c->cand_slot,
                              c->clist.as<u64>(), cand_key ? 2 : 0, cand_key, 0, c->host_state.cand_words)) return rc;
   const u64 n_final = c->host_state.n_list;
+  hs.mark("sets merged");
   if (c->track_order && n_final > 1) {
     if (int rc = c->ec_first.ensure(n_final * sizeof(u64), 0, c->stream)) return rc;
     hipLaunchKernelGGL(k_final_keys, dim3(grid_for(n_final, BLOCK)), dim3(BLOCK), 0, c->stream, c->ctable.as<TSlot>(), c->clist.as<u64>(), n_final,
@@ -1227,9 +1368,7 @@
                        c->clist.as<u64>(), n_final, c->sizes.as<u32>());
     if (int rc = exclusive_scan(c, c->sizes.as<u32>(), n_final, c->ec_off.as<u64>(), &dst->bound_words)) return rc;
     hipLaunchKernelGGL(k_set_last, dim3(1), dim3(64), 0, c->stream, c->ec_off.as<u64>(), n_final, &dst->bound_words);
-    if (int rc = sync_state(c)) return rc;
-    nnz = c->host_state.bound_words;
-    if (int rc = c->ec_ids.ensure((nnz + 1) * sizeof(u32), 0, c->stream)) return rc;
+    if (int rc = c->ec_ids.ensure((cand_words_bound + 1) * sizeof(u32), 0, c->stream)) return rc;
     hipLaunchKernelGGL(k_final_write, dim3(grid_for(n_final * 64, BLOCK)), dim3(BLOCK), 0, c->stream, c->cand.as<u32>(), c->ctable.as<TSlot>(),
                        c->clist.as<u64>(), n_final, c->ec_off.as<u64>(), c->ec_ids.as<u32>(), c->ec_counts.as<u32>());
     HIPC(hipGetLastError());
@@ -1238,7 +1377,13 @@
     if (int rc = c->ec_ids.ensure(sizeof(u32), 0, c->stream)) return rc;
   }
   HIPC(hipEventRecord(c->ev_fin1, c->stream));
-  HIPC(hipStreamSynchronize(c->stream));
+  hs.mark("CSR queued");
+  if (n_final) {
+    if (int rc = sync_state(c)) return rc;
+    nnz = c->host_state.bound_words;
+    if (nnz > cand_words_bound) return kamd::fail(-4, "kamd_ec_finalize: the final sets hold more members than the candidate stream");
+  } else HIPC(hipStreamSynchronize(c->stream));
+  hs.mark("done");
   HIPC(hipEventElapsedTime(&c->last_finalize_ms, c->ev_fin0, c->ev_fin1));
   c->last_fin_records = n_t; c->last_fin_stream_words = c->host_state.ts_words; c->last_fin_cand_words = c->host_state.cand_words;
   ++c->ec_generation;
diff --git a/kallisto_amd/csrc/kamd_em.hip b/kallisto_amd/csrc/kamd_em.hip
--- a/kallisto_amd/csrc/kamd_em.hip
+++ b/kallisto_amd/csrc/kamd_em.hip
@@ -1882,8 +1882,17 @@
                o_tf = t1.take(ng_max * 4 + 8);
   if (int rc = c->eml_tmp.ensure(t1.off, 0, c->stream)) return rc;
   char* tb = (char*)c->eml_tmp.p;
+  HostStamps hs("em_local_setup_device");
+  Carver pn;
+  const size_t n_first = pn.take(256), n_eff = pn.take(T * 8), n_g = pn.take((o_gn - o_gr) + ng_max * 4), n_rb = pn.take((ng_max + 1) * 4), n_tb = pn.take((ng_max + 1) * 4),
+               n_zb = pn.take((ng_max + 1) * 8);
+  (void)n_first; (void)n_tb; (void)n_zb;
+  if (int rc = plan_pin_ensure(c, pn.off)) return rc;
+  char* const pin = (char*)c->plan_pin;
   HIPC(hipMemsetAsync(tb, 0, o_cum, c->stream));
-  HIPC(hipMemcpyAsync(tb + o_eff, eff_lens, T * 8, hipMemcpyHostToDevice, c->stream));
+  memcpy(pin + n_eff, eff_lens, T * 8);
+  HIPC(hipMemcpyAsync(tb + o_eff, pin + n_eff, T * 8, hipMemcpyHostToDevice, c->stream));
+  hs.mark("eff queued");
   L::BuildArgs A{};
   A.ec_off = (const uint64_t*)d_ec_off; A.ec_ids = d_ec_ids; A.counts = d_counts; A.wcounts = d_wcounts; A.n_ecs = n_ecs;
   A.eff = (const double*)(tb + o_eff); A.T = T; A.label = c->labels_override ? c->labels_override : c->pt_label.as<u32>(); A.target_nnz = std::max<u64>(1, target);
@@ -1891,7 +1900,6 @@
   A.c_tr = (u32*)(tb + o_ct); A.cum_nnz = (const uint64_t*)(tb + o_cum); A.local_of = (u32*)(tb + o_loc); A.row_new = (u32*)(tb + o_rnew);
   hipLaunchKernelGGL(k_eml_step<0>, dim3(grid_for(n_ecs, BLOCK)), dim3(BLOCK), 0, c->stream, A, n_ecs);
   hipLaunchKernelGGL(k_eml_step<1>, dim3(grid_for(T, BLOCK)), dim3(BLOCK), 0, c->stream, A, T);
-  if (int rc = plan_pin_ensure(c, 256)) return rc;
   CompStats cst{};
   CompStats* const cst_pin = (CompStats*)c->plan_pin;
   u64* const nz_pin = (u64*)((char*)c->plan_pin + 64);
@@ -1908,7 +1916,9 @@
     if (int rc = exclusive_scan(c, A.c_big, T, (u64*)(tb + o_cumb), (u64*)(tb + o_cumb) + T)) return rc;
     HIPC(hipMemcpyAsync(&nz_pin[0], (u64*)(tb + o_cum) + T, 8, hipMemcpyDeviceToHost, c->stream));
     HIPC(hipMemcpyAsync(&nz_pin[1], (u64*)(tb + o_cumb) + T, 8, hipMemcpyDeviceToHost, c->stream));
+    hs.mark("sizes queued");
     HIPC(hipStreamSynchronize(c->stream));
+    hs.mark("sizes read");
     const u64 nz2[2] = {nz_pin[0], nz_pin[1]};
     cst = *cst_pin;
     NZ = nz2[0] + nz2[1];
@@ -1921,7 +1931,9 @@
   } else {
     if (int rc = exclusive_scan(c, A.c_nnz, T, (u64*)(tb + o_cum), (u64*)(tb + o_cum) + T)) return rc;
     HIPC(hipMemcpyAsync(&nz_pin[0], (u64*)(tb + o_cum) + T, 8, hipMemcpyDeviceToHost, c->stream));
+    hs.mark("sizes queued");
     HIPC(hipStreamSynchronize(c->stream));
+    hs.mark("sizes read");
     NZ = nz_pin[0];
     cst = *cst_pin;
     if (comp_out) *comp_out = cst;
@@ -1935,12 +1947,13 @@
   A.g_rows = (u32*)(tb + o_gr); A.g_tr = (u32*)(tb + o_gt); A.g_nnz = (u32*)(tb + o_gn); A.row_fill = (u32*)(tb + o_rf); A.tr_fill = (u32*)(tb + o_tf);
   hipLaunchKernelGGL(k_eml_step<2>, dim3(grid_for(T, BLOCK)), dim3(BLOCK), 0, c->stream, A, T);
   const size_t g_span = (o_gn - o_gr) + (size_t)ng * 4;
-  if (int rc = plan_pin_ensure(c, g_span)) return rc;
-  HIPC(hipMemcpyAsync(c->plan_pin, tb + o_gr, g_span, hipMemcpyDeviceToHost, c->stream));
+  HIPC(hipMemcpyAsync(pin + n_g, tb + o_gr, g_span, hipMemcpyDeviceToHost, c->stream));
+  hs.mark("groups queued");
   HIPC(hipStreamSynchronize(c->stream));
-  const u32* const g_rows = (const u32*)c->plan_pin;
-  const u32* const g_tr = (const u32*)((const char*)c->plan_pin + (o_gt - o_gr));
-  const u32* const g_nnz = (const u32*)((const char*)c->plan_pin + (o_gn - o_gr));
+  hs.mark("groups read");
+  const u32* const g_rows = (const u32*)(pin + n_g);
+  const u32* const g_tr = (const u32*)(pin + n_g + (o_gt - o_gr));
+  const u32* const g_nnz = (const u32*)(pin + n_g + (o_gn - o_gr));
   P->n_groups = ng; P->T = T; P->max_group_bytes = 0;
   P->row_base.assign(ng + 1, 0); P->tr_base.assign(ng + 1, 0); P->nz_base.assign(ng + 1, 0);
   for (u32 g = 0; g < ng; g++) {
@@ -1959,9 +1972,13 @@
   const size_t p_tt = pv.take(M * 4 + 8), p_rk = pv.take(R * 8 + 8), p_crt = pv.take(NZ * 2 + 8), p_ec = pv.take(NZ * 4 + 8), p_re = pv.take(R * 4 + 8), p_ref = pv.take(R * 4 + 8);
   if (int rc = c->pm_a.ensure(pv.off, 0, c->stream)) return rc;
   char* pb = (char*)c->pm_a.p;
-  HIPC(hipMemcpyAsync(pb + p_rb, P->row_base.data(), (ng + 1) * 4, hipMemcpyHostToDevice, c->stream));
-  HIPC(hipMemcpyAsync(pb + p_tb, P->tr_base.data(), (ng + 1) * 4, hipMemcpyHostToDevice, c->stream));
-  HIPC(hipMemcpyAsync(pb + p_zb, P->nz_base.data(), (ng + 1) * 8, hipMemcpyHostToDevice, c->stream));
+  {
+    char* const img = pin + n_rb;
+    memcpy(img, P->row_base.data(), (ng + 1) * 4);
+    memcpy(img + (p_tb - p_rb), P->tr_base.data(), (ng + 1) * 4);
+    memcpy(img + (p_zb - p_rb), P->nz_base.data(), (ng + 1) * 8);
+    HIPC(hipMemcpyAsync(pb + p_rb, img, (p_zb - p_rb) + (ng + 1) * 8, hipMemcpyHostToDevice, c->stream));
+  }
   HIPC(hipMemsetAsync(pb + p_cc, 0, p_cabs - p_cc, c->stream));
   A.row_base = (const u32*)(pb + p_rb); A.tr_base = (const u32*)(pb + p_tb); A.nz_base = (const uint64_t*)(pb + p_zb);
   A.row_ptr = (u32*)(pb + p_rp); A.col_ptr = (u32*)(pb + p_cp); A.row_tr = (uint16_t*)(pb + p_rt); A.col_row = (uint16_t*)(pb + p_cr);
@@ -1974,8 +1991,8 @@
   const bool lds_rank = rk_lds <= 150 * 1024;
   hipLaunchKernelGGL(k_eml_step<3>, dim3(grid_for(T, BLOCK)), dim3(BLOCK), 0, c->stream, A, T);
   if (lds_rank) {
-    HIPC(hipFuncSetAttribute((const void*)k_eml_rank_tr, hipFuncAttributeMaxDynamicSharedMemorySize, (int)rk_lds));
-    HIPC(hipFuncSetAttribute((const void*)k_eml_rank_rows, hipFuncAttributeMaxDynamicSharedMemorySize, (int)rk_lds));
+    if (int rc = max_dynamic_lds(c->device, (const void*)k_eml_rank_tr, rk_lds)) return rc;
+    if (int rc = max_dynamic_lds(c->device, (const void*)k_eml_rank_rows, rk_lds)) return rc;
     hipLaunchKernelGGL(k_eml_rank_tr, dim3(ng), dim3(BLOCK), rk_lds, c->stream, A);
   } else hipLaunchKernelGGL(k_eml_step<10>, dim3(grid_for(M, BLOCK)), dim3(BLOCK), 0, c->stream, A, M);
   if (A.n_groups <= (u32)RG_BINS) hipLaunchKernelGGL(k_eml_rows_g, dim3(grid_for(n_ecs, RG_BLOCK * RG_PER)), dim3(RG_BLOCK), 0, c->stream, A);
@@ -1986,7 +2003,7 @@
   for (u32 g = 0; g < ng; g++)
     gb_lds = std::max(gb_lds, ((size_t)g_rows[g] + 1 + 2 * (size_t)g_tr[g] + 1) * 4 + (((size_t)g_nnz[g] + 1) & ~(size_t)1) * 4 + 16);
   if (gb_lds <= 150 * 1024) {
-    HIPC(hipFuncSetAttribute((const void*)k_eml_group_build, hipFuncAttributeMaxDynamicSharedMemorySize, (int)gb_lds));
+    if (int rc = max_dynamic_lds(c->device, (const void*)k_eml_group_build, gb_lds)) return rc;
     hipLaunchKernelGGL(k_eml_group_build, dim3(ng), dim3(BLOCK), gb_lds, c->stream, A);
   } else {
     if (int rc = exclusive_scan(c, A.len_new, R, (u64*)(pb + p_rabs), (u64*)(pb + p_rabs) + R)) return rc;
@@ -1998,6 +2015,7 @@
     hipLaunchKernelGGL(k_eml_step<12>, dim3(grid_for(NZ, BLOCK)), dim3(BLOCK), 0, c->stream, A, NZ);
   }
   HIPC(hipGetLastError());
+  hs.mark("plan queued");
   if (host_maps) {
     P->tr_id.resize(M); P->single_all.resize(T);
     if (M) HIPC(hipMemcpyAsync(P->tr_id.data(), A.tr_id, M * 4, hipMemcpyDeviceToHost, c->stream));
@@ -2609,8 +2627,8 @@
   if (int rc = gb_setup_side(c, P.roff, P.rs, A.R, A.M, 0, &ga.rows)) return rc;
   if (int rc = gb_setup_side(c, P.coff, P.cs, A.M, A.R, 1, &ga.cols)) return rc;
   ga.cw = A.cw; ga.single = A.single; ga.eff = A.eff; ga.R = A.R; ga.M = A.M;
-  HIPC(hipFuncSetAttribute((const void*)k_gb_pass<0>, hipFuncAttributeMaxDynamicSharedMemorySize, (int)GB_LDS_BYTES));
-  HIPC(hipFuncSetAttribute((const void*)k_gb_pass<1>, hipFuncAttributeMaxDynamicSharedMemorySize, (int)GB_LDS_BYTES));
+  if (int rc = max_dynamic_lds(c->device, (const void*)k_gb_pass<0>, GB_LDS_BYTES)) return rc;
+  if (int rc = max_dynamic_lds(c->device, (const void*)k_gb_pass<1>, GB_LDS_BYTES)) return rc;
   G.gb.args = ga; G.gb.valid = true;
   if (getenv("KAMD_DEBUG_FIN")) fprintf(stderr, "[kamd] blocked EM: R %u M %u nnz %llu; rows: %u chunks, %u pieces, %u workgroups; columns: %u chunks, %u pieces, %u workgroups\n", A.R, A.M,
                                         (unsigned long long)P.nzpad, ga.rows.n_chunks, ga.rows.n_pieces, ga.rows.n_wg, ga.cols.n_chunks, ga.cols.n_pieces, ga.cols.n_wg);
@@ -2818,14 +2836,14 @@
     if (c->tune.em_reg_slices == 1) reg_words = cap <= 8 ? 2 : cap <= 16 ? 4 : cap <= 32 ? 8 : 0;
   }
   if (P.n_groups > P.n_small) {
-    HIPC(hipFuncSetAttribute((const void*)k_em_sell<false, 0>, hipFuncAttributeMaxDynamicSharedMemorySize, (int)lds));
-    HIPC(hipFuncSetAttribute((const void*)k_em_sell<true, 0>, hipFuncAttributeMaxDynamicSharedMemorySize, (int)lds));
-    HIPC(hipFuncSetAttribute((const void*)k_em_sell<false, 0, 2>, hipFuncAttributeMaxDynamicSharedMemorySize, (int)lds));
-    HIPC(hipFuncSetAttribute((const void*)k_em_sell<true, 0, 2>, hipFuncAttributeMaxDynamicSharedMemorySize, (int)lds));
-    HIPC(hipFuncSetAttribute((const void*)k_em_sell<false, 0, 4, 2>, hipFuncAttributeMaxDynamicSharedMemorySize, (int)lds));
-    HIPC(hipFuncSetAttribute((const void*)k_em_sell<true, 0, 4, 2>, hipFuncAttributeMaxDynamicSharedMemorySize, (int)lds));
-    HIPC(hipFuncSetAttribute((const void*)k_em_sell<false, 0, 8>, hipFuncAttributeMaxDynamicSharedMemorySize, (int)lds));
-    HIPC(hipFuncSetAttribute((const void*)k_em_sell<true, 0, 8>, hipFuncAttributeMaxDynamicSharedMemorySize, (int)lds));
+    if (int rc = max_dynamic_lds(c->device, (const void*)k_em_sell<false, 0>, lds)) return rc;
+    if (int rc = max_dynamic_lds(c->device, (const void*)k_em_sell<true, 0>, lds)) return rc;
+    if (int rc = max_dynamic_lds(c->device, (const void*)k_em_sell<false, 0, 2>, lds)) return rc;
+    if (int rc = max_dynamic_lds(c->device, (const void*)k_em_sell<true, 0, 2>, lds)) return rc;
+    if (int rc = max_dynamic_lds(c->device, (const void*)k_em_sell<false, 0, 4, 2>, lds)) return rc;
+    if (int rc = max_dynamic_lds(c->device, (const void*)k_em_sell<true, 0, 4, 2>, lds)) return rc;
+    if (int rc = max_dynamic_lds(c->device, (const void*)k_em_sell<false, 0, 8>, lds)) return rc;
+    if (int rc = max_dynamic_lds(c->device, (const void*)k_em_sell<true, 0, 8>, lds)) return rc;
   }
   if (gi && !c->em_ev_fork) {
     HIPC(hipEventCreateWithFlags(&c->em_ev_fork, hipEventDisableTiming));
@@ -2834,7 +2852,7 @@
   if (gi) ev_fork = c->em_ev_fork;
   if (P.n_small) {
     team_bytes = ((size_t)P.max_small_bytes + 15) & ~(size_t)15;
-    HIPC(hipFuncSetAttribute((const void*)k_em_sell_wave, hipFuncAttributeMaxDynamicSharedMemorySize, (int)(EMS_WAVE_TEAMS * team_bytes)));
+    if (int rc = max_dynamic_lds(c->device, (const void*)k_em_sell_wave, EMS_WAVE_TEAMS * team_bytes)) return rc;
     if (!c->em_side_stream) {
       HIPC(hipStreamCreateWithFlags(&c->em_side_stream, hipStreamNonBlocking));
       if (!c->em_ev_fork) {
@@ -3000,10 +3018,15 @@
   const u64 nseg = std::max(R, M);
   hipLaunchKernelGGL(k_sell_lens, dim3(grid_for(nseg, BLOCK)), dim3(BLOCK), 0, c->stream, B);
   hipLaunchKernelGGL(k_sell_sizes, dim3(grid_for(2 * (u64)ng, SELL_BUILD_WAVES)), dim3(64 * SELL_BUILD_WAVES), 0, c->stream, B);
-  if (int rc = plan_pin_ensure(c, (size_t)ng * 16)) return rc;
-  const u32* const gsz = (const u32*)c->plan_pin;
-  HIPC(hipMemcpyAsync(c->plan_pin, B.gsz, (size_t)ng * 16, hipMemcpyDeviceToHost, c->stream));
+  HostStamps hs("em_sell_setup_device");
+  Carver pn;
+  const size_t n_gsz = pn.take((size_t)ng * 16), n_img = pn.take(2 * (((size_t)(ng + 1) * 4 + 255) & ~(size_t)255) + 2 * (((size_t)(ng + 1) * 8 + 255) & ~(size_t)255));
+  if (int rc = plan_pin_ensure(c, pn.off)) return rc;
+  const u32* const gsz = (const u32*)((char*)c->plan_pin + n_gsz);
+  HIPC(hipMemcpyAsync((char*)c->plan_pin + n_gsz, B.gsz, (size_t)ng * 16, hipMemcpyDeviceToHost, c->stream));
+  hs.mark("sizes queued");
   HIPC(hipStreamSynchronize(c->stream));
+  hs.mark("sizes read");
   P->n_groups = ng; P->n_small = C.n_small; P->T = T; P->row_base = C.row_base; P->tr_base = C.tr_base; P->single_all = C.single_all;
   P->rslice_base.assign(ng + 1, 0); P->cslice_base.assign(ng + 1, 0); P->rell_base.assign(ng + 1, 0); P->cell_base.assign(ng + 1, 0);
   P->max_group_bytes = 0; P->max_small_bytes = 0;
@@ -3026,10 +3049,14 @@
   const size_t p_cw = pv.take(R * 8 + 8), p_sg = pv.take(M * 8 + 8), p_ef = pv.take(M * 8 + 8), p_id = pv.take(M * 4 + 8);
   if (int rc = c->ems_plan.ensure(pv.off, 0, c->stream)) return rc;
   char* pb = (char*)c->ems_plan.p;
-  HIPC(hipMemcpyAsync(pb + p_rsb, P->rslice_base.data(), (ng + 1) * 4, hipMemcpyHostToDevice, c->stream));
-  HIPC(hipMemcpyAsync(pb + p_csb, P->cslice_base.data(), (ng + 1) * 4, hipMemcpyHostToDevice, c->stream));
-  HIPC(hipMemcpyAsync(pb + p_reb, P->rell_base.data(), (ng + 1) * 8, hipMemcpyHostToDevice, c->stream));
-  HIPC(hipMemcpyAsync(pb + p_ceb, P->cell_base.data(), (ng + 1) * 8, hipMemcpyHostToDevice, c->stream));
+  {
+    char* const img = (char*)c->plan_pin + n_img;
+    memcpy(img + p_rsb, P->rslice_base.data(), (ng + 1) * 4);
+    memcpy(img + p_csb, P->cslice_base.data(), (ng + 1) * 4);
+    memcpy(img + p_reb, P->rell_base.data(), (ng + 1) * 8);
+    memcpy(img + p_ceb, P->cell_base.data(), (ng + 1) * 8);
+    HIPC(hipMemcpyAsync(pb + p_rsb, img, p_ceb + (ng + 1) * 8, hipMemcpyHostToDevice, c->stream));
+  }
   HIPC(hipMemsetAsync(pb + p_re, 0xFF, nru * 2, c->stream));
   HIPC(hipMemsetAsync(pb + p_ce, 0xFF, ncu * 2, c->stream));
   B.rslice_base = (const u32*)(pb + p_rsb); B.cslice_base = (const u32*)(pb + p_csb); B.rell_base = (const u64*)(pb + p_reb); B.cell_base = (const u64*)(pb + p_ceb);
@@ -3055,7 +3082,9 @@
                    B.cw_new, B.single_new, B.eff_new, (const u32*)(mb + b_gr)};
   hipLaunchKernelGGL(k_sell_group_rec, dim3(grid_for(ng, BLOCK)), dim3(BLOCK), 0, c->stream, *dev, ng, (u32*)(mb + b_gr));
   HIPC(hipGetLastError());
+  hs.mark("layout queued");
   HIPC(hipStreamSynchronize(c->stream));
+  hs.mark("layout done");
   if (cache) { cache->row_final = (u32*)(mb + b_rf); cache->mslot = (u32*)(mb + b_ms); cache->single_all = (double*)(mb + b_sa); cache->d_eff = (double*)(mb + b_ef); }
   return 0;
 }
diff --git a/kallisto_amd/csrc/kamd_match.hip b/kallisto_amd/csrc/kamd_match.hip
--- a/kallisto_amd/csrc/kamd_match.hip
+++ b/kallisto_amd/csrc/kamd_match.hip
@@ -728,7 +728,7 @@
   } else {
 #define KAMD_LAUNCH_V3L(DLV, TXT, LAY)                                                                                                   \
   do {                                                                                                                                  \
-    HIPC(hipFuncSetAttribute((const void*)k_match_v3<PAIRED, FILTER, DLV, TXT, LAY>, hipFuncAttributeMaxDynamicSharedMemorySize, (int)lds_bytes)); \
+    if (int lrc_ = max_dynamic_lds(c->device, (const void*)k_match_v3<PAIRED, FILTER, DLV, TXT, LAY>, lds_bytes)) return lrc_;                       \
     hipLaunchKernelGGL((k_match_v3<PAIRED, FILTER, DLV, TXT, LAY>), dim3(grid_for(n_waves, WAVES)), dim3(BLOCK), lds_bytes, s, c->ix, w, l, n, seq_words, \
                        rec_words, c->items_per_wave, c->refill_min, raw, stride, c->stats_a.as<DevStatsA>());                           \
   } while (0)
@@ -856,7 +856,7 @@
   u32* raw2 = c->raw2.as<u32>();
 #define KAMD_LAUNCH_V3L2(DLV, TXT, LAY)                                                                                                  \
   do {                                                                                                                                  \
-    HIPC(hipFuncSetAttribute((const void*)k_match_v3<PAIRED, FILTER, DLV, TXT, LAY, LC, true>, hipFuncAttributeMaxDynamicSharedMemorySize, (int)lds_bytes)); \
+    if (int lrc_ = max_dynamic_lds(c->device, (const void*)k_match_v3<PAIRED, FILTER, DLV, TXT, LAY, LC, true>, lds_bytes)) return lrc_;             \
     hipLaunchKernelGGL((k_match_v3<PAIRED, FILTER, DLV, TXT, LAY, LC, true>), dim3(grid_for(n_waves, WAVES)), dim3(BLOCK), lds_bytes, s, c->ix, d_words, d_len, nov, \
                        seq_words, rec_words, ipw, std::min(c->refill_min, 8), raw2, stride2, c->stats_b.as<DevStatsA>(), (const u64*)c->overflow_items.as<u64>()); \
   } while (0)
```

New measurement: 1186, median of 6. About the same (+1.3%).
